# KdaiP/StableTTS

Measured on AMD Instinct MI355X. Metric: mel-frames/sec (whole node), 31M DiT, n_timesteps=10+CFG, higher is better.
Workload: dtype f16

## Files before the change

### stabletts_amd/csrc/common.h

```cpp
#pragma once
#include <hip/hip_runtime.h>
#include <stdint.h>

namespace st {

typedef __attribute__((ext_vector_type(8))) __bf16 bf16x8_t;
typedef __attribute__((ext_vector_type(8))) _Float16 f16x8_t;
typedef __attribute__((ext_vector_type(16))) float f32x16_t;
typedef __attribute__((ext_vector_type(4))) float f32x4_t;

struct OpBF16 {
    using elem = __bf16;
    using vec8 = bf16x8_t;
    static constexpr float kMaskedScore = -1e30f;
    static __device__ __forceinline__ f32x16_t mfma(vec8 a, vec8 b, f32x16_t c) {
        return __builtin_amdgcn_mfma_f32_32x32x16_bf16(a, b, c, 0, 0, 0);
    }
    static __device__ __forceinline__ f32x4_t mfma16(vec8 a, vec8 b, f32x4_t c) {
        return __builtin_amdgcn_mfma_f32_16x16x32_bf16(a, b, c, 0, 0, 0);
    }
};
struct OpF16 {
    using elem = _Float16;
    using vec8 = f16x8_t;
    static constexpr float kMaskedScore = -60000.0f;
    static __device__ __forceinline__ f32x16_t mfma(vec8 a, vec8 b, f32x16_t c) {
        return __builtin_amdgcn_mfma_f32_32x32x16_f16(a, b, c, 0, 0, 0);
    }
    static __device__ __forceinline__ f32x4_t mfma16(vec8 a, vec8 b, f32x4_t c) {
        return __builtin_amdgcn_mfma_f32_16x16x32_f16(a, b, c, 0, 0, 0);
    }
};

template <class P>
__device__ __forceinline__ typename P::elem to16(float f) { return (typename P::elem)f; }

template <class P>
__device__ __forceinline__ uint2 pack4(float a, float b, float c, float d) {
    typedef __attribute__((ext_vector_type(4))) typename P::elem v4;
    v4 v;
    v[0] = (typename P::elem)a; v[1] = (typename P::elem)b;
    v[2] = (typename P::elem)c; v[3] = (typename P::elem)d;
    return __builtin_bit_cast(uint2, v);
}

template <class P>
__device__ __forceinline__ uint2 scale_pack4(float a, float b, float c, float d, float s) {
    float pa = a * s, pb = b * s, pc = c * s, pd = d * s;
    asm volatile("" : "+v"(pa), "+v"(pb), "+v"(pc), "+v"(pd));
    return pack4<P>(pa, pb, pc, pd);
}

template <class P>
__device__ __forceinline__ uint2 scale_pack4_lo(float a, float b, float c, float d, float s) {
    float pa = a * s, pb = b * s, pc = c * s, pd = d * s;
    asm volatile("" : "+v"(pa), "+v"(pb), "+v"(pc), "+v"(pd));
    return pack4<P>(pa - (float)to16<P>(pa), pb - (float)to16<P>(pb), pc - (float)to16<P>(pc), pd - (float)to16<P>(pd));
}

template <class P>
__device__ __forceinline__ typename P::vec8 as_vec8(uint4 v) {
    return __builtin_bit_cast(typename P::vec8, v);
}

__device__ __forceinline__ float silu_f(float x) { return x / (1.0f + expf(-x)); }
__device__ __forceinline__ float silu_grad(float a) {
    const float s = 1.0f / (1.0f + expf(-a));
    return s * (1.0f + a * (1.0f - s));
}

__device__ __forceinline__ float silu_fast(float x) {
    return x * __builtin_amdgcn_rcpf(1.0f + __builtin_amdgcn_exp2f(-1.4426950408889634f * x));
}
__device__ __forceinline__ float silu_grad_fast(float a) {
    const float s = __builtin_amdgcn_rcpf(1.0f + __builtin_amdgcn_exp2f(-1.4426950408889634f * a));
    return s * (1.0f + a * (1.0f - s));
}

__device__ __forceinline__ float gelu_erf(float x) {
    const float z = x * 0.70710678118654752f, az = fabsf(z);
    const float t = __builtin_amdgcn_rcpf(fmaf(0.3275911f, az, 1.0f));
    const float poly = t * fmaf(t, fmaf(t, fmaf(t, fmaf(t, 1.061405429f, -1.453152027f), 1.421413741f), -0.284496736f), 0.254829592f);
    const float e = __builtin_amdgcn_exp2f(-1.4426950408889634f * z * z);
    const float er = copysignf(fmaf(-poly, e, 1.0f), z);
    return 0.5f * x * (1.0f + er);
}

__device__ __forceinline__ float add_f32_scalar(float a, float b) { return a + b; }
__device__ __forceinline__ float add_f32_asm_safe(float a, float b) {
    float r;
    asm("s_nop 0\n\tv_add_f32 %0, %1, %2" : "=v"(r) : "v"(a), "v"(b));
    return r;
}

__device__ __forceinline__ void rope_rot(float& x1, float& x2, float c, float s) {
#pragma clang fp contract(off)
    const float p = x2 * s, q = x1 * s;
    const float a = __builtin_fmaf(x1, c, -p), b = __builtin_fmaf(x2, c, q);
    x1 = a; x2 = b;
}

template <int CTRL>
__device__ __forceinline__ float dpp_add(float v) {
    return v + __uint_as_float(__builtin_amdgcn_update_dpp(0u, __float_as_uint(v), CTRL, 0xf, 0xf, false));
}
__device__ __forceinline__ float xor32_sum(float v) {
    const auto r = __builtin_amdgcn_permlane32_swap(__float_as_uint(v), __float_as_uint(v), false, false);
    return __uint_as_float(r[0]) + __uint_as_float(r[1]);
}
__device__ __forceinline__ float xor32_max(float v) {
    const auto r = __builtin_amdgcn_permlane32_swap(__float_as_uint(v), __float_as_uint(v), false, false);
    return fmaxf(__uint_as_float(r[0]), __uint_as_float(r[1]));
}
__device__ __forceinline__ float wave_sum(float v) {
    v = dpp_add<0x128>(v); v = dpp_add<0x124>(v); v = dpp_add<0x122>(v); v = dpp_add<0x121>(v);
    const auto a = __builtin_amdgcn_permlane16_swap(__float_as_uint(v), __float_as_uint(v), false, false);
    return xor32_sum(__uint_as_float(a[0]) + __uint_as_float(a[1]));
}

typedef unsigned u32x4_t __attribute__((ext_vector_type(4)));
typedef unsigned u32x2_t __attribute__((ext_vector_type(2)));
#if !defined(ST_ROW_STORE_POLICY) && defined(ST_ROW_STORE_POL)
#if ST_ROW_STORE_POL == 1
#define ST_ROW_STORE_POLICY "nt"
#elif ST_ROW_STORE_POL == 2
#define ST_ROW_STORE_POLICY "sc1 nt"
#elif ST_ROW_STORE_POL == 3
#define ST_ROW_STORE_POLICY "sc0 sc1"
#elif ST_ROW_STORE_POL == 4
#define ST_ROW_STORE_POLICY "sc0 sc1 nt"
#endif
#endif
#ifndef ST_ROW_STORE_POLICY
#define ST_ROW_STORE_POLICY "sc1"
#endif
__device__ __forceinline__ void store_row16(void* p, uint4 v) {
    asm volatile("global_store_dwordx4 %0, %1, off " ST_ROW_STORE_POLICY "\n\ts_nop 1" :: "v"(p), "v"(__builtin_bit_cast(u32x4_t, v)) : "memory");
}
__device__ __forceinline__ void store_row16(void* p, float4 v) { store_row16(p, __builtin_bit_cast(uint4, v)); }
__device__ __forceinline__ void store_row8(void* p, uint2 v) {
    asm volatile("global_store_dwordx2 %0, %1, off " ST_ROW_STORE_POLICY "\n\ts_nop 1" :: "v"(p), "v"(__builtin_bit_cast(u32x2_t, v)) : "memory");
}

typedef __attribute__((address_space(3))) void lds_void_t;
typedef __attribute__((address_space(1))) const void global_cvoid_t;

__device__ __forceinline__ void glds16b(const void* gsrc, unsigned char* lds_wave_base) {
    const unsigned off = __builtin_amdgcn_readfirstlane((unsigned)(uintptr_t)(lds_void_t*)lds_wave_base);
    unsigned keep;
    asm volatile("s_mov_b32 %0, m0\n\ts_mov_b32 m0, %2\n\ts_nop 0\n\tglobal_load_lds_dwordx4 %1, off\n\ts_mov_b32 m0, %0"
                 : "=&s"(keep) : "v"(gsrc), "s"(off) : "memory");
}
__device__ __forceinline__ void glds16s(const void* sbase, unsigned voff, unsigned char* lds_wave_base) {
    const unsigned off = __builtin_amdgcn_readfirstlane((unsigned)(uintptr_t)(lds_void_t*)lds_wave_base);
    unsigned keep;
    asm volatile("s_mov_b32 %0, m0\n\ts_mov_b32 m0, %3\n\ts_nop 0\n\tglobal_load_lds_dwordx4 %1, %2\n\ts_mov_b32 m0, %0"
                 : "=&s"(keep) : "v"(voff), "s"(sbase), "s"(off) : "memory");
}
__device__ __forceinline__ void glds16o(const void* sbase, unsigned voff, unsigned lds_off) {
    unsigned keep;
    asm volatile("s_mov_b32 %0, m0\n\ts_mov_b32 m0, %3\n\ts_nop 0\n\tglobal_load_lds_dwordx4 %1, %2\n\ts_mov_b32 m0, %0"
                 : "=&s"(keep) : "v"(voff), "s"(sbase), "s"(lds_off) : "memory");
}
__device__ __forceinline__ void glds16bo(const void* gsrc, unsigned lds_off) {
    unsigned keep;
    asm volatile("s_mov_b32 %0, m0\n\ts_mov_b32 m0, %2\n\ts_nop 0\n\tglobal_load_lds_dwordx4 %1, off\n\ts_mov_b32 m0, %0"
                 : "=&s"(keep) : "v"(gsrc), "s"(lds_off) : "memory");
}
__device__ __forceinline__ void glds4bo(const void* gsrc, unsigned lds_off) {
    unsigned keep;
    asm volatile("s_mov_b32 %0, m0\n\ts_mov_b32 m0, %2\n\ts_nop 0\n\tglobal_load_lds_dword %1, off\n\ts_mov_b32 m0, %0"
                 : "=&s"(keep) : "v"(gsrc), "s"(lds_off) : "memory");
}
__device__ __forceinline__ const unsigned char* sgpr_ptr64(const void* p) {
    const uintptr_t v = (uintptr_t)p;
    return (const unsigned char*)(((uintptr_t)(unsigned)__builtin_amdgcn_readfirstlane((int)(v >> 32)) << 32) |
                                  (unsigned)__builtin_amdgcn_readfirstlane((int)(unsigned)v));
}
__device__ __forceinline__ uint4 lds_read16(unsigned addr) {
    typedef unsigned __attribute__((ext_vector_type(4))) u32x4_raw;
    const u32x4_raw v = *(const __attribute__((address_space(3))) u32x4_raw*)(uintptr_t)addr;
    return make_uint4(v[0], v[1], v[2], v[3]);
}
#define ST_DMA_WAIT(n) asm volatile("s_waitcnt vmcnt(" #n ")" ::: "memory")

__host__ __device__ __forceinline__ unsigned drop_mix32(unsigned h) {
    h ^= h >> 16; h *= 0x85ebca6bu; h ^= h >> 13; h *= 0xc2b2ae35u; h ^= h >> 16;
    return h;
}
__host__ __device__ __forceinline__ unsigned drop_pair(unsigned rh, unsigned ch) {
    unsigned h = (rh ^ ch) * 0x9E3779B1u;
    return h ^ (h >> 15);
}
__host__ __device__ __forceinline__ unsigned drop_rowh(unsigned long long seed, unsigned row) { return drop_mix32((unsigned)seed ^ (row * 0x9E3779B1u)); }
__host__ __device__ __forceinline__ unsigned drop_colh(unsigned long long seed, unsigned j) { return drop_mix32((unsigned)(seed >> 32) ^ (j * 0x85ebca77u)); }
template <class D>
// ... 38 lines not shown
```

### stabletts_amd/csrc/conv_gemm2_impl.h

```cpp
#pragma once
#include "common.h"
#include "launch.h"
#include <algorithm>
#include <cstdlib>

#ifndef ST_STAGE_TIMING
#define ST_STAGE_TIMING 0
#endif

namespace st {

template <int BC, int BF, int WC, int WF, int TAPS, int WBUF = 2>
struct G2Cfg {
    static constexpr int NW = WC * WF, NT = 64 * NW;
    static constexpr int TC = BC / WC, TF = BF / WF, FC = TC / 32, FF = TF / 32;
    static constexpr int AROWS = BF + TAPS - 1;
    static constexpr int A_BYTES = AROWS * 128, W_BYTES = BC * 128;
    static constexpr int PITCH = BC + 4;
    static constexpr int STAGE_BYTES = (NW == 8 ? TF : BF) * PITCH * 4;
    static constexpr int STAGE16_BYTES = BF * (BC * 2 + 16);
    static constexpr int LOOP_BYTES = 2 * A_BYTES + WBUF * W_BYTES;
    static constexpr int LDS_MAX2 = LOOP_BYTES > STAGE_BYTES ? LOOP_BYTES : STAGE_BYTES;
    static constexpr int LDS_BYTES = LDS_MAX2 > STAGE16_BYTES ? LDS_MAX2 : STAGE16_BYTES;
    static_assert((BC / 8) % NW == 0 && (BF / 8) % NW == 0, "DMA pieces must split evenly over the waves");
// ... 27 lines not shown
                                        const float4 (&xin)[R]) {
    size_t grow[R];
#pragma unroll
    for (int u = 0; u < R; ++u) grow[u] = (size_t)n * g.T + t[u];
    static_assert(EPI != EPI_ACT16, "EPI_ACT16 has its own epilogue (g2_epilogue_act16)");
    {
        if constexpr (EPI == EPI_F32) {
            const bool msk = g.flags & GF_MASK;
#pragma unroll
            for (int u = 0; u < R; ++u) {
                const float mm = msk ? m[u] : 1.0f;
                v[u].x = (v[u].x + k.bias.x + xin[u].x) * mm; v[u].y = (v[u].y + k.bias.y + xin[u].y) * mm;
                v[u].z = (v[u].z + k.bias.z + xin[u].z) * mm; v[u].w = (v[u].w + k.bias.w + xin[u].w) * mm;
            }
        } else {
            if (g.branch32) {
#pragma unroll
                for (int u = 0; u < R; ++u)
                    if (ok[u]) store_row16(g.branch32 + grow[u] * g.cout + ch,
                                           make_float4((v[u].x + k.bias.x) * m[u], (v[u].y + k.bias.y) * m[u], (v[u].z + k.bias.z) * m[u], (v[u].w + k.bias.w) * m[u]));
            }
#pragma unroll
            for (int u = 0; u < R; ++u) {
                v[u].x = xin[u].x + k.gate.x * ((v[u].x + k.bias.x) * m[u]); v[u].y = xin[u].y + k.gate.y * ((v[u].y + k.bias.y) * m[u]);
                v[u].z = xin[u].z + k.gate.z * ((v[u].z + k.bias.z) * m[u]); v[u].w = xin[u].w + k.gate.w * ((v[u].w + k.bias.w) * m[u]);
            }
        }
        if (g.out16) {
#pragma unroll
            for (int u = 0; u < R; ++u)
                if (ok[u]) store_row8((unsigned char*)g.out16 + (grow[u] * g.cout + ch) * 2, pack4<P>(v[u].x, v[u].y, v[u].z, v[u].w));
            if (g.out16_lo) {
#pragma unroll
                for (int u = 0; u < R; ++u) {
                    const float4 l = make_float4(v[u].x - (float)to16<P>(v[u].x), v[u].y - (float)to16<P>(v[u].y),
                                                 v[u].z - (float)to16<P>(v[u].z), v[u].w - (float)to16<P>(v[u].w));
                    if (ok[u]) store_row8((unsigned char*)g.out16_lo + (grow[u] * g.cout + ch) * 2, pack4<P>(l.x, l.y, l.z, l.w));
                }
            }
        }
        if constexpr (LN) {
            if (g.ln_h16) {
                if (g.ln_film) {
#pragma unroll
                    for (int u = 0; u < R; ++u) {
                        v[u].x = (k.ga.x * v[u].x + k.be.x) * m[u]; v[u].y = (k.ga.y * v[u].y + k.be.y) * m[u];
                        v[u].z = (k.ga.z * v[u].z + k.be.z) * m[u]; v[u].w = (k.ga.w * v[u].w + k.be.w) * m[u];
                    }
                }
                if (g.out32) {
#pragma unroll
                    for (int u = 0; u < R; ++u)
                        if (ok[u]) store_row16(g.out32 + grow[u] * g.cout + ch, v[u]);
                }
                float mean[R], rstd[R];
#pragma unroll
                for (int u = 0; u < R; ++u) mean[u] = wave_sum(v[u].x + v[u].y + v[u].z + v[u].w) * (1.0f / 256.0f);
#pragma unroll
                for (int u = 0; u < R; ++u) {
                    v[u].x -= mean[u]; v[u].y -= mean[u]; v[u].z -= mean[u]; v[u].w -= mean[u];
                    rstd[u] = wave_sum(v[u].x * v[u].x + v[u].y * v[u].y + v[u].z * v[u].z + v[u].w * v[u].w) * (1.0f / 256.0f);
                }
                const bool mout = g.ln_mask_out;
#pragma unroll
                for (int u = 0; u < R; ++u) {
                    const float rs = 1.0f / sqrtf(rstd[u] + 1e-5f);
                    const float mm = mout ? m[u] : 1.0f;
                    const float h0 = (v[u].x * rs * (1.0f + k.sc.x) + k.sh.x) * mm, h1 = (v[u].y * rs * (1.0f + k.sc.y) + k.sh.y) * mm;
                    const float h2 = (v[u].z * rs * (1.0f + k.sc.z) + k.sh.z) * mm, h3 = (v[u].w * rs * (1.0f + k.sc.w) + k.sh.w) * mm;
                    if (ok[u]) store_row8((unsigned char*)g.ln_h16 + (grow[u] * 256 + ch) * 2, pack4<P>(h0, h1, h2, h3));
                }
                return;
            }
        }
        if (g.out32 && !(EPI == EPI_RESGATE && g.out32_readonly)) {
#pragma unroll
            for (int u = 0; u < R; ++u)
                if (ok[u]) store_row16(g.out32 + grow[u] * g.cout + ch, v[u]);
        }
    }
}

template <class P, int EPI, int BC, int BF, int WC, int WF, class Park>
__device__ __forceinline__ void g2_epilogue_core(Park park, float* stage, const ConvGemmArgs& g,
                                                 int n, int t0, int fvalid, int cbase, int wave, int lane) {
    constexpr int NW = WC * WF, TF = BF / WF, PITCH = BC + 4;
    const int l31 = lane & 31, hi = lane >> 5;
    const int wf = wave / WC;
    const int T = g.T;
    static_assert(EPI != EPI_QKV && EPI != EPI_ACT16 && EPI != EPI_SILU, "QKV: g2_epilogue_qkv; ACT16: g2_epilogue_act16; SILU: g2_epilogue_silu");
    static_assert(BC == 128 || BC == 256, "row walker handles 128 or 256 channels");
    constexpr bool LN = (BC == 256);
    constexpr int PASSF = (NW == 8) ? TF : BF, WFP = PASSF / TF, NPASS = BF / PASSF;
    static_assert(PASSF % TF == 0 && BF % PASSF == 0, "pass geometry");
    constexpr int RPW = LN ? PASSF / NW : PASSF / (2 * NW);
    const int chl = LN ? lane * 4 : l31 * 4;
    const G2Consts kc = g2_consts<EPI, LN>(g, n, cbase + chl);
    const float* mrow = g.mask ? g.mask + (size_t)(n % g.mask_mod) * T : nullptr;
    const int an = n < g.add_clamp ? n : g.add_clamp;
    const int tlim = g.t_lim ? min(T, g.t_lim[n % g.t_lim_mod]) : T;
#pragma unroll 1
    for (int p = 0; p < NPASS; ++p) {
        if (wf / WFP == p) park((wf % WFP) * TF);
        const int tbase = t0 + p * PASSF;
        float mk[RPW]; float4 xin[RPW]; int fr[RPW], tt[RPW]; bool ok[RPW];
#pragma unroll
        for (int u = 0; u < RPW; ++u) {
            const int f = LN ? (wave + u * NW) : ((wave + u * NW) * 2 + hi);
            const int t = tbase + f;
            fr[u] = f; tt[u] = t;
            ok[u] = (t < tlim) && (p * PASSF + f < fvalid);
            const int tl = t < tlim ? t : tlim - 1;
            mk[u] = mrow ? mrow[tl] : 1.0f;
            xin[u] = make_float4(0.f, 0.f, 0.f, 0.f);
            if constexpr (EPI == EPI_RESGATE) xin[u] = *(const float4*)((g.res32 ? g.res32 : g.out32) + ((size_t)n * T + tl) * g.cout + cbase + chl);
            if constexpr (EPI == EPI_F32) { if (g.add32) xin[u] = *(const float4*)(g.add32 + ((size_t)an * T + tl) * g.cout + cbase + chl); }
        }
        __syncthreads();
        constexpr int RB = (EPI != EPI_ACT16 && RPW > 4) ? 4 : RPW;
#pragma unroll
        for (int b0 = 0; b0 < RPW; b0 += RB) {
            float mk2[RB]; float4 xin2[RB], v[RB]; int tt2[RB]; bool ok2[RB];
#pragma unroll
            for (int u = 0; u < RB; ++u) {
                v[u] = *(const float4*)(stage + fr[b0 + u] * PITCH + chl);
                mk2[u] = mk[b0 + u]; xin2[u] = xin[b0 + u]; tt2[u] = tt[b0 + u]; ok2[u] = ok[b0 + u];
            }
            g2_rows<P, EPI, LN, RB>(g, kc, n, tt2, ok2, cbase + chl, v, mk2, xin2);
        }
        if (p + 1 < NPASS) __syncthreads();
    }
}

template <class P, int EPI, int BC, int BF, int WC, int WF>
__device__ __forceinline__ void g2_epilogue(f32x16_t (&acc)[BC / WC / 32][BF / WF / 32], float* stage, const ConvGemmArgs& g,
                                            int n, int t0, int fvalid, int cbase, int wave, int lane) {
    constexpr int TC = BC / WC, FC = TC / 32, FF = BF / WF / 32, PITCH = BC + 4;
    const int l31 = lane & 31, hi = lane >> 5, wc = wave % WC;
    g2_epilogue_core<P, EPI, BC, BF, WC, WF>([&](int fbase) {
#pragma unroll
        for (int a = 0; a < FC; ++a)
#pragma unroll
            for (int b = 0; b < FF; ++b)
#pragma unroll
                for (int q4 = 0; q4 < 4; ++q4) {
                    const int fl = fbase + b * 32 + l31;
                    const int ch = wc * TC + a * 32 + 8 * q4 + 4 * hi;
                    *(float4*)(stage + fl * PITCH + ch) = make_float4(acc[a][b][4 * q4 + 0], acc[a][b][4 * q4 + 1],
                                                                      acc[a][b][4 * q4 + 2], acc[a][b][4 * q4 + 3]);
                }
    }, stage, g, n, t0, fvalid, cbase, wave, lane);
}

template <int EPI, int FC, int FF>
__device__ __forceinline__ void g2_init_acc(f32x16_t (&acc)[FC][FF], const ConvGemmArgs& g, int chw, int hi) {
#pragma unroll
    for (int a = 0; a < FC; ++a)
#pragma unroll
        for (int q4 = 0; q4 < 4; ++q4) {
            float4 bv = make_float4(0.f, 0.f, 0.f, 0.f);
            if constexpr (EPI == EPI_ACT16 || EPI == EPI_GELU16 || EPI == EPI_QKV) { if (g.bias) bv = *(const float4*)(g.bias + chw + a * 32 + 8 * q4 + 4 * hi); }
#pragma unroll
            for (int b = 0; b < FF; ++b) {
                acc[a][b][4 * q4 + 0] = bv.x; acc[a][b][4 * q4 + 1] = bv.y;
                acc[a][b][4 * q4 + 2] = bv.z; acc[a][b][4 * q4 + 3] = bv.w;
            }
        }
}

template <class P, int BC, int BF, int WC, int WF, bool GELU = false>
__device__ __forceinline__ void g2_epilogue_act16(f32x16_t (&acc)[BC / WC / 32][BF / WF / 32], unsigned char* stage,
                                                  const ConvGemmArgs& g, int n, int t0, int fvalid, int cbase, int wave, int lane) {
    constexpr int NW = WC * WF, TC = BC / WC, TF = BF / WF, FC = TC / 32, FF = TF / 32, PB = BC * 2 + 16;
    const int l31 = lane & 31, hi = lane >> 5;
    const int wc = wave % WC, wf = wave / WC;
    const int T = g.T;
    const bool do_silu = g.flags & GF_SILU;
    const float* mrow = ((g.flags & GF_MASK) && g.mask) ? g.mask + (size_t)(n % g.mask_mod) * T : nullptr;
#pragma unroll
    for (int b = 0; b < FF; ++b) {
        const int fl = wf * TF + b * 32 + l31;
        const int t = t0 + fl;
        const float m = mrow ? mrow[t < T ? t : T - 1] : 1.0f;
        const bool allone = __all(m == 1.0f);
#pragma unroll
        for (int a = 0; a < FC; ++a) {
            f32x16_t v = acc[a][b];
            if constexpr (GELU) {
#pragma unroll
                for (int r = 0; r < 16; ++r) v[r] = gelu_erf(v[r]);
            } else if (do_silu) {
#pragma unroll
                for (int r = 0; r < 16; ++r) v[r] = silu_fast(v[r]);
            }
            if (!allone) {
#pragma unroll
                for (int r = 0; r < 16; ++r) v[r] *= m;
            }
#pragma unroll
            for (int q4 = 0; q4 < 4; ++q4) {
                const int ch = wc * TC + a * 32 + 8 * q4 + 4 * hi;
                *(uint2*)(stage + fl * PB + ch * 2) = pack4<P>(v[4 * q4 + 0], v[4 * q4 + 1], v[4 * q4 + 2], v[4 * q4 + 3]);
            }
        }
    }
    __syncthreads();
    constexpr int LPR = BC / 8, RPI = 64 / LPR;
    const int rsub = lane / LPR, cl = lane % LPR;
    unsigned char* obase = (unsigned char*)g.out16 + (((size_t)n * T + t0) * g.cout + cbase) * 2 + cl * 16;
#pragma unroll
    for (int i = 0; i < BF / (NW * RPI); ++i) {
        const int f = (i * NW + wave) * RPI + rsub;
        const uint4 v = *(const uint4*)(stage + f * PB + cl * 16);
        if (t0 + f < T && f < fvalid) store_row16(obase + (size_t)f * g.cout * 2, v);
    }
}

template <class P, int BC, int BF, int WC, int WF>
__device__ __forceinline__ void g2_epilogue_silu(f32x16_t (&acc)[BC / WC / 32][BF / WF / 32], unsigned char* stage,
                                                 const ConvGemmArgs& g, int n, int t0, int fvalid, int cbase, int wave, int lane) {
    constexpr int NW = WC * WF, TC = BC / WC, TF = BF / WF, FC = TC / 32, FF = TF / 32, PB = BC * 2 + 16;
    constexpr int LPR = BC / 8, RPI = 64 / LPR;
    typedef __attribute__((ext_vector_type(4))) typename P::elem v4;
    const int l31 = lane & 31, hi = lane >> 5;
    const int wc = wave % WC, wf = wave / WC;
    const int T = g.T;
    const float* mrow = g.mask ? g.mask + (size_t)(n % g.mask_mod) * T : nullptr;
    struct { unsigned long long seed; unsigned thresh16; float scale; } d = {g.drop_seed, g.drop_thresh16, g.drop_scale};
    const int rsub = lane / LPR, cl = lane % LPR;
    const size_t tile0 = (((size_t)n * T + t0) * g.cout + cbase) * 2 + cl * 16;
    auto rows_out = [&](void* dst) {
#pragma unroll
        for (int i = 0; i < BF / (NW * RPI); ++i) {
            const int f = (i * NW + wave) * RPI + rsub;
            const uint4 v = *(const uint4*)(stage + f * PB + cl * 16);
            if (t0 + f < T && f < fvalid) store_row16((unsigned char*)dst + tile0 + (size_t)f * g.cout * 2, v);
        }
    };
    const bool fwd = g.act16 != nullptr;
    if (!fwd) {
#pragma unroll
        for (int i = 0; i < BF / (NW * RPI); ++i) {
            const int f = (i * NW + wave) * RPI + rsub;
            uint4 v = make_uint4(0, 0, 0, 0);
            if (t0 + f < T && f < fvalid) v = *(const uint4*)((const unsigned char*)g.dact16 + tile0 + (size_t)f * g.cout * 2);
            *(uint4*)(stage + f * PB + cl * 16) = v;
        }
        __syncthreads();
    }
    auto factors = [&](int t, int ch, float2& f01, float2& f23) {
        f01 = make_float2(1.0f, 1.0f); f23 = f01;
        if (d.thresh16) {
            const unsigned long long i = ((unsigned long long)n * T + t) * g.cout + cbase + ch;
            f01 = drop_factors2(d, drop_ffn_hash(d, i)); f23 = drop_factors2(d, drop_ffn_hash(d, i + 2));
        }
    };
    if (fwd) {
#pragma unroll
        for (int b = 0; b < FF; ++b) {
            const int fl = wf * TF + b * 32 + l31;
#pragma unroll
            for (int a = 0; a < FC; ++a)
#pragma unroll
                for (int q4 = 0; q4 < 4; ++q4) {
                    const int ch = wc * TC + a * 32 + 8 * q4 + 4 * hi;
                    const float4 bv = g.bias ? *(const float4*)(g.bias + cbase + ch) : make_float4(0.f, 0.f, 0.f, 0.f);
                    *(uint2*)(stage + fl * PB + ch * 2) = pack4<P>(acc[a][b][4 * q4 + 0] + bv.x, acc[a][b][4 * q4 + 1] + bv.y,
                                                                   acc[a][b][4 * q4 + 2] + bv.z, acc[a][b][4 * q4 + 3] + bv.w);
                }
        }
        __syncthreads();
        rows_out(g.out16);
        __syncthreads();
    }
#pragma unroll
    for (int b = 0; b < FF; ++b) {
        const int fl = wf * TF + b * 32 + l31;
        const int t = t0 + fl;
        const float m = mrow ? mrow[t < T ? t : T - 1] : 1.0f;
#pragma unroll
        for (int a = 0; a < FC; ++a)
#pragma unroll
            for (int q4 = 0; q4 < 4; ++q4) {
                const int ch = wc * TC + a * 32 + 8 * q4 + 4 * hi;
                float2 f01, f23;
                factors(t, ch, f01, f23);
                const v4 pre = *(const v4*)(stage + fl * PB + ch * 2);
                uint2 o;
                if (fwd)
                    o = pack4<P>(silu_fast((float)pre[0]) * f01.x * m, silu_fast((float)pre[1]) * f01.y * m,
                                 silu_fast((float)pre[2]) * f23.x * m, silu_fast((float)pre[3]) * f23.y * m);
                else
                    o = pack4<P>(acc[a][b][4 * q4 + 0] * m * f01.x * silu_grad_fast((float)pre[0]), acc[a][b][4 * q4 + 1] * m * f01.y * silu_grad_fast((float)pre[1]),
                                 acc[a][b][4 * q4 + 2] * m * f23.x * silu_grad_fast((float)pre[2]), acc[a][b][4 * q4 + 3] * m * f23.y * silu_grad_fast((float)pre[3]));
                *(uint2*)(stage + fl * PB + ch * 2) = o;
            }
    }
    __syncthreads();
    rows_out(fwd ? g.act16 : g.out16);
}

constexpr int kQkvRowPitch = 144;
template <int BC, int BF> constexpr int g2_qkv_lds_bytes() {
    return (BC / 64) * BF * kQkvRowPitch > BC * (BF * 2 + 16) ? (BC / 64) * BF * kQkvRowPitch : BC * (BF * 2 + 16);
}
template <class P, int BC, int BF, int WC, int WF>
__device__ __forceinline__ void g2_epilogue_qkv(f32x16_t (&acc)[BC / WC / 32][BF / WF / 32], unsigned char* stage,
                                                const ConvGemmArgs& g, int n, int t0, int cbase, int wave, int lane) {
    static_assert(BC == 256 && (BC / WC) % 64 == 0, "one q/k/v plane per block, whole heads per wave");
    constexpr int NW = WC * WF, TC = BC / WC, TF = BF / WF, FF = TF / 32, HPW = TC / 64, PQ = kQkvRowPitch, PV = BF * 2 + 16;
    const int l31 = lane & 31, hi = lane >> 5;
    const int wc = wave % WC, wf = wave / WC;
    const int T = g.T, H = g.n_heads;
    const int which = cbase / BC;
    const int tlim = g.t_lim ? min(T, g.t_lim[n % g.t_lim_mod]) : T;
    if (which < 2) {
        const float sc = which == 0 ? g.qscale : 1.0f;
        unsigned char* dst_lo = (unsigned char*)(which == 0 ? g.q_lo : g.k_lo);
        for (int pass = 0; pass < (dst_lo ? 2 : 1); ++pass) {
        if (pass) __syncthreads();
#pragma unroll
        for (int b = 0; b < FF; ++b) {
            const int fl = wf * TF + b * 32 + l31;
            const int tl = t0 + fl < T ? t0 + fl : T - 1;
            float cc[2][4], ss[2][4];
#pragma unroll
            for (int q4 = 0; q4 < 2; ++q4) {
                const float4 cs = *(const float4*)(g.rope_cos + (size_t)tl * 16 + 8 * q4 + 4 * hi);
                const float4 sn = *(const float4*)(g.rope_sin + (size_t)tl * 16 + 8 * q4 + 4 * hi);
                cc[q4][0] = cs.x; cc[q4][1] = cs.y; cc[q4][2] = cs.z; cc[q4][3] = cs.w;
                ss[q4][0] = sn.x; ss[q4][1] = sn.y; ss[q4][2] = sn.z; ss[q4][3] = sn.w;
            }
#pragma unroll
            for (int hh = 0; hh < HPW; ++hh) {
                f32x16_t r = acc[2 * hh][b];
#pragma unroll
                for (int q4 = 0; q4 < 2; ++q4)
#pragma unroll
                    for (int e = 0; e < 4; ++e) {
                        float x1 = r[4 * q4 + e], x2 = r[4 * (q4 + 2) + e];
                        rope_rot(x1, x2, cc[q4][e], ss[q4][e]);
                        r[4 * q4 + e] = x1; r[4 * (q4 + 2) + e] = x2;
                    }
                unsigned char* row = stage + ((wc * HPW + hh) * BF + fl) * PQ + 4 * hi * 2;
#pragma unroll
                for (int q4 = 0; q4 < 4; ++q4) {
                    if (pass == 0) {
                        *(uint2*)(row + 16 * q4) = scale_pack4<P>(r[4 * q4 + 0], r[4 * q4 + 1], r[4 * q4 + 2], r[4 * q4 + 3], sc);
                        *(uint2*)(row + 64 + 16 * q4) = scale_pack4<P>(acc[2 * hh + 1][b][4 * q4 + 0], acc[2 * hh + 1][b][4 * q4 + 1],
                                                                       acc[2 * hh + 1][b][4 * q4 + 2], acc[2 * hh + 1][b][4 * q4 + 3], sc);
                    } else {
                        *(uint2*)(row + 16 * q4) = scale_pack4_lo<P>(r[4 * q4 + 0], r[4 * q4 + 1], r[4 * q4 + 2], r[4 * q4 + 3], sc);
                        *(uint2*)(row + 64 + 16 * q4) = scale_pack4_lo<P>(acc[2 * hh + 1][b][4 * q4 + 0], acc[2 * hh + 1][b][4 * q4 + 1],
                                                                          acc[2 * hh + 1][b][4 * q4 + 2], acc[2 * hh + 1][b][4 * q4 + 3], sc);
                    }
                }
            }
        }
        __syncthreads();
        unsigned char* dst = pass ? dst_lo : (unsigned char*)(which == 0 ? g.q : g.k);
        const int rsub = lane >> 3, seg = lane & 7;
#pragma unroll
        for (int i = 0; i < (BC / 64) * BF / (NW * 8); ++i) {
            const int rowid = (i * NW + wave) * 8 + rsub;
            const int head = rowid / BF, f = rowid % BF;
            const uint4 v = *(const uint4*)(stage + rowid * PQ + seg * 16);
            if (t0 + f < tlim) store_row16(dst + (((size_t)n * H + head) * T + t0 + f) * 128 + seg * 16, v);
        }
        }
    } else {
        auto plane = [&](auto pass_c, unsigned char* dst) {
            constexpr bool LO = decltype(pass_c)::value;
#pragma unroll
            for (int b = 0; b < FF; ++b) {
                const int fl = wf * TF + b * 32 + l31;
                const bool tv = t0 + fl < T;
                const int pos = (fl & ~12) | ((fl & 4) << 1) | ((fl & 8) >> 1);
#pragma unroll
                for (int a = 0; a < TC / 32; ++a)
#pragma unroll
                    for (int r = 0; r < 16; ++r) {
                        const int ch = wc * TC + a * 32 + (r & 3) + 8 * (r >> 2) + 4 * hi;
                        float x = tv ? acc[a][b][r] : 0.0f;
                        if constexpr (LO) {
                            asm volatile("" : "+v"(x));
                            x -= (float)to16<P>(x);
                        }
                        *(typename P::elem*)(stage + ch * PV + pos * 2) = to16<P>(x);
                    }
            }
            __syncthreads();
            constexpr int SPR = BF / 8, RPI = 64 / SPR;
            const int rsub = lane / SPR, seg = lane % SPR;
#pragma unroll
            for (int i = 0; i < BC / (NW * RPI); ++i) {
                const int ch = (i * NW + wave) * RPI + rsub;
                const uint4 v = *(const uint4*)(stage + ch * PV + seg * 16);
                const int tcol = t0 + seg * 8;
                if (tcol < g.Tp)
                    store_row16(dst + ((((size_t)n * H + (ch >> 6)) * 64 + (ch & 63)) * g.Tp + tcol) * 2, v);
            }
        };
        plane(std::false_type{}, (unsigned char*)g.vt);
        if (g.vt_lo) {
            __syncthreads();
            plane(std::true_type{}, (unsigned char*)g.vt_lo);
        }
    }
}

template <class P, int TAPS, int EPI, int BC, int BF, int WC, int WF, int WBUF = 2>
__global__ __launch_bounds__(64 * WC * WF, WBUF == 1 ? 4 : 2)
void conv_gemm2_kernel(const ConvGemmArgs g) {
    using vec8 = typename P::vec8;
    using K = G2Cfg<BC, BF, WC, WF, TAPS, WBUF>;
    constexpr int NW = K::NW, FC = K::FC, FF = K::FF, TC = K::TC, TF = K::TF;
    constexpr int A_BYTES = K::A_BYTES, W_BYTES = K::W_BYTES;

    extern __shared__ __attribute__((aligned(16))) unsigned char smem[];
    unsigned char* As = smem;
    unsigned char* Ws = smem + 2 * A_BYTES;

    const int ks = g.ksplit > 1 ? g.ksplit : 1;
    const int total = g.n_items * g.tiles_f * g.tiles_c * ks;
    const int per_xcd = gridDim.x >> 3;
    const int lin0 = (blockIdx.x & 7) * per_xcd + (blockIdx.x >> 3);
    if (lin0 >= total) return;
    const int kz = lin0 % ks;
    const int lin = lin0 / ks;
    const int tc = lin % g.tiles_c;
    const int rest = lin / g.tiles_c;
    const int tf = rest % g.tiles_f;
    const int n = rest / g.tiles_f;

    const int tid = threadIdx.x, lane = tid & 63;
    const int wave = __builtin_amdgcn_readfirstlane(tid >> 6);
    const int l31 = lane & 31, hi = lane >> 5;
    const int wc = wave % WC, wf = wave / WC;
    const int cbase = tc * BC, t0 = tf * BF;
    if (g.t_lim && t0 >= g.t_lim[n % g.t_lim_mod]) return;
    const int cin = g.c0 + g.c1 + g.c2;
    const int nch_all = (EPI == EPI_QKV && (g.flags & GF_K2_V_ONLY) && cbase < 2 * BC ? g.c0 : cin) >> 6;
    const int cb = kz * nch_all / ks, nch = (kz + 1) * nch_all / ks;
    const int T = g.T;

    const unsigned char* a0 = (const unsigned char*)g.a0 + (size_t)(n % g.a0_mod) * T * g.c0 * 2;
    const unsigned char* a1 = g.c1 ? (const unsigned char*)g.a1 + (size_t)(n % g.a1_mod) * T * g.c1 * 2 : nullptr;
    const unsigned char* wsrc = (const unsigned char*)g.w + (size_t)n * g.w_item_stride;

    constexpr int WPW = (BC / 8) / NW, APW = (BF / 8) / NW;
    const int prow = lane >> 3;
    unsigned voffW[WPW], voffA0[APW + 1], voffA1[APW + 1];
    bool validA[APW + 1];
#pragma unroll
    for (int k = 0; k < WPW; ++k) {
        const int row = (wave * WPW + k) * 8 + prow;
        voffW[k] = (unsigned)((cbase + row) * TAPS * cin * 2 + (((lane & 7) ^ ((row >> 1) & 7)) << 4));
    }
#pragma unroll
    for (int k = 0; k <= APW; ++k) {
        const int row = (k < APW) ? (wave * APW + k) * 8 + prow : BF + prow;
        const int t = t0 + row - (TAPS / 2);
        const unsigned segb = (unsigned)(((lane & 7) ^ ((row >> 1) & 7)) << 4);
        const bool mine = (k < APW) || (TAPS == 3 && wave == 0 && lane < 16);
        validA[k] = mine && (t >= 0 && t < T);
        voffA0[k] = (unsigned)(t * g.c0 * 2) + segb;
        voffA1[k] = (unsigned)(t * g.c1 * 2) + segb;
        if (mine && !(t >= 0 && t < T)) {
            const int pc = (k < APW) ? wave * APW + k : BF / 8;
            *(uint4*)(As + pc * 1024 + lane * 16) = make_uint4(0, 0, 0, 0);
            *(uint4*)(As + A_BYTES + pc * 1024 + lane * 16) = make_uint4(0, 0, 0, 0);
        }
    }
    auto issueW = [&](int c, int j, int buf) {
        const unsigned char* sb = wsrc + (size_t)(j * cin + (c << 6)) * 2;
#pragma unroll
        for (int k = 0; k < WPW; ++k) glds16s(sb, voffW[k], Ws + buf * W_BYTES + (wave * WPW + k) * 1024);
    };
    auto issueA = [&](int c, int buf) {
        int ch0 = c << 6;
        if (ch0 >= g.c0 + g.c1) ch0 -= g.c0 + g.c1;
        if (ch0 < g.c0) {
            const unsigned char* sb = a0 + (size_t)ch0 * 2;
#pragma unroll
            for (int k = 0; k <= APW; ++k) {
                if (k == APW && TAPS != 3) continue;
                const int pc = (k < APW) ? wave * APW + k : BF / 8;
                if (validA[k]) glds16s(sb, voffA0[k], As + buf * A_BYTES + pc * 1024);
            }
        } else {
            const unsigned char* sb = a1 + (size_t)(ch0 - g.c0) * 2;
#pragma unroll
            for (int k = 0; k <= APW; ++k) {
                if (k == APW && TAPS != 3) continue;
                const int pc = (k < APW) ? wave * APW + k : BF / 8;
                if (validA[k]) glds16s(sb, voffA1[k], As + buf * A_BYTES + pc * 1024);
            }
        }
    };

    f32x16_t acc[FC][FF];
    g2_init_acc<EPI, FC, FF>(acc, g, cbase + wc * TC, hi);

    int wrow_off[FC], wswz[FC];
#pragma unroll
    for (int a = 0; a < FC; ++a) {
        const int row = wc * TC + a * 32 + l31;
        wrow_off[a] = row * 128; wswz[a] = (row >> 1) & 7;
    }
    auto compute = [&](int abuf, int wbuf, int j) {
        const unsigned char* Ab = As + abuf * A_BYTES;
        const unsigned char* Wb = Ws + wbuf * W_BYTES;
        int arow_off[FF], aswz[FF];
#pragma unroll
        for (int b = 0; b < FF; ++b) {
            const int row = wf * TF + b * 32 + l31 + j;
            arow_off[b] = row * 128; aswz[b] = (row >> 1) & 7;
        }
#pragma unroll
        for (int ks = 0; ks < 4; ++ks) {
            vec8 wfr[FC], afr[FF];
            const int seg = ks * 2 + hi;
#pragma unroll
            for (int a = 0; a < FC; ++a) wfr[a] = as_vec8<P>(*(const uint4*)(Wb + wrow_off[a] + ((seg ^ wswz[a]) << 4)));
#pragma unroll
            for (int b = 0; b < FF; ++b) afr[b] = as_vec8<P>(*(const uint4*)(Ab + arow_off[b] + ((seg ^ aswz[b]) << 4)));
#pragma unroll
            for (int a = 0; a < FC; ++a)
#pragma unroll
                for (int b = 0; b < FF; ++b) acc[a][b] = P::mfma(wfr[a], afr[b], acc[a][b]);
        }
    };

    issueA(cb, cb & 1); issueW(cb, 0, 0);
    ST_DMA_WAIT(0);
    __syncthreads();
#if ST_STAGE_TIMING
    unsigned long long tm_issue = 0, tm_compute = 0, tm_dma = 0, tm_barrier = 0, tm_n = 0;
    unsigned long long tS = __builtin_amdgcn_s_memtime();
    const unsigned long long tStart = tS;
#endif
    int it = 0;
    for (int c = cb; c < nch; ++c) {
#pragma unroll
        for (int j = 0; j < TAPS; ++j) {
            const bool last = (c == nch - 1) && (j == TAPS - 1);
            if constexpr (WBUF == 1) {
                if ((j == 0) && (c + 1 < nch)) issueA(c + 1, (c + 1) & 1);
                compute(c & 1, 0, j);
                __syncthreads();
                if (!last) { if (j == TAPS - 1) issueW(c + 1, 0, 0); else issueW(c, j + 1, 0); }
                ST_DMA_WAIT(0);
                __syncthreads();
                ++it;
                continue;
            }
            if ((j == 0) && (c + 1 < nch)) issueA(c + 1, (c + 1) & 1);
            if (!last) { if (j == TAPS - 1) issueW(c + 1, 0, (it + 1) & 1); else issueW(c, j + 1, (it + 1) & 1); }
#if ST_STAGE_TIMING
            const unsigned long long tA = __builtin_amdgcn_s_memtime();
#endif
            compute(c & 1, it & 1, j);
#if ST_STAGE_TIMING
            asm volatile("s_waitcnt lgkmcnt(0)" ::: "memory");
            const unsigned long long tB = __builtin_amdgcn_s_memtime();
#endif
            ST_DMA_WAIT(0);
#if ST_STAGE_TIMING
            const unsigned long long tC = __builtin_amdgcn_s_memtime();
#endif
            __syncthreads();
#if ST_STAGE_TIMING
            {
                const unsigned long long tD = __builtin_amdgcn_s_memtime();
                tm_issue += tA - tS; tm_compute += tB - tA; tm_dma += tC - tB; tm_barrier += tD - tC; tS = tD; ++tm_n;
            }
#endif
            ++it;
        }
    }

#if ST_STAGE_TIMING
    const unsigned long long tLoop = __builtin_amdgcn_s_memtime();
#endif
    if constexpr (EPI == EPI_ACT16 || EPI == EPI_GELU16)
        g2_epilogue_act16<P, BC, BF, WC, WF, EPI == EPI_GELU16>(acc, smem, g, n, t0, BF, cbase, wave, lane);
    else if constexpr (EPI == EPI_QKV) g2_epilogue_qkv<P, BC, BF, WC, WF>(acc, smem, g, n, t0, cbase, wave, lane);
    else g2_epilogue<P, EPI, BC, BF, WC, WF>(acc, (float*)smem, g, kz * g.n_items + n, t0, BF, cbase, wave, lane);
#if ST_STAGE_TIMING
    if (g.dbg && lane == 0 && (wave == 0 || wave == NW - 1) && lin < 64) {
        unsigned long long* d = g.dbg + (size_t)(lin * 2 + (wave ? 1 : 0)) * 8;
        d[0] = tm_issue; d[1] = tm_compute; d[2] = tm_dma; d[3] = tm_barrier; d[4] = tm_n;
        d[5] = tLoop - tStart; d[6] = __builtin_amdgcn_s_memtime() - tLoop; d[7] = 1;
    }
#endif
}

template <class P, int EPI, int BC, int BF, int WC, int WF>
__global__ __launch_bounds__(64 * WC * WF, 2) void conv_gemm3_kernel(const ConvGemmArgs g) {
    using vec8 = typename P::vec8;
    constexpr int BFV = BF - 2, NW = WC * WF, TC = BC / WC, TF = BF / WF, FC = TC / 32, FF = TF / 32;
    constexpr int A_BYTES = BF * 128, W_BYTES = BC * 128;
    constexpr int WPW = (BC / 8) / NW, APW = (BF / 8) / NW;
    static_assert(WPW == 4 && APW == 4, "the counted waits below assume 4 + 4 pieces per wave");
    extern __shared__ __attribute__((aligned(16))) unsigned char smem[];
    unsigned char* As = smem;
    unsigned char* Ws = smem + 2 * A_BYTES;

    const int total = g.n_items * g.tiles_f * g.tiles_c;
    const int per_xcd = gridDim.x >> 3;
    const int lin = (blockIdx.x & 7) * per_xcd + (blockIdx.x >> 3);
    if (lin >= total) return;
    const int tc = lin % g.tiles_c;
    const int rest = lin / g.tiles_c;
    const int tf = rest % g.tiles_f;
    const int n = rest / g.tiles_f;

    const int tid = threadIdx.x, lane = tid & 63;
    const int wave = __builtin_amdgcn_readfirstlane(tid >> 6);
    const int l31 = lane & 31, hi = lane >> 5;
    const int wc = wave % WC, wf = wave / WC;
    const int cbase = tc * BC, t0 = tf * BFV;
    if (g.t_lim && t0 >= g.t_lim[n % g.t_lim_mod]) return;
    const int cin = g.c0 + g.c1;
    const int nch = cin >> 6;
    const int nst = nch * 3;
    const int T = g.T;

    const unsigned char* a0 = (const unsigned char*)g.a0 + (size_t)(n % g.a0_mod) * T * g.c0 * 2;
    const unsigned char* a1 = g.c1 ? (const unsigned char*)g.a1 + (size_t)(n % g.a1_mod) * T * g.c1 * 2 : nullptr;
    const unsigned char* wsrc = (const unsigned char*)g.w;
    const unsigned char* zeros = (const unsigned char*)g.zeros;

    const int prow = lane >> 3;
    auto issueW = [&](int c, int j, int buf) {
#pragma unroll
        for (int k = 0; k < WPW; ++k) {
            const int piece = wave * WPW + k;
            const int row = piece * 8 + prow;
            const int seg = (lane & 7) ^ ((row >> 1) & 7);
            const unsigned char* src = wsrc + ((size_t)((cbase + row) * 3 + j) * cin + (c << 6)) * 2 + seg * 16;
            glds16b(src, Ws + buf * W_BYTES + piece * 1024);
        }
    };
    auto issueA = [&](int c, int buf) {
        const int ch0 = c << 6;
        const unsigned char* srcb; int cs, coff;
        if (ch0 < g.c0) { srcb = a0; cs = g.c0; coff = ch0; }
        else            { srcb = a1; cs = g.c1; coff = ch0 - g.c0; }
#pragma unroll
        for (int k = 0; k < APW; ++k) {
            const int piece = wave * APW + k;
            const int row = piece * 8 + prow;
            const int seg = (lane & 7) ^ ((row >> 1) & 7);
            const int t = t0 + row - 1;
            const unsigned char* src = (t >= 0 && t < T) ? srcb + ((size_t)t * cs + coff) * 2 + seg * 16 : zeros;
            glds16b(src, As + buf * A_BYTES + piece * 1024);
        }
    };

    f32x16_t acc[FC][FF];
    g2_init_acc<EPI, FC, FF>(acc, g, cbase + wc * TC, hi);

    int wrow_off[FC], wswz[FC];
#pragma unroll
    for (int a = 0; a < FC; ++a) {
        const int row = wc * TC + a * 32 + l31;
        wrow_off[a] = row * 128; wswz[a] = (row >> 1) & 7;
    }
    auto compute = [&](int abuf, int wbuf, int j) {
        const unsigned char* Ab = As + abuf * A_BYTES;
        const unsigned char* Wb = Ws + wbuf * W_BYTES;
        int arow_off[FF], aswz[FF];
#pragma unroll
        for (int b = 0; b < FF; ++b) {
            const int row = wf * TF + b * 32 + l31 + j;
            arow_off[b] = row * 128; aswz[b] = (row >> 1) & 7;
        }
#pragma unroll
        for (int ks = 0; ks < 4; ++ks) {
            vec8 wfr[FC], afr[FF];
            const int seg = ks * 2 + hi;
#pragma unroll
            for (int a = 0; a < FC; ++a) wfr[a] = as_vec8<P>(*(const uint4*)(Wb + wrow_off[a] + ((seg ^ wswz[a]) << 4)));
#pragma unroll
            for (int b = 0; b < FF; ++b) afr[b] = as_vec8<P>(*(const uint4*)(Ab + arow_off[b] + ((seg ^ aswz[b]) << 4)));
#pragma unroll
            for (int a = 0; a < FC; ++a)
#pragma unroll
                for (int b = 0; b < FF; ++b) acc[a][b] = P::mfma(wfr[a], afr[b], acc[a][b]);
        }
    };
    auto wait_keep = [&](int keep) {
        if (keep >= 8)      asm volatile("s_waitcnt vmcnt(8)" ::: "memory");
        else if (keep >= 4) asm volatile("s_waitcnt vmcnt(4)" ::: "memory");
        else                asm volatile("s_waitcnt vmcnt(0)" ::: "memory");
    };

    issueA(0, 0); issueW(0, 0, 0);
    if (nst > 1) issueW(0, 1, 1);
    wait_keep(0);
    __builtin_amdgcn_s_barrier();
    for (int c = 0; c < nch; ++c) {
#pragma unroll
        for (int j = 0; j < 3; ++j) {
            const int gi = c * 3 + j;
            int younger = 0;
            if (j == 0 && c + 1 < nch) { issueA(c + 1, (c + 1) & 1); younger += 4; }
            if (gi + 2 < nst) {
                if (j == 0) issueW(c, 2, 2); else issueW(c + 1, j - 1, j - 1);
                younger += 4;
            }
            compute(c & 1, j, j);
            wait_keep(younger);
            asm volatile("s_waitcnt lgkmcnt(0)" ::: "memory");
            __builtin_amdgcn_s_barrier();
        }
    }
    if constexpr (EPI == EPI_ACT16) g2_epilogue_act16<P, BC, BF, WC, WF>(acc, smem, g, n, t0, BFV, cbase, wave, lane);
    else g2_epilogue<P, EPI, BC, BF, WC, WF>(acc, (float*)smem, g, n, t0, BFV, cbase, wave, lane);
}

template <class P, int EPI>
__global__ __launch_bounds__(256) void splitk_finish_kernel(const ConvGemmArgs g, const float* __restrict__ part, int S) {
    const int lane = threadIdx.x & 63;
    const int wave = __builtin_amdgcn_readfirstlane((int)(threadIdx.x >> 6));
    const int rows = g.n_items * g.T;
    const int row = blockIdx.x * 4 + wave;
    if (row >= rows) return;
    const int n = row / g.T, t = row - n * g.T;
    const int ch = lane * 4;
    const G2Consts kc = g2_consts<EPI, true>(g, n, ch);
    const float* src = part + (size_t)row * 256 + ch;
    const size_t plane = (size_t)rows * 256;
    float4 v[1]; v[0] = *(const float4*)src;
    int s = 1;
    for (; s + 4 <= S; s += 4) {
        float4 p[4];
#pragma unroll
        for (int i = 0; i < 4; ++i) p[i] = *(const float4*)(src + (s + i) * plane);
#pragma unroll
        for (int i = 0; i < 4; ++i) { v[0].x += p[i].x; v[0].y += p[i].y; v[0].z += p[i].z; v[0].w += p[i].w; }
    }
    for (; s < S; ++s) {
        const float4 p = *(const float4*)(src + s * plane);
        v[0].x += p.x; v[0].y += p.y; v[0].z += p.z; v[0].w += p.w;
    }
    const float m[1] = {g.mask ? g.mask[(size_t)(n % g.mask_mod) * g.T + t] : 1.0f};
    float4 xin[1]; xin[0] = make_float4(0.f, 0.f, 0.f, 0.f);
    if constexpr (EPI == EPI_RESGATE) xin[0] = *(const float4*)((g.res32 ? g.res32 : g.out32) + (size_t)row * 256 + ch);
    if constexpr (EPI == EPI_F32) {
        if (g.add32) xin[0] = *(const float4*)(g.add32 + ((size_t)(n < g.add_clamp ? n : g.add_clamp) * g.T + t) * 256 + ch);
    }
    const int tt[1] = {t}; const bool ok[1] = {true};
    g2_rows<P, EPI, true, 1>(g, kc, n, tt, ok, ch, v, m, xin);
}

template <class P>
static hipError_t launch_splitk_finish_t(int epi, const ConvGemmArgs& a, const float* part, int S, hipStream_t s) {
    if (a.cout != 256 || S < 1 || !part) return hipErrorInvalidValue;
    const int rows = a.n_items * a.T;
    const dim3 grid((rows + 3) / 4), blk(256);
    if (epi == EPI_F32) hipLaunchKernelGGL((splitk_finish_kernel<P, EPI_F32>), grid, blk, 0, s, a, part, S);
    else if (epi == EPI_RESGATE) hipLaunchKernelGGL((splitk_finish_kernel<P, EPI_RESGATE>), grid, blk, 0, s, a, part, S);
    else return hipErrorInvalidValue;
    return hipGetLastError();
}

template <class P, int EPI, int BC = 128, int BF = 128, int WC = 2, int WF = 2>
static hipError_t launch_g3(const ConvGemmArgs& a, hipStream_t s) {
    constexpr int lds_loop = 2 * BF * 128 + 3 * BC * 128, lds_stage = (WC * WF == 8 ? BF / WF : BF) * (BC + 4) * 4;
    constexpr int lds2 = lds_loop > lds_stage ? lds_loop : lds_stage, lds16 = BF * (BC * 2 + 16);
    constexpr int lds = lds2 > lds16 ? lds2 : lds16;
    static bool attr_done_dev[64] = {};
    int dev_ = 0;
    if (hipGetDevice(&dev_) != hipSuccess || dev_ < 0 || dev_ >= 64) return hipErrorInvalidDevice;
    bool& attr_done = attr_done_dev[dev_];
    if (!attr_done) {
        hipError_t e = hipFuncSetAttribute((const void*)conv_gemm3_kernel<P, EPI, BC, BF, WC, WF>, hipFuncAttributeMaxDynamicSharedMemorySize, lds);
        if (e != hipSuccess) return e;
        attr_done = true;
    }
    if (!a.zeros || (a.cout % BC) != 0 || ((a.c0 | a.c1) & 63) != 0 || a.c2 != 0 || a.ksplit > 1) return hipErrorInvalidValue;
    ConvGemmArgs b = a;
    b.tiles_f = (a.T + BF - 3) / (BF - 2);
    b.tiles_c = a.cout / BC;
    const int total = b.n_items * b.tiles_f * b.tiles_c;
    const int grid = ((total + 7) / 8) * 8;
    hipLaunchKernelGGL((conv_gemm3_kernel<P, EPI, BC, BF, WC, WF>), dim3(grid), dim3(64 * WC * WF), lds, s, b);
    return hipGetLastError();
}

template <class P, int TAPS, int EPI, int BC, int BF, int WC, int WF, int WBUF = 2>
static hipError_t launch_g2(const ConvGemmArgs& a, hipStream_t s) {
    using K = G2Cfg<BC, BF, WC, WF, TAPS, WBUF>;
    constexpr int qkv_lds = (EPI == EPI_QKV) ? g2_qkv_lds_bytes<BC, BF>() : 0;
    constexpr int LDS = K::LDS_BYTES > qkv_lds ? K::LDS_BYTES : qkv_lds;
    static bool attr_done_dev[64] = {};
    int dev_ = 0;
    if (hipGetDevice(&dev_) != hipSuccess || dev_ < 0 || dev_ >= 64) return hipErrorInvalidDevice;
    bool& attr_done = attr_done_dev[dev_];
    if (!attr_done) {
        hipError_t e = hipFuncSetAttribute((const void*)conv_gemm2_kernel<P, TAPS, EPI, BC, BF, WC, WF, WBUF>,
                                           hipFuncAttributeMaxDynamicSharedMemorySize, LDS);
        if (e != hipSuccess) return e;
        attr_done = true;
    }
    if (!a.zeros || (a.cout % BC) != 0 || ((a.c0 | a.c1 | a.c2) & 63) != 0 || (a.c2 && a.c2 > a.c0)) return hipErrorInvalidValue;
    ConvGemmArgs b = a;
    b.tiles_f = (a.T + BF - 1) / BF;
    b.tiles_c = a.cout / BC;
    if (a.ksplit > 1) {
        if (EPI != EPI_F32 || a.bias || a.add32 || a.out16 || a.ln_h16 || (a.flags & GF_MASK) || !a.out32 ||
            a.ksplit > (a.c0 + a.c1 + a.c2) / 64 || a.w_item_stride)
            return hipErrorInvalidValue;
    }
    const int total = b.n_items * b.tiles_f * b.tiles_c * (a.ksplit > 1 ? a.ksplit : 1);
    const int grid = ((total + 7) / 8) * 8;
    if (EPI == EPI_QKV && (a.cout != 3 * BC || a.n_heads * 64 != BC || !a.q || !a.k || !a.vt)) return hipErrorInvalidValue;
    hipLaunchKernelGGL((conv_gemm2_kernel<P, TAPS, EPI, BC, BF, WC, WF, WBUF>), dim3(grid), dim3(K::NT), LDS, s, b);
    return hipGetLastError();
}

}
```

### stabletts_amd/csrc/conv_gemm2_inst.h

```cpp
#pragma once
#include "conv_gemm2_impl.h"
#include "conv_gemm_phased.h"

namespace st {

template <class P>
static hipError_t launch_conv_gemm2_t(int cfg, int taps, int epi, const ConvGemmArgs& a, hipStream_t s) {
    if (cfg == 0) {
        if (taps == 3 && epi == EPI_ACT16) return launch_g2<P, 3, EPI_ACT16, 128, 128, 2, 2>(a, s);
        if (taps == 1 && epi == EPI_F32) return launch_g2<P, 1, EPI_F32, 128, 128, 2, 2>(a, s);
        if (taps == 3 && epi == EPI_F32) return launch_g2<P, 3, EPI_F32, 128, 128, 2, 2>(a, s);
        if (taps == 1 && epi == EPI_RESGATE) return launch_g2<P, 1, EPI_RESGATE, 128, 128, 2, 2>(a, s);
        if (taps == 3 && epi == EPI_RESGATE) return launch_g2<P, 3, EPI_RESGATE, 128, 128, 2, 2>(a, s);
        if (taps == 1 && epi == EPI_GELU16) return launch_g2<P, 1, EPI_GELU16, 128, 128, 2, 2>(a, s);
    } else if (cfg == 1) {
        if (taps == 3 && epi == EPI_F32) return launch_g2<P, 3, EPI_F32, 256, 128, 4, 2>(a, s);
        if (taps == 1 && epi == EPI_F32) return launch_g2<P, 1, EPI_F32, 256, 128, 4, 2>(a, s);
        if (taps == 3 && epi == EPI_RESGATE) return launch_g2<P, 3, EPI_RESGATE, 256, 128, 4, 2>(a, s);
        if (taps == 1 && epi == EPI_RESGATE) return launch_g2<P, 1, EPI_RESGATE, 256, 128, 4, 2>(a, s);
        if (taps == 1 && epi == EPI_QKV) return launch_g2<P, 1, EPI_QKV, 256, 128, 4, 2>(a, s);
    } else if (cfg == 3) {
        if (taps == 3 && epi == EPI_ACT16) return launch_g2<P, 3, EPI_ACT16, 256, 256, 2, 4>(a, s);
        if (taps == 3 && epi == EPI_F32) return launch_g2<P, 3, EPI_F32, 256, 256, 2, 4>(a, s);
        if (taps == 1 && epi == EPI_F32) return launch_g2<P, 1, EPI_F32, 256, 256, 2, 4>(a, s);
        if (taps == 3 && epi == EPI_RESGATE) return launch_g2<P, 3, EPI_RESGATE, 256, 256, 2, 4>(a, s);
        if (taps == 1 && epi == EPI_RESGATE) return launch_g2<P, 1, EPI_RESGATE, 256, 256, 2, 4>(a, s);
        if (taps == 1 && epi == EPI_QKV) return launch_g2<P, 1, EPI_QKV, 256, 256, 2, 4>(a, s);
        if (taps == 1 && epi == EPI_GELU16) return launch_g2<P, 1, EPI_GELU16, 256, 256, 2, 4>(a, s);
    } else if (cfg == 4) {
        if (taps == 3 && epi == EPI_ACT16) return launch_g2<P, 3, EPI_ACT16, 128, 64, 2, 2>(a, s);
        if (taps == 1 && epi == EPI_F32) return launch_g2<P, 1, EPI_F32, 128, 64, 2, 2>(a, s);
        if (taps == 3 && epi == EPI_F32) return launch_g2<P, 3, EPI_F32, 128, 64, 2, 2>(a, s);
    } else if (cfg == 5) {
        if (taps == 1 && epi == EPI_QKV) return launch_g2<P, 1, EPI_QKV, 256, 64, 4, 2>(a, s);
    } else if (cfg == 6) {
        if (taps == 3 && epi == EPI_ACT16) return launch_phased3<P, EPI_ACT16>(a, s);
        if (taps == 3 && epi == EPI_F32) return launch_phased3<P, EPI_F32>(a, s);
        if (taps == 3 && epi == EPI_RESGATE) return launch_phased3<P, EPI_RESGATE>(a, s);
        if (taps == 3 && epi == EPI_SILU) return launch_phased3<P, EPI_SILU>(a, s);
    } else if (cfg == 7) {
        if (taps == 1 && epi == EPI_QKV) return launch_g2<P, 1, EPI_QKV, 256, 128, 4, 2, 1>(a, s);
    } else if (cfg == 2) {
        if (taps == 3 && epi == EPI_ACT16) return launch_g3<P, EPI_ACT16>(a, s);
        if (taps == 3 && epi == EPI_F32) return launch_g3<P, EPI_F32>(a, s);
        if (taps == 3 && epi == EPI_RESGATE) return launch_g3<P, EPI_RESGATE>(a, s);
    }
    return hipErrorInvalidValue;
}

}
```

### stabletts_amd/csrc/engine.cpp

```cpp
#include "engine_internal.h"
#include "train_launch.h"
#include "mas_launch.h"
#include "align_train_launch.h"

#include <algorithm>
#include <cmath>
#include <cstdio>
#include <cstring>
#include <map>
#include <string>
#include <vector>

using namespace st;
using namespace sthost;

namespace sthost {
std::string g_create_error;

const char* kProfNames[PC_COUNT] = {
    "prep", "prenet_conv", "in_proj", "film_ln1", "qkv_rope", "attention", "out_proj", "ln2",
    "ffn_conv1", "ffn_conv2", "lsc_conv", "final_proj", "ode_update", "train_forward", "train_backward"};

int dev_alloc(st_engine* e, void** p, size_t bytes) {
    HIPCHK(e, hipMalloc(p, bytes ? bytes : 16));
// ... 37 lines not shown
            expect(e, p + "block.attn.conv_" + nm + ".bias", {C});
        }
        expect(e, p + "block.mlp.conv_1.weight", {F, C, K}); expect(e, p + "block.mlp.conv_1.bias", {F});
        expect(e, p + "block.mlp.conv_2.weight", {C, F, K}); expect(e, p + "block.mlp.conv_2.bias", {C});
        if (G != C) {
            expect(e, p + "block.adaLN_modulation.0.weight", {C, G});
            expect(e, p + "block.adaLN_modulation.0.bias", {C});
        }
        expect(e, p + "block.adaLN_modulation.2.weight", {6 * C, C});
        expect(e, p + "block.adaLN_modulation.2.bias", {6 * C});
    }
    expect(e, "final_proj.weight", {M, C, 1}); expect(e, "final_proj.bias", {M});
    expect(e, "cond_proj.0.weight", {F, M, K}); expect(e, "cond_proj.0.bias", {F});
    expect(e, "cond_proj.2.weight", {F, F, K}); expect(e, "cond_proj.2.bias", {F});
    expect(e, "cond_proj.4.weight", {C, F, K}); expect(e, "cond_proj.4.bias", {C});
    for (int i = 0; i < e->L / 2; ++i) {
        expect(e, "lsc_layers." + std::to_string(i) + ".weight", {C, 2 * C, K});
        expect(e, "lsc_layers." + std::to_string(i) + ".bias", {C});
    }
}

const float* P(st_engine* e, const std::string& name) { return e->params.at(name).dev; }

static bool big_tiles(const st_engine* e, const ConvGemmArgs& a) {
    const int T = a.T;
    const bool fills = ((T + 255) / 256) * 256 * 10 <= ((T + 127) / 128) * 128 * 11;
    const bool big_fills_chip = (int64_t)e->conc * a.n_items * ((T + 255) / 256) * (a.cout / 256) >= e->big_min_blocks;
    return a.cout % 256 == 0 && fills && big_fills_chip;
}
bool gemm_is_phased(const st_engine* e, int taps, const ConvGemmArgs& a) { return taps == 3 && e->phased && big_tiles(e, a); }

hipError_t gemm(st_engine* e, int taps, int epi, const ConvGemmArgs& a, hipStream_t s) {
    const bool bf = e->dt == DT_BF16;
    const int T = a.T;
    if (epi == EPI_SILU && !gemm_is_phased(e, taps, a)) return hipErrorInvalidValue;
    if (e->kpart && e->conc == 1 && a.cout == 256 && (epi == EPI_F32 || epi == EPI_RESGATE) && !a.w_item_stride) {
        const int nch = (a.c0 + a.c1 + a.c2) / 64;
        const int64_t blocks = (int64_t)a.n_items * ((T + 127) / 128) * 2;
        const int64_t plane = (int64_t)a.n_items * T * 256 * 4;
        int ks = (int)std::min<int64_t>(std::min(nch, e->splitk_max), e->splitk_target / blocks);
        ks = (int)std::min<int64_t>(ks, (int64_t)e->kpart_bytes / plane);
        if (ks >= 2 && nch * taps >= e->splitk_min_stages) {
            ConvGemmArgs pa = a;
            pa.t_lim = nullptr;
            pa.bias = nullptr; pa.flags = 0; pa.mask = nullptr; pa.add32 = nullptr; pa.out16 = nullptr; pa.out16_lo = nullptr;
            pa.ln_h16 = nullptr; pa.gate = nullptr; pa.res32 = nullptr; pa.branch32 = nullptr; pa.out32 = e->kpart; pa.ksplit = ks;
            const int pcfg = e->small_tiles ? G2_T64 : G2_T128;
            hipError_t he = bf ? launch_conv_gemm2_bf16(pcfg, taps, EPI_F32, pa, s) : launch_conv_gemm2_f16(pcfg, taps, EPI_F32, pa, s);
            if (he != hipSuccess) return he;
            return bf ? launch_splitk_finish_bf16(epi, a, e->kpart, ks, s) : launch_splitk_finish_f16(epi, a, e->kpart, ks, s);
        }
    }
    if (epi == EPI_QKV && e->qkv_ws && !a.q_lo && !a.vt_lo && e->sink && a.w_frag && a.cout == 768 && a.c0 == 256 && !a.c1 && !a.c2 && a.n_heads == 4 &&
        (int64_t)a.n_items * ((T + 63) / 64) >= e->qkv_ws_min_tiles) {
        ConvGemmArgs b = a; b.sink = e->sink;
        return launch_qkv_ws(e->dt, b, s);
    }
    if (epi == EPI_RESGATE && taps == 1 && e->oproj_ws && e->sink && a.w_frag && a.ln_h16 && !a.ln_film && a.cout == 256 && a.c0 == 256 &&
        !a.c1 && !a.c2 && !a.out16 && !a.res32 && !a.branch32 && !a.out32_readonly && a.out32 &&
        (int64_t)a.n_items * ((T + 31) / 32) >= e->oproj_ws_min_tiles) {
        ConvGemmArgs b = a; b.sink = e->sink;
        return launch_oproj_ws(e->dt, b, s);
    }
    int cfg;
    if (big_tiles(e, a)) cfg = (e->phased && taps == 3) ? G2_PHASED : (epi == EPI_QKV && e->qkv_rc1) ? G2_RC1 : G2_BIG;
    else if (a.ln_h16 || epi == EPI_QKV) cfg = G2_RC;
    else if (taps == 3 && a.c0 + a.c1 >= 512 && a.c2 == 0) cfg = G2_K3PIPE;
    else cfg = G2_T128;
    const bool tiny = e->small_tiles && e->conc == 1 && (int64_t)a.n_items * ((T + 127) / 128) * (a.cout / 128) <= e->small_tiles;
    if (tiny && cfg == G2_T128 && (epi == EPI_ACT16 ? taps == 3 : epi == EPI_F32)) cfg = G2_T64;
    if (tiny && cfg == G2_RC && epi == EPI_QKV) cfg = G2_RC64;
    return bf ? launch_conv_gemm2_bf16(cfg, taps, epi, a, s) : launch_conv_gemm2_f16(cfg, taps, epi, a, s);
}

ProfScope::ProfScope(st_engine* e_, hipStream_t s_, int cls, double flops) : e(e_), s(s_) {
    if (!e->prof || !((e->prof_mask >> cls) & 1ull)) return;
    if ((e->prof_seen[cls]++ % e->prof_stride) != 0) return;
    ProfEvent ev; ev.cls = cls; ev.flops = flops;
    for (hipEvent_t* h : {&ev.a, &ev.b}) {
        if (!e->ev_pool.empty()) { *h = e->ev_pool.back(); e->ev_pool.pop_back(); }
        else if (hipEventCreate(h) != hipSuccess) return;
    }
    hipEventRecord(ev.a, s);
    e->evs.push_back(ev);
    idx = (int)e->evs.size() - 1;
}
ProfScope::~ProfScope() { if (idx >= 0) hipEventRecord(e->evs[idx].b, s); }

void prof_collect(st_engine* e) {
    for (auto& ev : e->evs) {
        float ms = 0.f;
        if (hipEventSynchronize(ev.b) == hipSuccess && hipEventElapsedTime(&ms, ev.a, ev.b) == hipSuccess) {
            e->prof_launches[ev.cls] += 1;
            e->prof_ms[ev.cls] += ms;
            e->prof_flops[ev.cls] = ev.flops;
        }
        e->ev_pool.push_back(ev.a); e->ev_pool.push_back(ev.b);
    }
    e->evs.clear();
}

void capture(st_engine* e, const std::string& name, const void* dev, int64_t n, bool is16, hipStream_t s) {
    if (!e->capture) return;
    Captured& c = e->caps[name];
    const size_t bytes = (size_t)n * (is16 ? 2 : 4);
    if (c.dev) { hipFree(c.dev); c.dev = nullptr; }
    if (hipMalloc(&c.dev, bytes) != hipSuccess) { c.dev = nullptr; return; }
    c.n = n; c.is16 = is16;
    hipMemcpyAsync(c.dev, dev, bytes, hipMemcpyDeviceToDevice, s);
}

size_t layout_plan(st_engine* e, int B, int T, bool cfg, int n_t, size_t off, Plan* p) {
    const int C = e->C, F = e->F, Mp = e->Mp, L = e->L;
    p->B = B; p->T = T; p->cfg = cfg; p->n_t = n_t;
    p->Tp = (T + 63) / 64 * 64;
    p->N = cfg ? 2 * B : B;
    p->Pn = cfg ? B + 1 : B;
    const size_t N = p->N, Pn = p->Pn, TT = T;
    p->slots.clear();
    auto want = [&](void** dst, size_t bytes) { p->slots.push_back({dst, off}); off = align_up(off + bytes, 256); };
    want(&p->mu16, Pn * TT * Mp * 2);
    want(&p->pre1, Pn * TT * F * 2);
    want(&p->pre2, Pn * TT * F * 2);
    want(&p->cond16, Pn * TT * C * 2);
    want(&p->cond16lo, Pn * TT * C * 2);
    want((void**)&p->cpart, Pn * TT * C * 4);
    want(&p->x16, (size_t)B * TT * Mp * 2);
    want(&p->x16lo, (size_t)B * TT * Mp * 2);
    want((void**)&p->xstate, (size_t)B * TT * Mp * 4);
    for (int i = 0; i < 7; ++i) want((void**)&p->kbuf[i], (size_t)B * TT * Mp * 4);
    want((void**)&p->ynew, (size_t)B * TT * Mp * 4);
    want((void**)&p->ode_partial, (size_t)2 * kOdeNormBlocks * 4);
    want((void**)&p->ode_out, 16);
    want((void**)&p->X, N * TT * C * 4);
    want(&p->h16, N * TT * C * 2);
    want(&p->h2_16, N * TT * C * 2);
    want(&p->q16, N * TT * C * 2);
    want(&p->k16, N * TT * C * 2);
    want(&p->q16lo, N * TT * C * 2);
    want(&p->k16lo, N * TT * C * 2);
    want(&p->vt16, N * (size_t)C * p->Tp * 2);
    want(&p->ao16, N * TT * C * 2);
    want(&p->u16, N * TT * F * 2);
    want(&p->cur16, N * TT * C * 2);
    want(&p->cur16lo, N * TT * C * 2);
    for (int i = 0; i < L / 2; ++i) want(&p->skip16[i], N * TT * C * 2);
    want((void**)&p->v32, N * TT * Mp * 4);
    want((void**)&p->tvals, (size_t)n_t * 4);
    want((void**)&p->emb, (size_t)n_t * C * 4);
    want((void**)&p->th, (size_t)n_t * F * 4);
    want((void**)&p->tau, (size_t)n_t * C * 4);
    want((void**)&p->film, (size_t)L * n_t * 2 * C * 4);
    want((void**)&p->cvec, N * (size_t)e->G * 4);
    want((void**)&p->ada_tmp, N * (size_t)C * 4);
    want((void**)&p->ada, (size_t)L * N * 6 * C * 4);
    want((void**)&p->n_full, (size_t)B * 4);
    want((void**)&p->kv_end, (size_t)B * 4);
    want((void**)&p->t_lim, (size_t)(B + 1) * 4);
    want((void**)&p->kbias, (size_t)B * p->Tp * 4);
    want((void**)&p->maskbuf, (size_t)B * TT * 4);
    return off;
}

int ensure_ws(st_engine* e, size_t bytes) {
    if (bytes <= e->ws_cap) return ST_OK;
    e->drop_graphs();
    if (e->ws) { HIPCHK(e, hipDeviceSynchronize()); HIPCHK(e, hipFree(e->ws)); e->ws = nullptr; e->ws_cap = 0; }
    HIPCHK(e, hipMalloc((void**)&e->ws, bytes));
    e->ws_cap = bytes;
    e->ws_sig = 0;
    return ST_OK;
}

int arena_fresh(st_engine* e, uint64_t sig, size_t used_bytes, hipStream_t s) {
    if (sig == e->ws_sig) return ST_OK;
    HIPCHK(e, hipMemsetAsync(e->ws, 0, used_bytes, s));
    e->ws_sig = sig;
    return ST_OK;
}

uint64_t layout_sig(int entry, int B, int T, int cfg, int n_t, int parts) {
    uint64_t h = 1469598103934665603ull;
    for (uint64_t v : {(uint64_t)entry, (uint64_t)B, (uint64_t)T, (uint64_t)cfg, (uint64_t)n_t, (uint64_t)parts}) { h ^= v + 0x9E3779B97F4A7C15ull; h *= 1099511628211ull; }
    return h | 1ull;
}

void bind_plan(st_engine* e, Plan* p) {
    for (auto& sl : p->slots) *sl.dst = e->ws + sl.off;
}

int make_plan(st_engine* e, int B, int T, bool cfg, int n_t, Plan* p) {
    const size_t end = layout_plan(e, B, T, cfg, n_t, 0, p);
    int rc = ensure_ws(e, end); if (rc) return rc;
    bind_plan(e, p);
    return ST_OK;
}

int ensure_rope(st_engine* e, int T, hipStream_t s) {
    if (T <= e->rope_T) return ST_OK;
    const int newT = (T + 255) / 256 * 256;
    std::vector<float> hc((size_t)newT * 16), hs((size_t)newT * 16);
    for (int j = 0; j < 16; ++j) {
        const float theta = 1.0f / powf(10000.0f, (float)(2 * j) / 32.0f);
        for (int t = 0; t < newT; ++t) {
            const float ang = (float)t * theta;
            hc[(size_t)t * 16 + j] = cosf(ang);
            hs[(size_t)t * 16 + j] = sinf(ang);
        }
    }
    if (e->rope_cos) {
        e->drop_graphs();
        HIPCHK(e, hipDeviceSynchronize()); hipFree(e->rope_cos); hipFree(e->rope_sin);
        e->rope_cos = e->rope_sin = nullptr; e->rope_T = 0;
    }
    HIPCHK(e, hipMalloc((void**)&e->rope_cos, hc.size() * 4));
    HIPCHK(e, hipMalloc((void**)&e->rope_sin, hs.size() * 4));
    HIPCHK(e, hipMemcpy(e->rope_cos, hc.data(), hc.size() * 4, hipMemcpyHostToDevice));
    HIPCHK(e, hipMemcpy(e->rope_sin, hs.data(), hs.size() * 4, hipMemcpyHostToDevice));
    e->rope_T = newT;
    (void)s;
    return ST_OK;
}

ConvGemmArgs base_args(const st_engine* e, const Plan& p, const Conv& cv, int n_items) {
    ConvGemmArgs a;
    memset(&a, 0, sizeof(a));
    a.w = cv.w; a.bias = cv.bias; a.cout = cv.cout; a.T = p.T; a.n_items = n_items;
    a.tiles_f = (p.T + kGemmFramesPerTile - 1) / kGemmFramesPerTile;
    a.tiles_c = cv.cout / kGemmChannelsPerTile;
    a.a0_mod = n_items; a.a1_mod = n_items; a.mask_mod = p.B;
    a.zeros = e->zeros;
    if (e->ragged_skip && !e->capture && e->kind == KIND_DECODER) { a.t_lim = p.t_lim; a.t_lim_mod = (n_items == p.B + 1) ? p.B + 1 : p.B; }
    return a;
}

inline double conv_flops(const Plan& p, const Conv& cv, int n_items) {
    return 2.0 * (double)n_items * p.T * cv.cout * (cv.split ? cv.cin / 3 : cv.cin) * cv.taps;
}

int run_prenet(st_engine* e, const Plan& p, hipStream_t s) {
    {
        ConvGemmArgs a = base_args(e, p, e->pre[0], p.Pn);
        a.a0 = p.mu16; a.c0 = e->Mp; a.flags = GF_SILU; a.out16 = p.pre1;
        ProfScope ps(e, s, PC_PRENET, conv_flops(p, e->pre[0], p.Pn));
        HIPCHK(e, gemm(e, 3, EPI_ACT16, a, s));
    }
    {
        ConvGemmArgs a = base_args(e, p, e->pre[1], p.Pn);
        a.a0 = p.pre1; a.c0 = e->F; a.flags = GF_SILU; a.out16 = p.pre2;
        ProfScope ps(e, s, PC_PRENET, conv_flops(p, e->pre[1], p.Pn));
        HIPCHK(e, gemm(e, 3, EPI_ACT16, a, s));
    }
    {
        ConvGemmArgs a = base_args(e, p, e->pre[2], p.Pn);
        a.a0 = p.pre2; a.c0 = e->F; a.out16 = p.cond16; a.out16_lo = p.cond16lo;
        ProfScope ps(e, s, PC_PRENET, conv_flops(p, e->pre[2], p.Pn));
        HIPCHK(e, gemm(e, 3, EPI_F32, a, s));
    }
    capture(e, "cond", p.cond16, (int64_t)p.Pn * p.T * e->C, true, s);
    {
        ConvGemmArgs a = base_args(e, p, e->inc, p.Pn);
        a.a0 = p.cond16; a.c0 = e->C; a.a1 = p.cond16lo; a.c1 = e->C; a.c2 = e->C; a.out32 = p.cpart;
        ProfScope ps(e, s, PC_INPROJ, conv_flops(p, e->inc, p.Pn));
        HIPCHK(e, gemm(e, 1, EPI_F32, a, s));
    }
    return ST_OK;
}

int run_adaln(st_engine* e, const Plan& p, hipStream_t s) {
    const int C = e->C;
    ProfScope ps(e, s, PC_PREP, 0);
    if (e->G == C) HIPCHK(e, launch_silu_rows(p.cvec, (int64_t)p.N * C, p.ada_tmp, s));
    for (int i = 0; i < e->L; ++i) {
        const std::string pre = e->blk(i) + "adaLN_modulation.";
        if (e->G != C) {
            HIPCHK(e, launch_linear(p.cvec, p.N, e->G, P(e, pre + "0.weight"), P(e, pre + "0.bias"), C, p.ada_tmp, 0, 0, s));
            HIPCHK(e, launch_linear(p.ada_tmp, p.N, C, P(e, pre + "2.weight"), P(e, pre + "2.bias"), 6 * C,
                                    p.ada + (size_t)i * p.N * 6 * C, 1, 0, s));
        } else {
            HIPCHK(e, launch_linear(p.ada_tmp, p.N, C, P(e, pre + "2.weight"), P(e, pre + "2.bias"), 6 * C,
                                    p.ada + (size_t)i * p.N * 6 * C, 0, 0, s));
        }
    }
    return ST_OK;
}

int run_time_tables(st_engine* e, const Plan& p, hipStream_t s) {
    const int C = e->C, F = e->F;
    ProfScope ps(e, s, PC_PREP, 0);
    HIPCHK(e, launch_time_embed(p.tvals, p.n_t, C, p.emb, s));
    HIPCHK(e, launch_linear(p.emb, p.n_t, C, P(e, "time_mlp.layer.0.weight"), P(e, "time_mlp.layer.0.bias"), F, p.th, 0, 1, s));
    HIPCHK(e, launch_linear(p.th, p.n_t, F, P(e, "time_mlp.layer.2.weight"), P(e, "time_mlp.layer.2.bias"), C, p.tau, 0, 0, s));
    for (int i = 0; i < e->L; ++i) {
        const std::string pre = "blocks." + std::to_string(i) + ".time_fusion.film.";
        HIPCHK(e, launch_linear(p.tau, p.n_t, C, P(e, pre + "weight"), P(e, pre + "bias"), 2 * C,
                                p.film + (size_t)i * p.n_t * 2 * C, 0, 0, s));
    }
    return ST_OK;
}

int run_estimator(st_engine* e, const Plan& p, const float* mask, int ev, hipStream_t s) {
    const int C = e->C, F = e->F, L = e->L, N = p.N, T = p.T;
    const int64_t rowsC = (int64_t)N * T * C;
    const bool cap = e->capture;
    const bool dec = e->kind == KIND_DECODER;
    const bool film = dec;
    const bool skips = dec;
    const bool dec_fast_paths = dec;
    const bool split_qk = dec_fast_paths && e->attn_split;
    const bool ragged = dec_fast_paths && e->ragged_skip && !cap;
    const int ln1_by_ffn = skips ? L / 2 : L;
    auto ada_of = [&](int i) { return p.ada + (size_t)i * N * 6 * C; };
    auto fuse_ln1 = [&](ConvGemmArgs& a, int i) {
        a.ln_film = nullptr; a.ln_film_stride = 0; a.ln_film_mod = 1;
        if (film) {
            const float* fb = p.film + (size_t)i * p.n_t * 2 * C;
            if (ev >= 0) a.ln_film = fb + (size_t)ev * 2 * C;
            else         { a.ln_film = fb; a.ln_film_stride = 2 * C; a.ln_film_mod = p.B; }
        }
        a.ln_ada = ada_of(i); a.ln_ada_stride = 6 * C; a.ln_shift_off = 0; a.ln_scale_off = C;
        a.ln_mask_out = 0; a.ln_h16 = p.h16; a.mask = mask;
    };
    if (film) {
        ConvGemmArgs a = base_args(e, p, e->inx, N);
        a.a0 = p.x16; a.c0 = e->Mp; a.a0_mod = p.B; a.a1 = p.x16lo; a.c1 = e->Mp; a.a1_mod = p.B; a.c2 = e->Mp;
        a.bias = nullptr;
        a.add32 = p.cpart; a.add_clamp = p.B;
        a.out32 = p.X; a.out16 = p.skip16[0];
        fuse_ln1(a, 0);
        ProfScope ps(e, s, PC_INPROJ, conv_flops(p, e->inx, N));
        HIPCHK(e, gemm(e, 1, EPI_F32, a, s));
    } else {
        FilmLnArgs a; memset(&a, 0, sizeof(a));
        a.X = p.X; a.h16 = p.h16; a.film = nullptr; a.film_mod = 1;
        a.ada = ada_of(0); a.ada_stride = 6 * C; a.shift_off = 0; a.scale_off = C;
        a.mask = mask; a.mask_mod = p.B; a.mask_out = 0; a.T = T; a.rows = N * T;
        ProfScope ps(e, s, PC_FILM_LN1, 0);
        HIPCHK(e, launch_film_ln(e->dt, a, s));
    }
    if (film && cap) capture(e, "h0", p.skip16[0], rowsC, true, s);
    for (int i = 0; i < L; ++i) {
        const std::string bn = "b" + std::to_string(i) + ".";
        const float* ada_i = ada_of(i);
        if (skips && i >= L / 2) {
            const int j = i - L / 2;
            ConvGemmArgs a = base_args(e, p, e->lsc[j], N);
            a.a0 = p.cur16; a.c0 = C; a.a1 = p.skip16[L - 1 - i]; a.c1 = C;
            a.out32 = p.X;
            fuse_ln1(a, i);
            ProfScope ps(e, s, PC_LSC, conv_flops(p, e->lsc[j], N));
            if (!(e->skip_mask >> PC_LSC & 1)) HIPCHK(e, gemm(e, 3, EPI_F32, a, s));
        }
        if (cap) { capture(e, bn + "x1", p.X, rowsC, false, s); capture(e, bn + "h1", p.h16, rowsC, true, s); }
        {
            ConvGemmArgs a = base_args(e, p, e->qkv[i], N);
            a.a0 = p.h16; a.c0 = C;
            a.q = p.q16; a.k = p.k16; a.vt = p.vt16; a.rope_cos = e->rope_cos; a.rope_sin = e->rope_sin;
            if (split_qk) { a.q_lo = p.q16lo; a.k_lo = p.k16lo; }
            a.Tp = p.Tp; a.n_heads = e->H;
            if ((int)e->qkv_frag.size() == L) a.w_frag = e->qkv_frag[i];
            a.qscale = 1.4426950408889634f / sqrtf((float)(C / e->H));
            ProfScope ps(e, s, PC_QKV, conv_flops(p, e->qkv[i], N));
            if (!(e->skip_mask >> PC_QKV & 1)) HIPCHK(e, gemm(e, 1, EPI_QKV, a, s));
        }
        if (cap) {
            capture(e, bn + "q", p.q16, rowsC, true, s); capture(e, bn + "k", p.k16, rowsC, true, s);
            capture(e, bn + "vt", p.vt16, (int64_t)N * C * p.Tp, true, s);
        }
        {
            AttnArgs a; memset(&a, 0, sizeof(a));
            a.q = p.q16; a.k = p.k16; a.vt = p.vt16; a.out = p.ao16; a.kbias = p.kbias; a.mask_mod = p.B; a.zeros = e->zeros;
            a.kv_end = p.kv_end; a.n_full = p.n_full; a.T = T; a.Tp = p.Tp; a.H = e->H; a.n_items = N;
            a.small_max_blocks = e->conc == 1 ? e->attn_small_blocks : 0;
            if (split_qk) { a.q_lo = p.q16lo; a.k_lo = p.k16lo; }
            if (dec_fast_paths) a.lse_max = e->lse_cells;
            if (ragged) a.t_lim = p.t_lim;
            ProfScope ps(e, s, PC_ATTN, 4.0 * (double)N * e->H * (double)T * T * (C / e->H));
            if (!(e->skip_mask >> PC_ATTN & 1)) HIPCHK(e, launch_attention(e->dt, a, s));
        }
        if (cap) capture(e, bn + "attn", p.ao16, rowsC, true, s);
        const bool fused = dec_fast_paths && e->fused_ffn && !cap && (int)e->ffn_stream.size() == L && e->ffn_stream[i] &&
                           (int64_t)e->conc * N * ((T + kFfnFusedFrames - 1) / kFfnFusedFrames) >= e->big_min_blocks;
        void* h2buf = fused ? p.h2_16 : p.h16;
        {
            ConvGemmArgs a = base_args(e, p, e->oproj[i], N);
            a.a0 = p.ao16; a.c0 = C; a.mask = mask; a.gate = ada_i + 2 * C; a.gate_stride = 6 * C; a.out32 = p.X;
            a.ln_h16 = h2buf; a.ln_film = nullptr; a.ln_film_mod = 1;
            a.ln_ada = ada_i; a.ln_ada_stride = 6 * C; a.ln_shift_off = 3 * C; a.ln_scale_off = 4 * C; a.ln_mask_out = 1;
            if (dec_fast_paths && (int)e->oproj_frag.size() == L && !cap) a.w_frag = e->oproj_frag[i];
            ProfScope ps(e, s, PC_OPROJ, conv_flops(p, e->oproj[i], N));
            if (!(e->skip_mask >> PC_OPROJ & 1)) HIPCHK(e, gemm(e, 1, EPI_RESGATE, a, s));
        }
        if (cap) { capture(e, bn + "x2", p.X, rowsC, false, s); capture(e, bn + "h2", p.h16, rowsC, true, s); }
        if (!fused) {
            ConvGemmArgs a = base_args(e, p, e->ffn1[i], N);
            a.a0 = p.h16; a.c0 = C; a.mask = mask; a.flags = GF_SILU | GF_MASK; a.out16 = p.u16;
            ProfScope ps(e, s, PC_FFN1, conv_flops(p, e->ffn1[i], N));
            HIPCHK(e, gemm(e, 3, EPI_ACT16, a, s));
        }
        if (cap) capture(e, bn + "u", p.u16, (int64_t)N * T * F, true, s);
        void* copy16 = (skips && i + 1 < L / 2) ? p.skip16[i + 1] : p.cur16;
        {
            ConvGemmArgs a = base_args(e, p, e->ffn2[i], N);
            a.a0 = p.u16; a.c0 = F; a.mask = mask; a.gate = ada_i + 5 * C; a.gate_stride = 6 * C; a.out32 = p.X;
            if (fused) { a.a0 = h2buf; a.c0 = C; a.w = e->ffn_stream[i]; a.bias1 = e->ffn1[i].bias; a.cmid = F; a.flags = GF_SILU | GF_MASK; }
            a.out16 = copy16;
            if (i + 1 == L) a.out16_lo = p.cur16lo;
            if (i + 1 < ln1_by_ffn) fuse_ln1(a, i + 1);
            else if (dec_fast_paths && !cap) a.out32_readonly = 1;
            ProfScope ps(e, s, PC_FFN2, conv_flops(p, e->ffn2[i], N) + (fused ? conv_flops(p, e->ffn1[i], N) : 0.0));
            if (e->skip_mask >> PC_FFN2 & 1) {}
            else if (fused && e->fused_ffn == 3) HIPCHK(e, launch_ffn_wino_f16(a, s));
            else if (fused) HIPCHK(e, e->dt == DT_BF16 ? launch_ffn_fused_bf16(a, s) : launch_ffn_fused_f16(a, s));
            else HIPCHK(e, gemm(e, 3, EPI_RESGATE, a, s));
        }
        if (cap) {
            if (film && i + 1 < ln1_by_ffn) capture(e, bn + "x3", copy16, rowsC, true, s);
            else capture(e, bn + "x3", p.X, rowsC, false, s);
        }
    }
    {
        ConvGemmArgs a = base_args(e, p, e->fin, N);
        a.a0 = p.cur16; a.c0 = C; a.a1 = p.cur16lo; a.c1 = C; a.c2 = C; a.mask = mask; a.flags = GF_MASK; a.out32 = p.v32;
        ProfScope ps(e, s, PC_FINAL, conv_flops(p, e->fin, N));
        HIPCHK(e, gemm(e, 1, EPI_F32, a, s));
    }
    if (cap) capture(e, "v", p.v32, (int64_t)N * T * e->Mp, false, s);
    return ST_OK;
}

int check_handle(st_engine* e, Kind kind) {
    if (!e) return ST_ERR_INVALID;
    if (e->kind != kind)
        return e->fail(ST_ERR_STATE, std::string("this handle is not a ") + kKinds[kind].what + " (" + kKinds[kind].creator + ")");
    return ST_OK;
}

int check_finalized(st_engine* e) {
    return e->finalized ? ST_OK : e->fail(ST_ERR_STATE, "st_finalize() has not been called after loading parameters");
}

int check_sizes(st_engine* e, int B, int T, const char* t_name) {
    return B >= 1 && T >= 1 ? ST_OK : e->fail(ST_ERR_INVALID, std::string("B and ") + t_name + " must be >= 1");
}

int check_dropout(st_engine* e, float p_dropout) {
    return p_dropout >= 0.0f && p_dropout < 1.0f ? ST_OK : e->fail(ST_ERR_INVALID, "p_dropout must be in [0, 1)");
}

int check_ready(st_engine* e, int B, int T) {
    if (!e) return ST_ERR_INVALID;
    int rc = check_finalized(e); if (rc) return rc;
    if ((rc = check_sizes(e, B, T))) return rc;
    if ((int64_t)2 * B * T * e->F >= (int64_t)1 << 31) return e->fail(ST_ERR_INVALID, "B*T too large for 32-bit row indexing");
    return ST_OK;
}

int new_handle(Kind kind, int device, st_engine** out) {
    int ndev = 0;
    if (hipGetDeviceCount(&ndev) != hipSuccess || device < 0 || device >= ndev) { g_create_error = "no such HIP device"; return ST_ERR_HIP; }
    if (hipSetDevice(device) != hipSuccess) { g_create_error = "hipSetDevice failed"; return ST_ERR_HIP; }
    st_engine* e = new st_engine();
    e->device = device; e->kind = kind;
    *out = e;
    return ST_OK;
}

static int find_param(st_engine* e, const char* name, const float* data, const int64_t* shape, int ndim, Param** out) {
    if (!e) return ST_ERR_INVALID;
    if (!name || !data || !shape) return e->fail(ST_ERR_INVALID, "null argument");
    auto it = e->params.find(name);
    if (it == e->params.end()) return e->fail(ST_ERR_INVALID, std::string("unexpected parameter name: ") + name);
    Param& p = it->second;
    bool ok = (int)p.shape.size() == ndim;
    for (int i = 0; ok && i < ndim; ++i) ok = p.shape[i] == shape[i];
    if (!ok) return e->fail(ST_ERR_INVALID, std::string("shape mismatch for ") + name);
    *out = &p;
    return ST_OK;
}

}

extern "C" {

int st_abi_version(void) { return ST_ABI_VERSION; }

static int create_engine(const st_config* cfg, Kind kind, int n_vocab, int device, st_engine** out) {
    if (!cfg || !out) { g_create_error = "null argument"; return ST_ERR_INVALID; }
    auto bad = [&](const char* m) { g_create_error = m; return ST_ERR_INVALID; };
    if (kind == KIND_DECODER && (cfg->n_layers % 2 != 0 || cfg->n_layers < 2 || cfg->n_layers > 16))
        return bad("n_layers must be even (estimator.py:92) and in [2, 16]");
    if (kind == KIND_TEXT_ENCODER && (cfg->n_layers < 1 || cfg->n_layers > 16)) return bad("n_layers must be in [1, 16]");
    if (kind == KIND_TEXT_ENCODER && n_vocab < 1) return bad("n_vocab must be >= 1");
    if (cfg->hidden_channels % 2 != 0) return bad("SinusoidalPosEmb requires dim to be even (estimator.py:39)");
    if (cfg->n_heads < 1 || cfg->hidden_channels % cfg->n_heads != 0)
        return bad("channels % n_heads != 0 (diffusion_transformer.py:35)");
    if (cfg->hidden_channels != 256) { g_create_error = "native kernels are built for hidden_channels == 256"; return ST_ERR_UNSUPPORTED; }
    if (cfg->hidden_channels / cfg->n_heads != 64) { g_create_error = "native kernels are built for head_dim == 64"; return ST_ERR_UNSUPPORTED; }
    if (cfg->kernel_size != 3) { g_create_error = "native kernels are built for kernel_size == 3"; return ST_ERR_UNSUPPORTED; }
    if (cfg->filter_channels % 128 != 0 || cfg->filter_channels < 128) { g_create_error = "filter_channels must be a multiple of 128"; return ST_ERR_UNSUPPORTED; }
    if (cfg->noise_channels < 1 || cfg->noise_channels > 1024) return bad("noise_channels out of range");
    if (cfg->gin_channels < 4 || cfg->gin_channels % 4 != 0) return bad("gin_channels must be a positive multiple of 4");
    if (cfg->operand_dtype != ST_OPERAND_BF16 && cfg->operand_dtype != ST_OPERAND_F16) return bad("operand_dtype");
    st_engine* e = nullptr;
    if (int rc = new_handle(kind, device, &e)) return rc;
    e->cfg = *cfg;
    e->dt = cfg->operand_dtype == ST_OPERAND_BF16 ? DT_BF16 : DT_F16;
    e->M = cfg->noise_channels; e->Mp = (e->M + 127) / 128 * 128;
    e->C = cfg->hidden_channels; e->F = cfg->filter_channels; e->H = cfg->n_heads; e->L = cfg->n_layers;
    e->K = cfg->kernel_size; e->G = cfg->gin_channels;
    e->n_vocab = n_vocab;
    if (const char* mb = getenv("ST_BIG_MIN_BLOCKS")) e->big_min_blocks = atoi(mb);
    if (const char* v = getenv("ST_PHASED")) e->phased = atoi(v);
    if (const char* v = getenv("ST_FUSED_FFN")) e->fused_ffn = atoi(v);
    if (e->fused_ffn < 0 || e->fused_ffn > 3 || e->fused_ffn == 2) e->fused_ffn = 1;
    if (e->fused_ffn == 3 && e->dt != DT_F16) e->fused_ffn = 1;
    if (const char* v = getenv("ST_RAGGED_SKIP")) e->ragged_skip = atoi(v);
#ifdef ST_DEVTOOLS
    if (const char* v = getenv("ST_SKIP_CLASSES")) e->skip_mask = (unsigned)strtoul(v, nullptr, 0);
#endif
    if (const char* v = getenv("ST_QKV_WS")) e->qkv_ws = atoi(v);
    if (const char* v = getenv("ST_QKV_WS_MIN_TILES")) e->qkv_ws_min_tiles = atoi(v);
    if (const char* v = getenv("ST_OPROJ_WS")) e->oproj_ws = atoi(v);
    if (const char* v = getenv("ST_OPROJ_WS_MIN_TILES")) e->oproj_ws_min_tiles = atoi(v);
    if (const char* v = getenv("ST_QKV_RC1")) e->qkv_rc1 = atoi(v);
    if (const char* v = getenv("ST_SMALL_GRID")) {
        if (atoi(v) == 0) {
            e->splitk_target = 0; e->small_tiles = 0; e->attn_small_blocks = 0;
        }
    }
    build_param_table(e);
    if (hipMalloc((void**)&e->kpart, kSplitKBytes) == hipSuccess) e->kpart_bytes = kSplitKBytes; else e->kpart = nullptr;
    if (hipMalloc(&e->sink, 65536) != hipSuccess) e->sink = nullptr;
    if (hipMalloc((void**)&e->lse_cells, kLseCells * 64) != hipSuccess ||
        hipMemsetD32((hipDeviceptr_t)e->lse_cells, (int)0x80000000, kLseCells * 16) != hipSuccess) { (void)hipGetLastError(); e->lse_cells = nullptr; }
    if (hipMalloc(&e->zeros, 256) != hipSuccess || hipMemset(e->zeros, 0, 256) != hipSuccess) {
        g_create_error = "hipMalloc failed";
        if (e->kpart) hipFree(e->kpart);
        delete e;
        return ST_ERR_HIP;
    }
    if (hipHostMalloc((void**)&e->status_host, sizeof(int), hipHostMallocMapped) == hipSuccess &&
        hipHostGetDevicePointer((void**)&e->status_dev, e->status_host, 0) == hipSuccess) *e->status_host = 0;
    else { (void)hipGetLastError(); e->status_host = nullptr; e->status_dev = nullptr; }
    *out = e;
    return ST_OK;
}

int st_create(const st_config* cfg, int device, st_engine** out) { return create_engine(cfg, KIND_DECODER, 0, device, out); }

int st_create_text_encoder(const st_config* cfg, int n_vocab, int device, st_engine** out) {
    return create_engine(cfg, KIND_TEXT_ENCODER, n_vocab, device, out);
}

void st_destroy(st_engine* e) {
    if (!e) return;
    hipSetDevice(e->device);
    hipDeviceSynchronize();
    e->drop_graphs();
    train_destroy(e);
    vocos_destroy(e);
    style_destroy(e);
    duration_destroy(e);
    mel_destroy(e);
    period_disc_destroy(e);
    resolution_disc_destroy(e);
    ffgan_destroy(e);
    sd_train_destroy(e);
    if (e->gstream) hipStreamDestroy(e->gstream);
    e->part_streams.destroy();
    for (auto& kv : e->params) if (kv.second.dev && !kv.second.borrowed) hipFree(kv.second.dev);
    for (void* p : e->owned) hipFree(p);
    for (auto& kv : e->caps) if (kv.second.dev) hipFree(kv.second.dev);
    prof_collect(e);
    for (hipEvent_t ev : e->ev_pool) hipEventDestroy(ev);
    if (e->ws) hipFree(e->ws);
    if (e->adams_buf) hipFree(e->adams_buf);
    if (e->pk_fwd.dev) hipFree(e->pk_fwd.dev);
    if (e->pk_T.dev) hipFree(e->pk_T.dev);
    if (e->rope_cos) hipFree(e->rope_cos);
    if (e->rope_sin) hipFree(e->rope_sin);
// ... 327 lines not shown
    if (!duration || !mask || !cum_scratch || !path) return align_fail(ST_ERR_INVALID, "null tensor pointer");
    if (B < 1 || Tx < 1 || Ty < 1 || B > 65535 || Tx > 65535) return align_fail(ST_ERR_INVALID, "shape out of range");
    if (launch_cumsum_rows(duration, B, Tx, cum_scratch, (hipStream_t)stream) != hipSuccess ||
        launch_path(cum_scratch, mask, B, Tx, Ty, path, (hipStream_t)stream) != hipSuccess)
        return align_fail(ST_ERR_HIP, "generate_path kernel launch failed");
    return ST_OK;
}

int st_align(const float* cum, const float* x_mask, const int64_t* y_lengths, const float* mu_x, int B, int M, int Tx, int Ty,
             float* attn, float* mu_y, float* y_mask, void* stream) {
    if (!cum || !x_mask || !y_lengths || !mu_x || !mu_y) return align_fail(ST_ERR_INVALID, "null tensor pointer");
    if (B < 1 || M < 1 || Tx < 1 || Ty < 1 || B > 65535) return align_fail(ST_ERR_INVALID, "shape out of range");
    if (launch_align(cum, x_mask, (const long long*)y_lengths, mu_x, B, M, Tx, Ty, attn, mu_y, y_mask, (hipStream_t)stream) != hipSuccess)
        return align_fail(ST_ERR_HIP, "align kernel launch failed");
    return ST_OK;
}

int64_t st_maximum_path_workspace_bytes(int B, int Ty, int Tx) { return (int64_t)mas_workspace_bytes(B, Ty, Tx); }

int st_maximum_path(const float* neg_cent, const int32_t* t_y, const int32_t* t_x, int B, int Ty, int Tx, float* path,
                    int32_t* durations, void* workspace, void* stream) {
    if (!neg_cent || !t_y || !t_x || !path) return align_fail(ST_ERR_INVALID, "null tensor pointer");
    if (B < 1 || Ty < 1 || Tx < 1 || B > 65535) return align_fail(ST_ERR_INVALID, "shape out of range");
    if (Tx > kMasMaxTx) return align_fail(ST_ERR_UNSUPPORTED, "maximum_path supports Tx <= 4096 (one row per wave in registers)");
    if (mas_workspace_bytes(B, Ty, Tx) && !workspace)
        return align_fail(ST_ERR_INVALID, "this shape needs st_maximum_path_workspace_bytes() of workspace");
    if (launch_mas_path(neg_cent, t_y, t_x, B, Ty, Tx, path, durations, workspace, (hipStream_t)stream) != hipSuccess)
        return align_fail(ST_ERR_HIP, "maximum_path kernel launch failed");
    return ST_OK;
}

int st_mas_neg_cent(const float* mu_x, const float* y, int B, int D, int Tx, int Ty, float* neg_cent, void* stream) {
    if (!mu_x || !y || !neg_cent) return align_fail(ST_ERR_INVALID, "null tensor pointer");
    if (B < 1 || D < 1 || Tx < 1 || Ty < 1 || B > 65535 || (Ty + 63) / 64 > 65535) return align_fail(ST_ERR_INVALID, "shape out of range");
    if (launch_mas_neg_cent(mu_x, y, B, D, Tx, Ty, neg_cent, (hipStream_t)stream) != hipSuccess)
        return align_fail(ST_ERR_HIP, "neg_cent kernel launch failed");
    return ST_OK;
}

int st_align_train_scratch_floats(int B, int M, int Ty) {
    if (B < 1 || M < 1 || Ty < 1) return ST_ERR_INVALID;
    return align_train_scratch_floats(B, M, Ty);
}

static int align_train_shape(int B, int M, int Tx, int Ty) {
    if (B < 1 || M < 1 || Tx < 1 || Ty < 1 || B > 65535 || (M + kAlignTrainChannels - 1) / kAlignTrainChannels > 65535 ||
        align_train_scratch_floats(B, M, Ty) < 0)
        return align_fail(ST_ERR_INVALID, "shape out of range");
    if (Tx > kAlignTrainMaxTx) return align_fail(ST_ERR_UNSUPPORTED, "the alignment training kernels support Tx <= 4096 (one item's running sum in LDS)");
    return ST_OK;
}

int st_align_train_forward(const int32_t* durations, const float* x_mask, const float* y_mask, const float* mu_x, const float* y,
                           const float* fake_content, const float* keep, int B, int M, int Tx, int Ty, int32_t* frame_token,
                           float* mu_y, float* mu_y_masked, float* scratch, float* prior_loss, void* stream) {
    if (!durations || !x_mask || !y_mask || !mu_x || !y || !frame_token || !mu_y_masked || !scratch || !prior_loss)
        return align_fail(ST_ERR_INVALID, "null tensor pointer");
    if (int rc = align_train_shape(B, M, Tx, Ty)) return rc;
    if (launch_align_train_forward(durations, x_mask, y_mask, mu_x, y, fake_content, keep, B, M, Tx, Ty, frame_token, mu_y, mu_y_masked,
                                   scratch, prior_loss, (hipStream_t)stream) != hipSuccess)
        return align_fail(ST_ERR_HIP, "align_train_forward kernel launch failed");
    return ST_OK;
}

int st_align_train_backward(const int32_t* durations, const float* x_mask, const float* y_mask, const float* mu_x, const float* y,
                            const float* keep, const float* scratch, const float* grad_mu_y_masked, const float* grad_mu_y,
                            const float* grad_prior, int B, int M, int Tx, int Ty, float* grad_mu_x, float* grad_fake_content,
                            void* stream) {
    if (!durations || !x_mask || !mu_x || !grad_mu_x) return align_fail(ST_ERR_INVALID, "null tensor pointer");
    if (grad_prior && (!y || !y_mask || !scratch)) return align_fail(ST_ERR_INVALID, "grad_prior needs y, y_mask and the forward's scratch");
    if (int rc = align_train_shape(B, M, Tx, Ty)) return rc;
    if (launch_align_train_backward(durations, x_mask, y_mask, mu_x, y, keep, scratch, grad_mu_y_masked, grad_mu_y, grad_prior, B, M, Tx,
                                    Ty, grad_mu_x, grad_fake_content, (hipStream_t)stream) != hipSuccess)
        return align_fail(ST_ERR_HIP, "align_train_backward kernel launch failed");
    return ST_OK;
}

int st_duration_loss_scratch_floats(void) { return kDurLossScratchFloats; }

int st_duration_loss(const float* logw, const int32_t* durations, const float* x_mask, const int64_t* x_lengths, int B, int Tx,
                     float* logw_target, float* scratch, float* loss, void* stream) {
    if (!logw || !durations || !x_mask || !x_lengths || !scratch || !loss) return align_fail(ST_ERR_INVALID, "null tensor pointer");
    if (B < 1 || Tx < 1) return align_fail(ST_ERR_INVALID, "shape out of range");
    if (launch_duration_loss(logw, durations, x_mask, (const long long*)x_lengths, B, Tx, logw_target, scratch, loss, (hipStream_t)stream) != hipSuccess)
        return align_fail(ST_ERR_HIP, "duration_loss kernel launch failed");
    return ST_OK;
}

int st_duration_loss_backward(const float* logw, const int32_t* durations, const float* x_mask, const float* scratch,
                              const float* grad_loss, int B, int Tx, float* grad_logw, void* stream) {
    if (!logw || !durations || !x_mask || !scratch || !grad_loss || !grad_logw) return align_fail(ST_ERR_INVALID, "null tensor pointer");
    if (B < 1 || Tx < 1) return align_fail(ST_ERR_INVALID, "shape out of range");
    if (launch_duration_loss_bwd(logw, durations, x_mask, scratch, grad_loss, B, Tx, grad_logw, (hipStream_t)stream) != hipSuccess)
        return align_fail(ST_ERR_HIP, "duration_loss_bwd kernel launch failed");
    return ST_OK;
}

int st_output_status(st_engine* e, void* stream, int* nonfinite) {
    if (!e) return ST_ERR_INVALID;
    if (!nonfinite) return e->fail(ST_ERR_INVALID, "null argument");
    if (!e->status_host) return e->fail(ST_ERR_UNSUPPORTED, "host-mapped status word unavailable on this device");
    HIPCHK(e, hipSetDevice(e->device));
    HIPCHK(e, hipStreamSynchronize((hipStream_t)stream));
    *nonfinite = *e->status_host != 0;
    e->arena_poisoned();
    return ST_OK;
}

int st_cfm_loss_prep(const float* x1, const float* z, const float* t_rand, float sigma_min, int B, int M, int T, float* t, float* y,
                     float* u, void* stream) {
    if (!x1 || !z || !t_rand || !t || !y || !u) return align_fail(ST_ERR_INVALID, "null tensor pointer");
    if (B < 1 || M < 1 || T < 1 || B > 65535) return align_fail(ST_ERR_INVALID, "shape out of range");
    if (launch_cfm_loss_prep(x1, z, t_rand, sigma_min, B, M, T, t, y, u, (hipStream_t)stream) != hipSuccess)
        return align_fail(ST_ERR_HIP, "cfm_loss_prep kernel launch failed");
    return ST_OK;
}

int st_cfm_loss(const float* pred, const float* u, const float* mask, int B, int M, int T, float* scratch, float* loss, void* stream) {
    if (!pred || !u || !mask || !scratch || !loss) return align_fail(ST_ERR_INVALID, "null tensor pointer");
    if (B < 1 || M < 1 || T < 1) return align_fail(ST_ERR_INVALID, "shape out of range");
    if (launch_cfm_loss(pred, u, mask, B, M, T, scratch, loss, (hipStream_t)stream) != hipSuccess)
        return align_fail(ST_ERR_HIP, "cfm_loss kernel launch failed");
    return ST_OK;
}

int st_cfm_loss_backward(const float* pred, const float* u, const float* scratch, const float* grad_loss, int B, int M, int T,
                         float* grad_pred, void* stream) {
    if (!pred || !u || !scratch || !grad_loss || !grad_pred) return align_fail(ST_ERR_INVALID, "null tensor pointer");
    if (B < 1 || M < 1 || T < 1) return align_fail(ST_ERR_INVALID, "shape out of range");
    if (launch_cfm_loss_bwd(pred, u, scratch, grad_loss, B, M, T, grad_pred, (hipStream_t)stream) != hipSuccess)
        return align_fail(ST_ERR_HIP, "cfm_loss_bwd kernel launch failed");
    return ST_OK;
}

int st_cfm_loss_scratch_floats(void) { return 2 * kCfmLossBlocks + 2; }

int st_last_solve_stats(const st_engine* e, int64_t* nfe, int64_t* steps, int64_t* rejects) {
    if (!e) return ST_ERR_INVALID;
    if (nfe) *nfe = e->last_nfe;
    if (steps) *steps = e->last_steps;
    if (rejects) *rejects = e->last_rejects;
    return ST_OK;
}

int st_set_option(st_engine* e, const char* name, int value) {
    if (!e || !name) return ST_ERR_INVALID;
    const std::string n(name);
    if (n == "attention_precision") {
        if (value != 0 && value != 1) return e->fail(ST_ERR_INVALID, "attention_precision: 0 (16-bit q / k operands) or 1 (split hi + lo operands)");
        if (e->kind != KIND_DECODER) return e->fail(ST_ERR_UNSUPPORTED, "attention_precision: CFM decoder handles only");
        if (value != e->attn_split) { e->drop_graphs(); e->attn_split = value; }
        return ST_OK;
    }
    if (n == "fused_ffn") return e->fail(ST_ERR_INVALID, "fused_ffn is read-only (ST_FUSED_FFN at st_create)");
    return e->fail(ST_ERR_INVALID, std::string("unknown option: ") + name);
}

int st_get_option(const st_engine* e, const char* name, int* value) {
    if (!e || !name || !value) return ST_ERR_INVALID;
    const std::string n(name);
    if (n == "attention_precision") { *value = e->attn_split; return ST_OK; }
    if (n == "fused_ffn") { *value = e->fused_ffn; return ST_OK; }
    return ST_ERR_INVALID;
}

int st_attention_stats(st_engine* e, void* stream, float* max_lse) {
    if (!e || !max_lse) return ST_ERR_INVALID;
    if (!e->lse_cells) return e->fail(ST_ERR_STATE, "attention statistics unavailable (allocation failed at st_create)");
    HIPCHK(e, hipSetDevice(e->device));
    HIPCHK(e, hipStreamSynchronize((hipStream_t)stream));
    int cells[kLseCells * 16];
    HIPCHK(e, hipMemcpy(cells, e->lse_cells, sizeof(cells), hipMemcpyDeviceToHost));
    int best = (int)0x80000000;
    for (int c = 0; c < kLseCells; ++c) best = std::max(best, cells[c * 16]);
    HIPCHK(e, hipMemsetD32((hipDeviceptr_t)e->lse_cells, (int)0x80000000, kLseCells * 16));
    if (best == (int)0x80000000) { *max_lse = -INFINITY; return ST_OK; }
    const int bits = best >= 0 ? best : best ^ 0x7fffffff;
    float v; memcpy(&v, &bits, 4);
    *max_lse = v * 0.6931471805599453f;
    return ST_OK;
}

int st_debug_capture(st_engine* e, int enable) {
    if (!e) return ST_ERR_INVALID;
    e->capture = enable != 0;
    if (!enable) {
        hipSetDevice(e->device);
        hipDeviceSynchronize();
        for (auto& kv : e->caps) if (kv.second.dev) hipFree(kv.second.dev);
        e->caps.clear();
    }
    return ST_OK;
}

int64_t st_debug_fetch(st_engine* e, const char* name, float* host_out, int64_t capacity) {
    if (!e || !name) return ST_ERR_INVALID;
    auto it = e->caps.find(name);
    if (it == e->caps.end() || !it->second.dev) { e->err = std::string("no captured tensor named ") + name; return ST_ERR_INVALID; }
    Captured& c = it->second;
    if (!host_out) return c.n;
    if (capacity < c.n) { e->err = "capacity too small"; return ST_ERR_INVALID; }
    if (hipSetDevice(e->device) != hipSuccess || hipDeviceSynchronize() != hipSuccess) return ST_ERR_HIP;
    if (!c.is16) {
        if (hipMemcpy(host_out, c.dev, (size_t)c.n * 4, hipMemcpyDeviceToHost) != hipSuccess) return ST_ERR_HIP;
        return c.n;
    }
    float* tmp = nullptr;
    if (hipMalloc((void**)&tmp, (size_t)c.n * 4) != hipSuccess) return ST_ERR_HIP;
    hipError_t r = launch_cvt16_to_f32(e->dt, c.dev, tmp, c.n, nullptr);
    if (r == hipSuccess) r = hipMemcpy(host_out, tmp, (size_t)c.n * 4, hipMemcpyDeviceToHost);
    hipFree(tmp);
    return r == hipSuccess ? c.n : (int64_t)ST_ERR_HIP;
}

int st_profile_enable(st_engine* e, int enable) {
    if (!e) return ST_ERR_INVALID;
    hipSetDevice(e->device);
    prof_collect(e);
    e->prof = enable != 0;
    for (int i = 0; i < PC_COUNT; ++i) { e->prof_launches[i] = 0; e->prof_ms[i] = 0; e->prof_flops[i] = 0; }
    return ST_OK;
}

int st_profile_select(st_engine* e, uint64_t class_mask) {
    if (!e) return ST_ERR_INVALID;
    e->prof_mask = class_mask;
    return ST_OK;
}

int st_profile_stride(st_engine* e, int stride) {
    if (!e || stride < 1) return ST_ERR_INVALID;
    e->prof_stride = stride;
    for (int i = 0; i < PC_COUNT; ++i) e->prof_seen[i] = 0;
    return ST_OK;
}

int st_profile_num_classes(void) { return PC_COUNT; }

const char* st_profile_class_name(int cls) { return (cls >= 0 && cls < PC_COUNT) ? kProfNames[cls] : ""; }

int st_profile_read(st_engine* e, int cls, int64_t* launches, double* total_ms, double* flops_per_launch) {
    if (!e || cls < 0 || cls >= PC_COUNT) return ST_ERR_INVALID;
    hipSetDevice(e->device);
    prof_collect(e);
    if (launches) *launches = e->prof_launches[cls];
    if (total_ms) *total_ms = e->prof_ms[cls];
    if (flops_per_launch) *flops_per_launch = e->prof_flops[cls];
    e->prof_launches[cls] = 0; e->prof_ms[cls] = 0;
    return ST_OK;
}

int64_t st_device_bytes(const st_engine* e) {
    if (!e) return ST_ERR_INVALID;
    int64_t n = e->weight_bytes + (int64_t)e->ws_cap + train_bytes(e);
    if (e->sdt) n += (int64_t)(e->sdt->act_cap + e->sdt->scr_cap);
    for (auto& kv : e->params) if (kv.second.dev && !kv.second.borrowed) n += kv.second.numel() * 4;
    return n;
}

}
```

### stabletts_amd/csrc/engine_internal.h

```cpp
#pragma once
#include "../../include/stabletts_hip.h"
#include "launch.h"
#include "stream_fork.h"

#include <map>
#include <string>
#include <vector>

namespace sthost {

enum ProfClass {
    PC_PREP = 0, PC_PRENET, PC_INPROJ, PC_FILM_LN1, PC_QKV, PC_ATTN, PC_OPROJ, PC_LN2, PC_FFN1, PC_FFN2,
    PC_LSC, PC_FINAL, PC_ODE, PC_TRAIN_FWD, PC_TRAIN_BWD, PC_COUNT
};

struct Param {
    std::vector<int64_t> shape;
    float* dev = nullptr;
    bool loaded = false;
    bool borrowed = false;
    int64_t numel() const { int64_t n = 1; for (auto s : shape) n *= s; return n; }
};

struct Conv {
    void* w = nullptr;
    float* bias = nullptr;
    int cout = 0, cin = 0, taps = 0;
    bool split = false;
};

struct Captured { void* dev = nullptr; int64_t n = 0; bool is16 = false; };

struct ProfEvent { int cls; hipEvent_t a, b; double flops; };

inline size_t align_up(size_t v, size_t a) { return (v + a - 1) / a * a; }

struct FloatArena {
    size_t off = 0;
    size_t want(size_t n) { const size_t o = off; off += (n + 63) / 64 * 64; return o; }
};

enum Kind { KIND_DECODER = 0, KIND_TEXT_ENCODER, KIND_VOCODER, KIND_STYLE_ENCODER, KIND_DURATION_PREDICTOR, KIND_MEL_EXTRACTOR, KIND_PERIOD_DISC, KIND_RESOLUTION_DISC,
            KIND_FFGAN, KIND_COUNT };
struct KindName { const char* what; const char* creator; };
constexpr KindName kKinds[KIND_COUNT] = {
    {"CFM decoder", "st_create"},
    {"text encoder", "st_create_text_encoder"},
    {"vocoder", "st_create_vocoder"},
    {"style encoder", "st_create_style_encoder"},
    {"duration predictor", "st_create_duration_predictor"},
    {"mel extractor", "st_create_mel_extractor"},
    {"period discriminator", "st_create_period_discriminator"},
    {"resolution discriminator", "st_create_resolution_discriminator"},
    {"FireflyGAN vocoder", "st_create_ffgan"},
};
constexpr bool reads_params_in_place(Kind k) { return k == KIND_STYLE_ENCODER || k == KIND_DURATION_PREDICTOR; }

struct TrainState;
struct VocosState;
struct StyleState;
struct DurState;
struct MelState;
struct PdState;
struct RdState;
struct FfganState;

struct SdTrain {
    char* act = nullptr; size_t act_cap = 0;
    char* scr = nullptr; size_t scr_cap = 0;
    int64_t serial = 0;
    bool have = false;
    int B = 0, T = 0;
    float p = 0.0f; unsigned long long seed = 0;
    bool masked = false;
};
int sd_train_grow(st_engine* e, char** buf, size_t* cap, size_t bytes);
void sd_train_destroy(st_engine* e);
SdTrain* sd_train_begin(st_engine* e);
void sd_train_commit(SdTrain* st, int B, int T, float p_dropout, unsigned long long seed, bool masked);
int sd_train_check(st_engine* e, const char* entry, const char* t_name, int64_t serial, int B, int T);

}

constexpr int kMaxParts = 1 + sthost::StreamFork::kMaxChildren;
constexpr int kSplitKMax = 16;
constexpr size_t kSplitKBytes = 32u << 20;

struct st_engine {
    st_config cfg{};
    int device = 0;
    int dt = st::DT_BF16;
    int M = 0, Mp = 0, C = 0, F = 0, H = 0, L = 0, K = 0, G = 0;
    sthost::Kind kind = sthost::KIND_DECODER;
    int n_vocab = 0;
    std::string blk(int i) const {
        return kind == sthost::KIND_DECODER ? "blocks." + std::to_string(i) + ".block." : "encoder." + std::to_string(i) + ".";
    }
    std::map<std::string, sthost::Param> params;
    bool finalized = false;
    struct PackList { std::vector<st::PackJob> jobs; st::PackJob* dev = nullptr; unsigned nblocks = 0; bool ready = false; bool recording = false; };
    PackList pk_fwd, pk_T;
    bool packed_once = false;
    std::string err;
    int64_t weight_bytes = 0;

    std::vector<sthost::Conv> pre;
    sthost::Conv inx, inc, fin;
    std::vector<sthost::Conv> lsc, qkv, oproj, ffn1, ffn2;
    std::vector<void*> oproj_frag;
    std::vector<void*> qkv_frag;
    std::vector<void*> ffn_stream;
    std::vector<void*> owned;

    float* rope_cos = nullptr; float* rope_sin = nullptr; int rope_T = 0;
    void* sink = nullptr;
    void* zeros = nullptr;

    char* ws = nullptr; size_t ws_cap = 0;
    uint64_t ws_sig = 0;

    bool capture = false;
    std::map<std::string, sthost::Captured> caps;
    bool prof = false;
    uint64_t prof_mask = ~0ull;
    int prof_stride = 1;
    int64_t prof_seen[sthost::PC_COUNT] = {0};
    std::vector<sthost::ProfEvent> evs;
    std::vector<hipEvent_t> ev_pool;
    int64_t prof_launches[sthost::PC_COUNT] = {0};
    double prof_ms[sthost::PC_COUNT] = {0};
    double prof_flops[sthost::PC_COUNT] = {0};

    int64_t last_nfe = 0, last_steps = 0, last_rejects = 0;
    int* status_host = nullptr; int* status_dev = nullptr;
    bool arena_poisoned() { if (status_host && *status_host) { *status_host = 0; ws_sig = 0; return true; } return false; }

    void* adams_buf = nullptr; size_t adams_bytes = 0;
    int big_min_blocks = 192;
    unsigned skip_mask = 0;
    int qkv_ws_min_tiles = 400;
    int qkv_ws = 1;
    int oproj_ws = 1;
    int oproj_ws_min_tiles = 1000;
    int qkv_rc1 = 1;
    int ragged_skip = 1;
    int fused_ffn = -1;
    int phased = 1;
    int splitk_max = kSplitKMax, splitk_min_stages = 4;
    int small_tiles = 256;
    int splitk_target = 256;
    int attn_split = 0;
    unsigned* lse_cells = nullptr;
    int attn_small_blocks = 32;
    float* kpart = nullptr;
    size_t kpart_bytes = 0;
    int conc = 1;
    sthost::StreamFork part_streams;

    struct SolveGraph {
        int B, T, n_steps, solver, use_cfg; float cfg_strength; const char* ws; int parts; int seen; hipGraphExec_t exec;
    };
    std::vector<SolveGraph> graphs;
    hipStream_t gstream = nullptr;
    void drop_graphs() {
        for (auto& g : graphs) if (g.exec) hipGraphExecDestroy(g.exec);
        graphs.clear();
    }

    sthost::TrainState* train = nullptr;
    sthost::VocosState* voc = nullptr;
    sthost::StyleState* sty = nullptr;
    sthost::SdTrain* sdt = nullptr;
    sthost::DurState* dur = nullptr;
    sthost::MelState* mel = nullptr;
    sthost::PdState* pd = nullptr;
    sthost::RdState* rd = nullptr;
    sthost::FfganState* ffg = nullptr;

    int fail(int code, const std::string& msg) { err = msg; return code; }
};


namespace sthost {

#define HIPCHK(e, call)                                                                         \
    do {                                                                                        \
        hipError_t _err = (call);                                                               \
        if (_err != hipSuccess)                                                                 \
            return (e)->fail(ST_ERR_HIP, std::string(#call) + ": " + hipGetErrorString(_err));  \
    } while (0)

int dev_alloc(st_engine* e, void** p, size_t bytes);
const float* P(st_engine* e, const std::string& name);
hipError_t gemm(st_engine* e, int taps, int epi, const st::ConvGemmArgs& a, hipStream_t s);
bool gemm_is_phased(const st_engine* e, int taps, const st::ConvGemmArgs& a);
void prof_collect(st_engine* e);
void capture(st_engine* e, const std::string& name, const void* dev, int64_t n, bool is16, hipStream_t s);
int ensure_ws(st_engine* e, size_t bytes);
int arena_fresh(st_engine* e, uint64_t sig, size_t used_bytes, hipStream_t s);
int ensure_rope(st_engine* e, int T, hipStream_t s);
int check_handle(st_engine* e, Kind kind);
int check_finalized(st_engine* e);
int check_sizes(st_engine* e, int B, int T, const char* t_name = "T");
int check_dropout(st_engine* e, float p_dropout);
int check_ready(st_engine* e, int B, int T);
extern std::string g_create_error;
int new_handle(Kind kind, int device, st_engine** out);
void expect(st_engine* e, const std::string& name, std::vector<int64_t> shape);
int vocos_finalize(st_engine* e);
int pack_all(st_engine* e, hipStream_t s);
bool pk_replay(st_engine* e, st_engine::PackList& L, hipStream_t s, int* rc);
void pk_begin(st_engine::PackList& L);
int pk_end(st_engine* e, st_engine::PackList& L, hipStream_t s);
void pk_drop(st_engine* e);
int pk_weight(st_engine* e, st_engine::PackList& L, const float* src, int cout, int cin_total, int K, int ci_off, int ci_cnt, void* dst,
              int row_off, int cin_p, int col_off, int slice_w, int lo, hipStream_t s);
int pk_weight_t(st_engine* e, st_engine::PackList& L, const float* src, int cout, int cin_total, int taps, int ci_off, int ci_cnt, void* dst,
                int cin_p, int ld, int col_off, hipStream_t s);
int pk_copy(st_engine* e, st_engine::PackList& L, float* dst, const float* src, int n, hipStream_t s);
void vocos_destroy(st_engine* e);
void style_destroy(st_engine* e);
void duration_destroy(st_engine* e);
int mel_finalize(st_engine* e);
void mel_destroy(st_engine* e);
int period_disc_weights(st_engine* e, hipStream_t s);
void period_disc_destroy(st_engine* e);
int resolution_disc_weights(st_engine* e, hipStream_t s);
void resolution_disc_destroy(st_engine* e);
int ffgan_finalize(st_engine* e);
void ffgan_destroy(st_engine* e);

struct ProfScope {
    st_engine* e; hipStream_t s; int idx = -1;
    ProfScope(st_engine* e_, hipStream_t s_, int cls, double flops);
    ~ProfScope();
};

struct Plan {
    int B, T, Tp, N, Pn, n_t;
    bool cfg;
    void *mu16, *pre1, *pre2, *cond16, *cond16lo, *x16, *x16lo, *h16, *h2_16, *q16, *k16, *q16lo, *k16lo, *vt16, *ao16, *u16, *cur16, *cur16lo;
    void* skip16[8];
    float *cpart, *X, *v32, *xstate, *kbuf[7], *ynew, *ode_partial, *ode_out, *tvals, *emb, *th, *tau, *film, *cvec, *ada, *ada_tmp;
    int *n_full, *kv_end;
    int* t_lim;
    float* kbias;
    float* maskbuf;
    struct Slot { void** dst; size_t off; };
    std::vector<Slot> slots;
};
size_t layout_plan(st_engine* e, int B, int T, bool cfg, int n_t, size_t off, Plan* p);
void bind_plan(st_engine* e, Plan* p);
uint64_t layout_sig(int entry, int B, int T, int cfg, int n_t, int parts);
int run_prenet(st_engine* e, const Plan& p, hipStream_t s);
int run_adaln(st_engine* e, const Plan& p, hipStream_t s);
int run_time_tables(st_engine* e, const Plan& p, hipStream_t s);
int run_estimator(st_engine* e, const Plan& p, const float* mask, int ev, hipStream_t s);

int train_prepare(st_engine* e, hipStream_t s);
void train_invalidate(st_engine* e);
void train_destroy(st_engine* e);
int64_t train_bytes(const st_engine* e);
int64_t train_grad_layout(const st_engine* e, std::map<std::string, int64_t>* offs);

}
```

### stabletts_amd/csrc/engine_solve.cpp

```cpp
#include "engine_internal.h"

#include <algorithm>
#include <cmath>
#include <cstring>
#include <deque>
#include <string>
#include <vector>

using namespace st;

namespace sthost {
namespace {

constexpr int kPartPhaseUs = 100;
constexpr int kDefaultSplit = -1;

std::vector<float> linspace01(int n) {
    const int steps = n + 1;
    std::vector<float> t(steps);
    const float step = (1.0f - 0.0f) / (float)(steps - 1);
    const int half = steps / 2;
    for (int i = 0; i < steps; ++i) t[i] = i < half ? 0.0f + step * (float)i : 1.0f - step * (float)(steps - i - 1);
    return t;
}
// ... 122 lines not shown
                for (int j = 0; j < 7; ++j) { ks[j] = k[0]; cm[j] = 0.f; }
                for (int j = 0; j < S; ++j) { ks[j] = k[j]; cm[j] = (float)(tb.cmid[j] * dt); }
                ks[6] = k[S]; cm[6] = (float)(tb.cmid[S] * dt);
                ProfScope ps(e, s, PC_ODE, 0);
                HIPCHK(e, launch_dopri5_interp(y, y1, ks, cm, (float)dt, (float)((t_end - t) / (t1 - t)), nstate, p.ynew, s));
                return ST_OK;
            }
            std::swap(y, y1);
            std::swap(k[0], k[S]);
            t = t1;
        } else {
            e->last_rejects += 1;
        }
        dt = dt_next;
        if (!(dt > 0.0) || dt < 1e-12) return e->fail(ST_ERR_INVALID, std::string(tb.name) + ": step size underflow");
    }
    return e->fail(ST_ERR_INVALID, std::string(tb.name) + ": too many steps");
}

static void adams_weights(int order, bool implicit, double* w) {
    std::vector<long double> nodes((size_t)order);
    for (int i = 0; i < order; ++i) nodes[(size_t)i] = implicit ? (i == 0 ? 1.0L : -(long double)(i - 1)) : -(long double)i;
    for (int j = 0; j < order; ++j) {
        std::vector<long double> poly(1, 1.0L);
        long double den = 1.0L;
        for (int i = 0; i < order; ++i) {
            if (i == j) continue;
            poly.insert(poly.begin(), 0.0L);
            for (size_t k = 0; k + 1 < poly.size(); ++k) poly[k] -= nodes[(size_t)i] * poly[k + 1];
            den *= nodes[(size_t)j] - nodes[(size_t)i];
        }
        long double integ = 0.0L;
        for (size_t k = 0; k < poly.size(); ++k) integ += poly[k] / (long double)(k + 1);
        w[j] = (double)(integ / den);
    }
}

int solve_implicit_adams(st_engine* e, const Plan& p, const float* mask, int use_cfg, float cfg_strength, int n_steps,
                         hipStream_t s) {
    constexpr int kMaxHist = 11, kMaxIters = 4, kExtra = 11;
    const double rtol = 1e-5, atol = 1e-5;
    const int64_t nstate = (int64_t)p.B * p.T * e->Mp;
    const size_t sbytes = (size_t)nstate * 4;
    int rc;
    if (e->adams_bytes < sbytes * kExtra) {
        if (e->adams_buf) { HIPCHK(e, hipStreamSynchronize(s)); hipFree(e->adams_buf); e->adams_buf = nullptr; e->adams_bytes = 0; }
        HIPCHK(e, hipMalloc(&e->adams_buf, sbytes * kExtra));
        e->adams_bytes = sbytes * kExtra;
    }
    std::vector<float*> pool;
    for (int j = 0; j < 7; ++j) pool.push_back(p.kbuf[j]);
    pool.push_back(p.ynew);
    for (int j = 0; j < kExtra; ++j) pool.push_back((float*)((char*)e->adams_buf + (size_t)j * sbytes));
    float* zero = pool.back(); pool.pop_back();
    float* dyA = pool.back(); pool.pop_back();
    float* dyB = pool.back(); pool.pop_back();
    float* delta = pool.back(); pool.pop_back();
    float* tmp[3]; for (int j = 0; j < 3; ++j) { tmp[j] = pool.back(); pool.pop_back(); }
    HIPCHK(e, hipMemsetAsync(zero, 0, sbytes, s));
    std::deque<float*> hist;
    auto eval = [&](float t, float* kout) { return eval_rhs(e, p, mask, use_cfg, cfg_strength, t, kout, s); };
    auto combine = [&](const float* base, const std::vector<const float*>& ks, const std::vector<float>& cf, float* out32, bool operands) -> int {
        size_t done = 0;
        const float* cur = base;
        do {
            const int nk = (int)std::min<size_t>(7, ks.size() - done);
            const bool last = done + (size_t)nk == ks.size();
            ProfScope ps(e, s, PC_ODE, 0);
            HIPCHK(e, launch_lincomb(e->dt, cur, ks.data() + done, cf.data() + done, nk, nstate, out32,
                                     last && operands ? p.x16 : nullptr, last && operands ? p.x16lo : nullptr, s));
            cur = out32; done += (size_t)nk;
        } while (done < ks.size());
        return ST_OK;
    };
    float* y = p.xstate;
    const std::vector<float> grid = linspace01(n_steps);
    float host2[2];
    for (int i = 0; i < n_steps; ++i) {
        const float t0 = grid[(size_t)i], t1 = grid[(size_t)i + 1], dt = t1 - t0;
        if ((int)hist.size() == kMaxHist) { pool.push_back(hist.back()); hist.pop_back(); }
        float* f0 = pool.back(); pool.pop_back();
        if ((rc = eval(t0, f0))) return rc;
        hist.push_front(f0);
        const int order = (int)hist.size();
        if (order < 3) {
            if ((rc = combine(y, {f0}, {dt / 3.0f}, nullptr, true))) return rc;
            if ((rc = eval(t0 + dt / 3.0f, tmp[0]))) return rc;
            if ((rc = combine(y, {tmp[0], f0}, {dt, -dt / 3.0f}, nullptr, true))) return rc;
            if ((rc = eval(t0 + dt * 2.0f / 3.0f, tmp[1]))) return rc;
            if ((rc = combine(y, {f0, tmp[0], tmp[1]}, {dt, -dt, dt}, nullptr, true))) return rc;
            if ((rc = eval(t1, tmp[2]))) return rc;
            if ((rc = combine(y, {f0, tmp[0], tmp[1], tmp[2]}, {dt * 0.125f, dt * 0.375f, dt * 0.375f, dt * 0.125f}, y, true))) return rc;
            continue;
        }
        double wb[12], wm[13];
        adams_weights(order, false, wb);
        adams_weights(order + 1, true, wm);
        std::vector<const float*> hs(hist.begin(), hist.end());
        std::vector<float> cb((size_t)order), cm((size_t)order);
        for (int j = 0; j < order; ++j) { cb[(size_t)j] = (float)((double)dt * wb[j]); cm[(size_t)j] = (float)((double)dt * wm[j + 1]); }
        float* dy = dyA; float* dyn = dyB;
        if ((rc = combine(zero, hs, cb, dy, false))) return rc;
        if ((rc = combine(zero, hs, cm, delta, false))) return rc;
        bool converged = false;
        for (int it = 0; it < kMaxIters && !converged; ++it) {
            if ((rc = combine(y, {dy}, {1.0f}, nullptr, true))) return rc;
            if ((rc = eval(t1, tmp[0]))) return rc;
            if ((rc = combine(delta, {tmp[0]}, {(float)((double)dt * wm[0])}, dyn, false))) return rc;
            OdeNormArgs na; memset(&na, 0, sizeof(na));
            na.mode = 3; na.y = dy; na.a = dy; na.b = dyn; na.rtol = (float)rtol; na.atol = (float)atol; na.n = nstate;
            na.partial = p.ode_partial; na.out = p.ode_out;
            HIPCHK(e, launch_ode_norm(na, s));
            HIPCHK(e, hipMemcpyAsync(host2, p.ode_out, 8, hipMemcpyDeviceToHost, s));
            HIPCHK(e, hipStreamSynchronize(s));
            converged = host2[0] == 0.0f;
            std::swap(dy, dyn);
        }
        if (!converged) { pool.push_back(hist.back()); hist.pop_back(); e->last_rejects += 1; }
        if ((rc = combine(y, {dy}, {1.0f}, y, true))) return rc;
    }
    return ST_OK;
}

struct Part { Plan p; int b0, nb; hipStream_t s; const float* mask; };

struct Solve {
    int B, T, n_steps, solver, use_cfg; float cfg_strength;
    bool adams, adaptive;
    int64_t per_item, bct;
    std::vector<Part> parts;
    std::vector<float> dts;
};

int solve_part_count(const st_engine* e, int B, int T, int use_cfg, bool adaptive) {
    int nparts = 1;
    const char* sv = getenv("ST_SPLIT");
    const int want = sv ? atoi(sv) : kDefaultSplit;
    const int64_t frames = (int64_t)(use_cfg ? 2 : 1) * B * T;
    if (!adaptive && !e->capture && B >= 2 && (want >= 2 || (want != 0 && want != 1 && frames >= 24000 && B >= 8))) nparts = 2;
    if (!adaptive && !e->capture && want != 0 && want != 1 && want != 2 && frames >= 48000 && B >= 32 && !(e->qkv_ws && e->sink)) nparts = 4;
    if (want > 2 && B >= want) nparts = std::min(want, kMaxParts);
    if (want == 1 || want == 0) nparts = 1;
    return nparts;
}

int boundary_in(st_engine* e, Solve& sv, const float* mu, const float* mask, const float* z, const float* c, const float* fake_speaker,
                const float* fake_content, const std::vector<float>& tv, hipStream_t s) {
    const int T = sv.T;
    for (auto& pt : sv.parts) {
        const Plan& p = pt.p;
        ProfScope ps(e, s, PC_PREP, 0);
        HIPCHK(e, launch_set_values(p.tvals, tv.data(), (int)tv.size(), s));
        HIPCHK(e, launch_mask_prep(mask + (int64_t)pt.b0 * T, pt.nb, T, p.Tp, p.n_full, p.kv_end, p.kbias, p.t_lim, s));
        HIPCHK(e, hipMemsetAsync(p.v32, 0, (size_t)p.N * T * e->Mp * 4, s));
        HIPCHK(e, launch_cvec_prep(mask + (int64_t)pt.b0 * T, nullptr, pt.nb, T, p.maskbuf, s));
        pt.mask = p.maskbuf;
        HIPCHK(e, launch_to_time_major(e->dt, mu + pt.b0 * sv.bct, pt.nb, e->M, T, e->Mp, nullptr, p.mu16, nullptr, s));
        HIPCHK(e, launch_to_time_major(e->dt, z + pt.b0 * sv.bct, pt.nb, e->M, T, e->Mp, p.xstate, p.x16, p.x16lo, s));
        HIPCHK(e, launch_cvec_prep(c + (int64_t)pt.b0 * e->G, sv.use_cfg ? fake_speaker : nullptr, pt.nb, e->G, p.cvec, s));
        if (sv.use_cfg) {
            HIPCHK(e, launch_fill_rows16(e->dt, fake_content, e->M, e->Mp, T,
                                         (char*)p.mu16 + (size_t)pt.nb * sv.per_item * 2, s));
        }
    }
    return ST_OK;
}

int step_fixed(st_engine* e, const Solve& sv, const Part& pt, int i) {
    const Plan& p = pt.p;
    const hipStream_t s = pt.s;
    const int Bp = pt.nb, use_cfg = sv.use_cfg;
    const int64_t per_item = sv.per_item, nstate = (int64_t)Bp * per_item;
    const float cfg_strength = sv.cfg_strength, dt = sv.dts[i];
    int rc;
    if (sv.solver == ST_SOLVER_EULER) {
        if ((rc = run_estimator(e, p, pt.mask, i, s))) return rc;
        ProfScope ps(e, s, PC_ODE, 0);
        HIPCHK(e, launch_cfg_combine(e->dt, p.v32, Bp, per_item, use_cfg, cfg_strength, nullptr, p.xstate, p.x16, p.x16lo, dt, s));
    } else if (sv.solver == ST_SOLVER_MIDPOINT) {
        if ((rc = run_estimator(e, p, pt.mask, 2 * i, s))) return rc;
        {
            ProfScope ps(e, s, PC_ODE, 0);
            HIPCHK(e, launch_cfg_combine(e->dt, p.v32, Bp, per_item, use_cfg, cfg_strength, p.kbuf[0], nullptr, nullptr, nullptr, 0.f, s));
            const float* ks[1] = {p.kbuf[0]}; const float cf[1] = {0.5f * dt};
            HIPCHK(e, launch_lincomb(e->dt, p.xstate, ks, cf, 1, nstate, nullptr, p.x16, p.x16lo, s));
        }
        if ((rc = run_estimator(e, p, pt.mask, 2 * i + 1, s))) return rc;
        ProfScope ps(e, s, PC_ODE, 0);
        HIPCHK(e, launch_cfg_combine(e->dt, p.v32, Bp, per_item, use_cfg, cfg_strength, nullptr, p.xstate, p.x16, p.x16lo, dt, s));
    } else {
        for (int st = 0; st < 4; ++st) {
            if ((rc = run_estimator(e, p, pt.mask, 4 * i + st, s))) return rc;
            ProfScope ps(e, s, PC_ODE, 0);
            HIPCHK(e, launch_cfg_combine(e->dt, p.v32, Bp, per_item, use_cfg, cfg_strength, p.kbuf[st], nullptr, nullptr, nullptr, 0.f, s));
            if (st == 0) {
                const float* ks[1] = {p.kbuf[0]}; const float cf[1] = {dt / 3.0f};
                HIPCHK(e, launch_lincomb(e->dt, p.xstate, ks, cf, 1, nstate, nullptr, p.x16, p.x16lo, s));
            } else if (st == 1) {
                const float* ks[2] = {p.kbuf[1], p.kbuf[0]}; const float cf[2] = {dt, -dt / 3.0f};
                HIPCHK(e, launch_lincomb(e->dt, p.xstate, ks, cf, 2, nstate, nullptr, p.x16, p.x16lo, s));
            } else if (st == 2) {
                const float* ks[3] = {p.kbuf[0], p.kbuf[1], p.kbuf[2]}; const float cf[3] = {dt, -dt, dt};
                HIPCHK(e, launch_lincomb(e->dt, p.xstate, ks, cf, 3, nstate, nullptr, p.x16, p.x16lo, s));
            } else {
                const float* ks[4] = {p.kbuf[0], p.kbuf[1], p.kbuf[2], p.kbuf[3]};
                const float cf[4] = {dt * 0.125f, dt * 0.375f, dt * 0.375f, dt * 0.125f};
                HIPCHK(e, launch_lincomb(e->dt, p.xstate, ks, cf, 4, nstate, p.xstate, p.x16, p.x16lo, s));
            }
        }
    }
    return ST_OK;
}

int solve_body(st_engine* e, Solve& sv, hipStream_t cs) {
    StreamFork& f = e->part_streams;
    ForkGuard guard{f, cs};
    const int nparts = (int)sv.parts.size();
    int rc;
    e->conc = nparts;
    HIPCHK(e, f.fork(cs, nparts - 1));
    for (int k = 0; k < nparts; ++k) sv.parts[k].s = k == 0 ? cs : f.child[k - 1];
    for (auto& pt : sv.parts) {
        if ((rc = run_prenet(e, pt.p, pt.s))) return rc;
        if ((rc = run_adaln(e, pt.p, pt.s))) return rc;
        if (!sv.adaptive && (rc = run_time_tables(e, pt.p, pt.s))) return rc;
    }
    if (sv.adams) {
        if ((rc = solve_implicit_adams(e, sv.parts[0].p, sv.parts[0].mask, sv.use_cfg, sv.cfg_strength, sv.n_steps, cs))) return rc;
    } else if (sv.adaptive) {
        const RkTableau& tb = sv.solver == ST_SOLVER_BOSH3 ? kBosh3 : sv.solver == ST_SOLVER_FEHLBERG2 ? kFehlberg2
                            : sv.solver == ST_SOLVER_ADAPTIVE_HEUN ? kAdaptiveHeun : kDopri5;
        if ((rc = solve_adaptive(e, sv.parts[0].p, sv.parts[0].mask, sv.use_cfg, sv.cfg_strength, tb, cs))) return rc;
    } else {
        if (nparts == 2) HIPCHK(e, launch_delay(kPartPhaseUs, sv.parts[1].s));
        for (int i = 0; i < sv.n_steps; ++i)
            for (auto& pt : sv.parts)
                if ((rc = step_fixed(e, sv, pt, i))) return rc;
    }
    HIPCHK(e, f.join(cs));
    return ST_OK;
}

int solve_graph(st_engine* e, Solve& sv, hipStream_t s, bool* replayed) {
    const char* genv = getenv("ST_HIP_GRAPH");
    if (!(genv && atoi(genv) == 1 && !sv.adaptive && !e->prof && !e->capture)) return ST_OK;
    const int nparts = (int)sv.parts.size();
    st_engine::SolveGraph* g = nullptr;
    for (auto& q : e->graphs)
        if (q.B == sv.B && q.T == sv.T && q.n_steps == sv.n_steps && q.solver == sv.solver && q.use_cfg == (sv.use_cfg != 0) &&
            q.cfg_strength == sv.cfg_strength && q.ws == e->ws && q.parts == nparts) g = &q;
    if (!g) {
        if (e->graphs.size() >= 16) e->drop_graphs();
        e->graphs.push_back({sv.B, sv.T, sv.n_steps, sv.solver, sv.use_cfg != 0, sv.cfg_strength, e->ws, nparts, 0, nullptr});
        g = &e->graphs.back();
    }
    if (g->seen >= 1 && !g->exec) {
        if (!e->gstream) HIPCHK(e, hipStreamCreateWithFlags(&e->gstream, hipStreamNonBlocking));
        hipGraph_t graph = nullptr;
        HIPCHK(e, hipStreamBeginCapture(e->gstream, hipStreamCaptureModeRelaxed));
        const int brc = solve_body(e, sv, e->gstream);
        const hipError_t ec = hipStreamEndCapture(e->gstream, &graph);
        e->conc = 1;
        if (brc) { if (graph) hipGraphDestroy(graph); return brc; }
        if (ec != hipSuccess || !graph) return e->fail(ST_ERR_HIP, std::string("hipStreamEndCapture: ") + hipGetErrorString(ec));
        const hipError_t ei = hipGraphInstantiate(&g->exec, graph, nullptr, nullptr, 0);
        hipGraphDestroy(graph);
        if (ei != hipSuccess) { g->exec = nullptr; return e->fail(ST_ERR_HIP, std::string("hipGraphInstantiate: ") + hipGetErrorString(ei)); }
    }
    g->seen += 1;
    if (g->exec) { HIPCHK(e, hipGraphLaunch(g->exec, s)); *replayed = true; }
    return ST_OK;
}

}
}

using namespace sthost;

extern "C" int st_cfm_solve(st_engine* e, const float* mu, const float* mask, const float* z, const float* c,
                            int n_steps, int solver, int use_cfg, float cfg_strength,
                            const float* fake_speaker, const float* fake_content,
                            float* out, int B, int T, void* stream) {
    int rc = check_ready(e, B, T); if (rc) return rc;
    if ((rc = check_handle(e, KIND_DECODER))) return rc;
    if (!mu || !mask || !z || !c || !out) return e->fail(ST_ERR_INVALID, "null tensor pointer");
    if (n_steps < 1 || n_steps > 4096) return e->fail(ST_ERR_INVALID, "n_steps out of range");
    if (solver < ST_SOLVER_EULER || solver > ST_SOLVER_IMPLICIT_ADAMS)
        return e->fail(ST_ERR_UNSUPPORTED, "solver not implemented natively (euler, midpoint, rk4, dopri5, bosh3, "
                                           "fehlberg2, adaptive_heun, implicit_adams are)");
    if (use_cfg && (!fake_speaker || !fake_content)) return e->fail(ST_ERR_INVALID, "CFG needs fake_speaker and fake_content");
    HIPCHK(e, hipSetDevice(e->device));
    hipStream_t s = (hipStream_t)stream;
    const bool adams = solver == ST_SOLVER_IMPLICIT_ADAMS;
    const bool adaptive = solver >= ST_SOLVER_DOPRI5;
    const int stages = solver == ST_SOLVER_EULER ? 1 : (solver == ST_SOLVER_MIDPOINT ? 2 : 4);
    const int n_t = adaptive ? 1 : n_steps * stages;
    const int nparts = solve_part_count(e, B, T, use_cfg, adaptive);
    Solve sv{B, T, n_steps, solver, use_cfg, cfg_strength, adams, adaptive, (int64_t)T * e->Mp, (int64_t)e->M * T,
             std::vector<Part>((size_t)nparts), std::vector<float>((size_t)n_steps)};
    {
        size_t off = 0;
        for (int k = 0; k < nparts; ++k) {
            sv.parts[k].b0 = (int)((int64_t)B * k / nparts);
            sv.parts[k].nb = (int)((int64_t)B * (k + 1) / nparts) - sv.parts[k].b0;
            off = layout_plan(e, sv.parts[k].nb, T, use_cfg != 0, n_t, off, &sv.parts[k].p);
        }
        if ((rc = ensure_ws(e, off))) return rc;
        e->arena_poisoned();
        if ((rc = arena_fresh(e, layout_sig(2, B, T, use_cfg != 0, n_t, nparts), off, s))) return rc;
        for (auto& pt : sv.parts) bind_plan(e, &pt.p);
    }
    if ((rc = ensure_rope(e, T, s))) return rc;
    if (nparts > 1) HIPCHK(e, e->part_streams.ensure(nparts - 1, 1, 0));

    const std::vector<float> grid = linspace01(n_steps);
    std::vector<float> tv((size_t)n_t);
    for (int i = 0; i < n_steps && !adaptive; ++i) {
        const float t0 = grid[i], t1 = grid[i + 1], dt = t1 - t0;
        sv.dts[i] = dt;
        if (stages == 1) tv[i] = t0;
        else if (stages == 2) { tv[2 * i] = t0; tv[2 * i + 1] = t0 + 0.5f * dt; }
        else { tv[4 * i] = t0; tv[4 * i + 1] = t0 + dt / 3.0f; tv[4 * i + 2] = t0 + dt * 2.0f / 3.0f; tv[4 * i + 3] = t1; }
    }
    if ((rc = boundary_in(e, sv, mu, mask, z, c, fake_speaker, fake_content, tv, s))) return rc;
    e->last_nfe = adaptive ? 0 : (int64_t)n_t; e->last_steps = adaptive && !adams ? 0 : n_steps; e->last_rejects = 0;

    bool replayed = false;
    if ((rc = solve_graph(e, sv, s, &replayed))) return rc;
// ... 12 lines not shown
```

### stabletts_amd/csrc/launch.h

```cpp
#pragma once
#include <hip/hip_runtime.h>
#include <stdint.h>

namespace st {

enum { DT_BF16 = 0, DT_F16 = 1 };

enum { EPI_ACT16 = 0, EPI_F32 = 1, EPI_RESGATE = 2, EPI_QKV = 3,
       EPI_GELU16 = 4,
       EPI_SILU = 5 };
enum { GF_SILU = 1, GF_MASK = 2,
       GF_K2_V_ONLY = 4 };

struct ConvGemmArgs {
    const void* a0; const void* a1;
    int c0, c1;
    int c2;
    int a0_mod, a1_mod;
    const void* w;
    long long w_item_stride;
    const float* bias;
    int cout, T, n_items;
    int tiles_f, tiles_c;
    const float* mask; int mask_mod;
    int flags;
    void* out16; float* out32;
    int out32_readonly;
    void* out16_lo;
    const float* add32; int add_clamp;
    const float* gate; int gate_stride;
    const float* res32;
    float* branch32;
    void* q; void* k; void* vt;
    void* q_lo; void* k_lo;
    void* vt_lo;
    const float* rope_cos; const float* rope_sin;
    int Tp; float qscale; int n_heads;
    const void* zeros;
    const void* w_frag;
    void* sink;
    void* ln_h16;
    const float* ln_film; int ln_film_stride; int ln_film_mod;
    const float* ln_ada; int ln_ada_stride; int ln_shift_off; int ln_scale_off;
    int ln_mask_out;
    const int* t_lim; int t_lim_mod;
    void* act16; const void* dact16;
    unsigned long long drop_seed; unsigned drop_thresh16; float drop_scale;
    int ksplit;
    const float* bias1; int cmid;
    unsigned long long* dbg;
};

enum { G2_T128 = 0, G2_RC = 1, G2_K3PIPE = 2,
       G2_BIG = 3,
       G2_T64 = 4, G2_RC64 = 5,
       G2_PHASED = 6,
       G2_RC1 = 7 };
hipError_t launch_conv_gemm2_bf16(int cfg, int taps, int epi, const ConvGemmArgs& a, hipStream_t s);
hipError_t launch_conv_gemm2_f16(int cfg, int taps, int epi, const ConvGemmArgs& a, hipStream_t s);
hipError_t launch_splitk_finish_bf16(int epi, const ConvGemmArgs& a, const float* part, int S, hipStream_t s);
hipError_t launch_splitk_finish_f16(int epi, const ConvGemmArgs& a, const float* part, int S, hipStream_t s);
constexpr int kFfnFusedFrames = 126;
hipError_t launch_ffn_fused_bf16(const ConvGemmArgs& a, hipStream_t s);
hipError_t launch_ffn_fused_f16(const ConvGemmArgs& a, hipStream_t s);
hipError_t launch_pack_ffn_stream(int dtype, const float* src, int stage, int F, void* dst, hipStream_t s);
hipError_t launch_pack_ffn_wino(const float* src, int stage, int F, void* dst, hipStream_t s);
hipError_t launch_ffn_wino_f16(const ConvGemmArgs& a, hipStream_t s);
hipError_t launch_qkv_ws(int dtype, const ConvGemmArgs& a, hipStream_t s);
hipError_t launch_oproj_ws(int dtype, const ConvGemmArgs& a, hipStream_t s);
hipError_t launch_pack_qkv_frag(int dtype, const float* src, int plane, void* dst, hipStream_t s);
constexpr int kGemmFramesPerTile = 128;
constexpr int kGemmChannelsPerTile = 128;

struct DropCfg { unsigned long long seed; unsigned thresh16; float scale; const unsigned* rowh; const unsigned* colh; };
hipError_t launch_drop_tables(const DropCfg& d, int n_rows, int n_colpairs, unsigned* rowh, unsigned* colh, hipStream_t s);

struct AttnArgs {
    const void* q; const void* k; const void* vt; void* out;
    const void* q_lo; const void* k_lo;
    const void* vt_lo;
    unsigned* lse_max;
    const float* kbias; int mask_mod;
    const int* kv_end; const int* n_full;
    int T, Tp, H, n_items;
    const void* zeros;
    float* lse;
    DropCfg drop;
    const int* t_lim;
    int small_max_blocks;
};
constexpr int kLseCells = 16;
hipError_t launch_attention(int dtype, const AttnArgs& a, hipStream_t s);

struct FilmLnArgs {
    float* X;
    void* h16;
    const float* film; int film_stride; int film_mod;
    const float* ada; int ada_stride;
    int shift_off, scale_off;
    const float* mask; int mask_mod;
    int mask_out;
    int T, rows;
};
hipError_t launch_film_ln(int dtype, const FilmLnArgs& a, hipStream_t s);

hipError_t launch_time_embed(const float* t, int n_t, int dim, float* emb, hipStream_t s);
hipError_t launch_silu_rows(const float* in, int64_t n, float* out, hipStream_t s);
struct LinearJobs { const float* in[8]; const float* W[8]; const float* bias[8]; float* out[8]; int n; };
hipError_t launch_linear_multi(const LinearJobs& J, int n, int k, int o, int silu_in, int silu_out, hipStream_t s);
hipError_t launch_linear(const float* in, int n, int k, const float* W, const float* bias, int o,
                         float* out, int silu_in, int silu_out, hipStream_t s);
constexpr int kFrameHalo = 4;
hipError_t launch_mask_prep(const float* mask, int B, int T, int Tp, int* n_full, int* kv_end, float* kbias, int* t_lim, hipStream_t s);

hipError_t launch_to_time_major(int dtype, const float* in, int B, int C, int T, int Cp,
                                float* out32, void* out16, void* out16lo, hipStream_t s);
hipError_t launch_from_time_major(const float* in, int B, int C, int T, int Cp, float* out, hipStream_t s, int* nonfinite = nullptr);
hipError_t launch_embed_tokens(const long long* tokens, const long long* lengths, const float* emb, int n_vocab,
                               int C, float scale, int B, int T, float* X, float* mask_out, hipStream_t s);
hipError_t launch_set_values(float* dst, const float* host_vals, int n, hipStream_t s);
hipError_t launch_delay(int us, hipStream_t s);
hipError_t launch_cvec_prep(const float* c, const float* fake_or_null, int B, int G, float* dst, hipStream_t s);
hipError_t launch_fill_rows16(int dtype, const float* vec, int C, int Cp, int T, void* out16, hipStream_t s);

hipError_t launch_cfg_combine(int dtype, const float* v, int B, int64_t per_item, int use_cfg, float s,
                              float* kout, float* xio, void* x16, void* x16lo, float dt, hipStream_t stream);
hipError_t launch_lincomb(int dtype, const float* x, const float* const* k, const float* coef, int nk,
                          int64_t n, float* y32, void* y16, void* y16lo, hipStream_t s);

hipError_t launch_pack_weight(int dtype, const float* src, int cout, int cin_total, int K, int ci_off,
                              int ci_cnt, void* dst, int row_off, int cin_p, int col_off, int slice_w, int lo,
                              hipStream_t s);
hipError_t launch_cvt16_to_f32(int dtype, const void* src, float* dst, int64_t n, hipStream_t s);
struct PackJob { const float* src; void* dst; int kind, cout, cin_total, K, ci_off, ci_cnt, row_off, cin_p, col_off, slice_w, lo; unsigned blk0; };
hipError_t launch_pack_jobs(int dtype, const PackJob* jobs_dev, int njobs, unsigned nblocks, hipStream_t s);

constexpr int kCfmLossBlocks = 1024;
hipError_t launch_cfm_loss_prep(const float* x1, const float* z, const float* t_rand, float sigma_min, int B, int M, int T,
                                float* t_out, float* y, float* u, hipStream_t s);
hipError_t launch_cfm_loss(const float* pred, const float* u, const float* mask, int B, int M, int T, float* scratch, float* loss, hipStream_t s);
hipError_t launch_cfm_loss_bwd(const float* pred, const float* u, const float* scratch, const float* grad_loss, int B, int M, int T, float* gpred, hipStream_t s);

hipError_t launch_durations(const float* logw, const float* x_mask, float length_scale, int B, int Tx, float* w_ceil,
                            float* cum, long long* y_len, hipStream_t s);
hipError_t launch_cumsum_rows(const float* dur, int B, int Tx, float* cum, hipStream_t s);
hipError_t launch_path(const float* cum, const float* mask, int B, int Tx, int Ty, float* path, hipStream_t s);
hipError_t launch_align(const float* cum, const float* x_mask, const long long* y_len, const float* mu_x, int B, int M, int Tx,
                        int Ty, float* attn, float* mu_y, float* y_mask, hipStream_t s);

hipError_t launch_set_scalar(float* dst, float v, hipStream_t s);
struct OdeNormArgs { const float* y; const float* a; const float* b; const float* k[7]; float coef[7]; int nk;
                     float rtol, atol; int64_t n; int mode; float* partial; float* out; };
hipError_t launch_ode_norm(const OdeNormArgs& a, hipStream_t s);
constexpr int kOdeNormBlocks = 1024;
hipError_t launch_dopri5_interp(const float* y0, const float* y1, const float* const* k, const float* cmid_dt, float dt,
                                float x, int64_t n, float* out, hipStream_t s);

}
```

### stabletts_amd/csrc/misc_kernels.hip

```cpp
#include "common.h"
#include "launch.h"

namespace st {

template <class P>
__global__ __launch_bounds__(256) void film_ln_kernel(const FilmLnArgs a) {
    const int lane = threadIdx.x & 63, wave = threadIdx.x >> 6;
    for (int row = blockIdx.x * 4 + wave; row < a.rows; row += gridDim.x * 4) {
        const int n = row / a.T, t = row - n * a.T;
        const float m = a.mask ? a.mask[(size_t)(n % a.mask_mod) * a.T + t] : 1.0f;
        float4 x = *(const float4*)(a.X + (size_t)row * 256 + lane * 4);
        if (a.film) {
            const float* f = a.film + (size_t)(n % a.film_mod) * a.film_stride + lane * 4;
            const float4 ga = *(const float4*)f;
            const float4 be = *(const float4*)(f + 256);
            x.x = (ga.x * x.x + be.x) * m; x.y = (ga.y * x.y + be.y) * m;
            x.z = (ga.z * x.z + be.z) * m; x.w = (ga.w * x.w + be.w) * m;
            *(float4*)(a.X + (size_t)row * 256 + lane * 4) = x;
        }
        const float mean = wave_sum(x.x + x.y + x.z + x.w) * (1.0f / 256.0f);
        const float d0 = x.x - mean, d1 = x.y - mean, d2 = x.z - mean, d3 = x.w - mean;
        const float var = wave_sum(d0 * d0 + d1 * d1 + d2 * d2 + d3 * d3) * (1.0f / 256.0f);
        const float rstd = 1.0f / sqrtf(var + 1e-5f);
        const float* ad = a.ada + (size_t)n * a.ada_stride + lane * 4;
        const float4 sh = *(const float4*)(ad + a.shift_off);
        const float4 sc = *(const float4*)(ad + a.scale_off);
        float h0 = d0 * rstd * (1.0f + sc.x) + sh.x;
        float h1 = d1 * rstd * (1.0f + sc.y) + sh.y;
        float h2 = d2 * rstd * (1.0f + sc.z) + sh.z;
        float h3 = d3 * rstd * (1.0f + sc.w) + sh.w;
        if (a.mask_out) { h0 *= m; h1 *= m; h2 *= m; h3 *= m; }
        *(uint2*)((unsigned char*)a.h16 + ((size_t)row * 256 + lane * 4) * 2) = pack4<P>(h0, h1, h2, h3);
    }
}

hipError_t launch_film_ln(int dtype, const FilmLnArgs& a, hipStream_t s) {
    int grid = (a.rows + 3) / 4;
    if (grid > 256 * 16) grid = 256 * 16;
    if (grid < 1) grid = 1;
    if (dtype == DT_BF16) hipLaunchKernelGGL((film_ln_kernel<OpBF16>), dim3(grid), dim3(256), 0, s, a);
    else                  hipLaunchKernelGGL((film_ln_kernel<OpF16>), dim3(grid), dim3(256), 0, s, a);
    return hipGetLastError();
}

__global__ void time_embed_kernel(const float* t, int n_t, int dim, float* emb) {
    const int half = dim / 2;
    const int idx = blockIdx.x * blockDim.x + threadIdx.x;
    if (idx >= n_t * half) return;
    const int n = idx / half, i = idx - n * half;
    const float e = logf(10000.0f) / (float)(half - 1);
    const float f = expf((float)i * -e);
    const float arg = 1000.0f * t[n] * f;
    emb[(size_t)n * dim + i] = sinf(arg);
    emb[(size_t)n * dim + half + i] = cosf(arg);
}

hipError_t launch_time_embed(const float* t, int n_t, int dim, float* emb, hipStream_t s) {
    const int total = n_t * (dim / 2);
    hipLaunchKernelGGL(time_embed_kernel, dim3((total + 255) / 256), dim3(256), 0, s, t, n_t, dim, emb);
    return hipGetLastError();
}

__global__ __launch_bounds__(256) void linear_kernel(const float* in, int n, int k, const float* W, const float* bias,
                                                     int o, float* out, int silu_in, int silu_out) {
    const int lane = threadIdx.x & 63;
    const long long wid = (long long)blockIdx.x * 4 + (threadIdx.x >> 6);
    if (wid >= (long long)n * o) return;
    const int ni = (int)(wid / o), oi = (int)(wid - (long long)ni * o);
    const float* x = in + (size_t)ni * k;
    const float* w = W + (size_t)oi * k;
    float acc = 0.f;
    for (int i = lane * 4; i < k; i += 256) {
        float4 xv = *(const float4*)(x + i);
        const float4 wv = *(const float4*)(w + i);
        if (silu_in) { xv.x = silu_f(xv.x); xv.y = silu_f(xv.y); xv.z = silu_f(xv.z); xv.w = silu_f(xv.w); }
        acc += xv.x * wv.x + xv.y * wv.y + xv.z * wv.z + xv.w * wv.w;
    }
    acc = wave_sum(acc);
    if (lane == 0) {
        float v = acc + (bias ? bias[oi] : 0.f);
        if (silu_out) v = silu_f(v);
        out[(size_t)ni * o + oi] = v;
    }
}

__global__ __launch_bounds__(256) void silu_rows_kernel(const float* in, int64_t n, float* out) {
    const int64_t i = (int64_t)blockIdx.x * 256 + threadIdx.x;
    if (i < n) out[i] = silu_f(in[i]);
}
hipError_t launch_silu_rows(const float* in, int64_t n, float* out, hipStream_t s) {
    hipLaunchKernelGGL(silu_rows_kernel, dim3((unsigned)((n + 255) / 256)), dim3(256), 0, s, in, n, out);
    return hipGetLastError();
}

__global__ __launch_bounds__(256) void linear_multi_kernel(LinearJobs J, int n, int k, int o, int silu_in, int silu_out) {
    constexpr int NI = 32, OT = 16, KC = 256, XP = KC + 4;
    __shared__ __attribute__((aligned(16))) float xs[NI][XP];
    __shared__ __attribute__((aligned(16))) float ws[OT][KC];
    const int tid = threadIdx.x;
    const int set = blockIdx.y, o0 = blockIdx.x * OT, n0 = blockIdx.z * NI;
    const float* X = J.in[set];
    const float* W = J.W[set];
    const int ni = tid & 31, op = tid >> 5;
    float acc0 = 0.f, acc1 = 0.f;
    for (int k0 = 0; k0 < k; k0 += KC) {
        const int kc = min(KC, k - k0);
#pragma unroll
        for (int i = 0; i < NI * KC / 4 / 256; ++i) {
            const int idx = tid + 256 * i, r = idx / (KC / 4), c = (idx % (KC / 4)) * 4;
            float4 v = make_float4(0.f, 0.f, 0.f, 0.f);
            if (n0 + r < n && c < kc) {
                v = *(const float4*)(X + (size_t)(n0 + r) * k + k0 + c);
                if (silu_in) { v.x = silu_f(v.x); v.y = silu_f(v.y); v.z = silu_f(v.z); v.w = silu_f(v.w); }
            }
            *(float4*)&xs[r][c] = v;
        }
#pragma unroll
        for (int i = 0; i < OT * KC / 4 / 256; ++i) {
            const int idx = tid + 256 * i, r = idx / (KC / 4), c = (idx % (KC / 4)) * 4;
            float4 v = make_float4(0.f, 0.f, 0.f, 0.f);
            if (o0 + r < o && c < kc) v = *(const float4*)(W + (size_t)(o0 + r) * k + k0 + c);
            *(float4*)&ws[r][c] = v;
        }
        __syncthreads();
#pragma unroll 8
        for (int c = 0; c < KC; c += 4) {
            const float4 xv = *(const float4*)&xs[ni][c];
            const float4 w0 = *(const float4*)&ws[2 * op][c];
            const float4 w1 = *(const float4*)&ws[2 * op + 1][c];
            acc0 += xv.x * w0.x + xv.y * w0.y + xv.z * w0.z + xv.w * w0.w;
            acc1 += xv.x * w1.x + xv.y * w1.y + xv.z * w1.z + xv.w * w1.w;
        }
        __syncthreads();
    }
    if (n0 + ni < n) {
        const float* bias = J.bias[set];
#pragma unroll
        for (int j = 0; j < 2; ++j) {
            const int oi = o0 + 2 * op + j;
            if (oi < o) {
                float v = (j ? acc1 : acc0) + (bias ? bias[oi] : 0.f);
                if (silu_out) v = silu_f(v);
                J.out[set][(size_t)(n0 + ni) * o + oi] = v;
            }
        }
    }
}
hipError_t launch_linear_multi(const LinearJobs& J, int n, int k, int o, int silu_in, int silu_out, hipStream_t s) {
    if (J.n < 1 || J.n > 8 || (k & 3) || n < 1 || o < 1) return hipErrorInvalidValue;
    hipLaunchKernelGGL(linear_multi_kernel, dim3((unsigned)((o + 15) / 16), J.n, (unsigned)((n + 31) / 32)), dim3(256), 0, s, J, n, k, o, silu_in, silu_out);
    return hipGetLastError();
}

hipError_t launch_linear(const float* in, int n, int k, const float* W, const float* bias, int o,
                         float* out, int silu_in, int silu_out, hipStream_t s) {
    const long long waves = (long long)n * o;
    const int grid = (int)((waves + 3) / 4);
    hipLaunchKernelGGL(linear_kernel, dim3(grid), dim3(256), 0, s, in, n, k, W, bias, o, out, silu_in, silu_out);
    return hipGetLastError();
}

__global__ __launch_bounds__(256) void mask_prep_kernel(const float* mask, int T, int Tp, int* n_full, int* kv_end,
                                                        float* kbias, int* t_lim) {
    __shared__ int s_first_zero, s_last_nz;
    const int b = blockIdx.x;
    if (threadIdx.x == 0) { s_first_zero = T; s_last_nz = -1; }
    __syncthreads();
    int fz = T, ln = -1;
    for (int t = threadIdx.x; t < Tp; t += blockDim.x) {
        const bool nz = (t < T) && (mask[(size_t)b * T + t] != 0.0f);
        kbias[(size_t)b * Tp + t] = nz ? 0.0f : -1e30f;
        if (t < T) {
            if (!nz && t < fz) fz = t;
            if (nz && t > ln) ln = t;
        }
    }
    atomicMin(&s_first_zero, fz);
    atomicMax(&s_last_nz, ln);
    __syncthreads();
    if (threadIdx.x == 0) {
        n_full[b] = s_first_zero; kv_end[b] = s_last_nz + 1;
        if (t_lim) {
            const int lim = min(T, s_last_nz + 1 + kFrameHalo);
            t_lim[b] = lim;
            atomicMax(&t_lim[gridDim.x], lim);
        }
    }
}

hipError_t launch_mask_prep(const float* mask, int B, int T, int Tp, int* n_full, int* kv_end, float* kbias, int* t_lim, hipStream_t s) {
    if (t_lim) { hipError_t e = hipMemsetAsync(t_lim + B, 0, sizeof(int), s); if (e != hipSuccess) return e; }
    hipLaunchKernelGGL(mask_prep_kernel, dim3(B), dim3(256), 0, s, mask, T, Tp, n_full, kv_end, kbias, t_lim);
    return hipGetLastError();
}

template <class P>
__global__ __launch_bounds__(256) void to_time_major_kernel(const float* in, int C, int T, int Cp,
                                                            float* out32, typename P::elem* out16, typename P::elem* out16lo) {
    __shared__ float tile[32][33];
    const int b = blockIdx.z, c0 = blockIdx.y * 32, t0 = blockIdx.x * 32;
    const int tx = threadIdx.x & 31, ty = threadIdx.x >> 5;
#pragma unroll
    for (int i = 0; i < 4; ++i) {
        const int c = c0 + ty + i * 8, t = t0 + tx;
        float v = 0.f;
        if (c < C && t < T) v = in[((size_t)b * C + c) * T + t];
        tile[ty + i * 8][tx] = v;
    }
    __syncthreads();
#pragma unroll
    for (int i = 0; i < 4; ++i) {
        const int t = t0 + ty + i * 8, c = c0 + tx;
        if (t < T && c < Cp) {
            const float v = tile[tx][ty + i * 8];
            const size_t o = ((size_t)b * T + t) * Cp + c;
            if (out32) out32[o] = v;
            if (out16) out16[o] = to16<P>(v);
            if (out16lo) out16lo[o] = to16<P>(v - (float)to16<P>(v));
        }
    }
}

hipError_t launch_to_time_major(int dtype, const float* in, int B, int C, int T, int Cp,
                                float* out32, void* out16, void* out16lo, hipStream_t s) {
    dim3 grid((T + 31) / 32, (Cp + 31) / 32, B);
    if (dtype == DT_BF16)
        hipLaunchKernelGGL((to_time_major_kernel<OpBF16>), grid, dim3(256), 0, s, in, C, T, Cp, out32, (__bf16*)out16, (__bf16*)out16lo);
    else
        hipLaunchKernelGGL((to_time_major_kernel<OpF16>), grid, dim3(256), 0, s, in, C, T, Cp, out32, (_Float16*)out16, (_Float16*)out16lo);
    return hipGetLastError();
}

__global__ __launch_bounds__(256) void from_time_major_kernel(const float* in, int C, int T, int Cp, float* out, int* nonfinite) {
    __shared__ float tile[32][33];
    const int b = blockIdx.z, c0 = blockIdx.y * 32, t0 = blockIdx.x * 32;
    const int tx = threadIdx.x & 31, ty = threadIdx.x >> 5;
#pragma unroll
    for (int i = 0; i < 4; ++i) {
        const int t = t0 + ty + i * 8, c = c0 + tx;
        float v = 0.f;
        if (t < T && c < Cp) v = in[((size_t)b * T + t) * Cp + c];
        tile[ty + i * 8][tx] = v;
    }
    __syncthreads();
#pragma unroll
    for (int i = 0; i < 4; ++i) {
        const int c = c0 + ty + i * 8, t = t0 + tx;
        if (c < C && t < T) {
            const float v = tile[tx][ty + i * 8];
            out[((size_t)b * C + c) * T + t] = v;
            if (nonfinite && !(fabsf(v) <= 3.4028234664e38f)) *nonfinite = 1;
        }
    }
}

hipError_t launch_from_time_major(const float* in, int B, int C, int T, int Cp, float* out, hipStream_t s, int* nonfinite) {
    dim3 grid((T + 31) / 32, (C + 31) / 32, B);
    hipLaunchKernelGGL(from_time_major_kernel, grid, dim3(256), 0, s, in, C, T, Cp, out, nonfinite);
    return hipGetLastError();
}

template <class P>
__global__ void fill_rows16_kernel(const float* vec, int C, int Cp, int T, typename P::elem* out) {
    const size_t idx = (size_t)blockIdx.x * blockDim.x + threadIdx.x;
    if (idx >= (size_t)T * Cp) return;
    const int c = (int)(idx % Cp);
    out[idx] = to16<P>(c < C ? vec[c] : 0.f);
}

hipError_t launch_fill_rows16(int dtype, const float* vec, int C, int Cp, int T, void* out16, hipStream_t s) {
    const size_t total = (size_t)T * Cp;
    const int grid = (int)((total + 255) / 256);
    if (dtype == DT_BF16) hipLaunchKernelGGL((fill_rows16_kernel<OpBF16>), dim3(grid), dim3(256), 0, s, vec, C, Cp, T, (__bf16*)out16);
    else                  hipLaunchKernelGGL((fill_rows16_kernel<OpF16>), dim3(grid), dim3(256), 0, s, vec, C, Cp, T, (_Float16*)out16);
    return hipGetLastError();
}

struct SetValuesArgs { float v[64]; };
__global__ void set_values_kernel(float* dst, int n, SetValuesArgs a) {
    const int i = threadIdx.x;
    if (i < n) dst[i] = a.v[i];
}
__global__ void delay_kernel(unsigned long long ticks, int max_iters) {
    const unsigned long long t0 = __builtin_amdgcn_s_memrealtime();
    for (int i = 0; i < max_iters && __builtin_amdgcn_s_memrealtime() - t0 < ticks; ++i) __builtin_amdgcn_s_sleep(16);
}
hipError_t launch_delay(int us, hipStream_t s) {
    static int khz[64] = {};
    int dev = 0;
    if (hipGetDevice(&dev) != hipSuccess || dev < 0 || dev >= 64) return hipErrorInvalidDevice;
    if (!khz[dev]) {
        int r = 0;
        if (hipDeviceGetAttribute(&r, hipDeviceAttributeWallClockRate, dev) != hipSuccess || r <= 0) { (void)hipGetLastError(); r = 100000; }
        khz[dev] = r;
    }
    hipLaunchKernelGGL(delay_kernel, dim3(1), dim3(64), 0, s, (unsigned long long)us * (unsigned long long)khz[dev] / 1000ull, 4 * us + 64);
    return hipGetLastError();
}

hipError_t launch_set_values(float* dst, const float* host_vals, int n, hipStream_t s) {
    for (int o = 0; o < n; o += 64) {
        SetValuesArgs a;
        const int m = n - o < 64 ? n - o : 64;
        for (int i = 0; i < 64; ++i) a.v[i] = i < m ? host_vals[o + i] : 0.f;
        hipLaunchKernelGGL(set_values_kernel, dim3(1), dim3(64), 0, s, dst + o, m, a);
    }
    return hipGetLastError();
}

__global__ void cvec_prep_kernel(const float* c, const float* fake, int B, int G, float* dst) {
    const int i = blockIdx.x * blockDim.x + threadIdx.x;
    const int n = B * G;
    if (i < n) dst[i] = c[i];
    else if (fake && i < 2 * n) dst[i] = fake[(i - n) % G];
}
hipError_t launch_cvec_prep(const float* c, const float* fake_or_null, int B, int G, float* dst, hipStream_t s) {
    const int total = (fake_or_null ? 2 : 1) * B * G;
    hipLaunchKernelGGL(cvec_prep_kernel, dim3((total + 255) / 256), dim3(256), 0, s, c, fake_or_null, B, G, dst);
    return hipGetLastError();
}

__global__ __launch_bounds__(256) void embed_tokens_kernel(const long long* tokens, const long long* lengths,
                                                           const float* emb, int n_vocab, int C, float scale, int B,
                                                           int T, float* X, float* mask_out) {
    const int row = blockIdx.x * 4 + (threadIdx.x >> 6);
    const int lane = threadIdx.x & 63;
    if (row >= B * T) return;
    const int b = row / T, t = row % T;
    const float m = (long long)t < lengths[b] ? 1.0f : 0.0f;
    long long tok = tokens[row];
    tok = tok < 0 ? 0 : (tok >= n_vocab ? n_vocab - 1 : tok);
    const float s = scale * m;
    for (int ch = lane * 4; ch < C; ch += 256) {
        const float4 v = *(const float4*)(emb + (size_t)tok * C + ch);
        *(float4*)(X + (size_t)row * C + ch) = make_float4(v.x * s, v.y * s, v.z * s, v.w * s);
    }
    if (lane == 0) mask_out[row] = m;
}
hipError_t launch_embed_tokens(const long long* tokens, const long long* lengths, const float* emb, int n_vocab,
                               int C, float scale, int B, int T, float* X, float* mask_out, hipStream_t s) {
    const int rows = B * T;
    hipLaunchKernelGGL(embed_tokens_kernel, dim3((rows + 3) / 4), dim3(256), 0, s, tokens, lengths, emb, n_vocab, C,
                       scale, B, T, X, mask_out);
    return hipGetLastError();
}

template <class P>
__device__ __forceinline__ uint2 pack4_lo(float a, float b, float c, float d) {
    return pack4<P>(a - (float)to16<P>(a), b - (float)to16<P>(b), c - (float)to16<P>(c), d - (float)to16<P>(d));
}

template <class P>
__global__ __launch_bounds__(256) void cfg_combine_kernel(const float* v, int64_t half, int use_cfg, float s,
                                                          float* kout, float* xio, typename P::elem* x16,
                                                          typename P::elem* x16lo, float dt) {
    const int64_t i = ((int64_t)blockIdx.x * blockDim.x + threadIdx.x) * 4;
    if (i >= half) return;
    float4 vc = *(const float4*)(v + i);
    if (use_cfg) {
        const float4 vu = *(const float4*)(v + half + i);
        vc.x = vu.x + s * (vc.x - vu.x); vc.y = vu.y + s * (vc.y - vu.y);
        vc.z = vu.z + s * (vc.z - vu.z); vc.w = vu.w + s * (vc.w - vu.w);
    }
    if (kout) *(float4*)(kout + i) = vc;
    if (xio) {
        float4 x = *(const float4*)(xio + i);
        x.x += dt * vc.x; x.y += dt * vc.y; x.z += dt * vc.z; x.w += dt * vc.w;
        *(float4*)(xio + i) = x;
        if (x16) *(uint2*)(x16 + i) = pack4<P>(x.x, x.y, x.z, x.w);
        if (x16lo) *(uint2*)(x16lo + i) = pack4_lo<P>(x.x, x.y, x.z, x.w);
    }
}

hipError_t launch_cfg_combine(int dtype, const float* v, int B, int64_t per_item, int use_cfg, float s,
                              float* kout, float* xio, void* x16, void* x16lo, float dt, hipStream_t stream) {
    const int64_t half = (int64_t)B * per_item;
    const int grid = (int)((half / 4 + 255) / 256);
    if (dtype == DT_BF16)
        hipLaunchKernelGGL((cfg_combine_kernel<OpBF16>), dim3(grid), dim3(256), 0, stream, v, half, use_cfg, s, kout, xio, (__bf16*)x16, (__bf16*)x16lo, dt);
    else
        hipLaunchKernelGGL((cfg_combine_kernel<OpF16>), dim3(grid), dim3(256), 0, stream, v, half, use_cfg, s, kout, xio, (_Float16*)x16, (_Float16*)x16lo, dt);
    return hipGetLastError();
}

constexpr int kMaxComb = 7;
struct LinCombArgs { const float* x; const float* k[kMaxComb]; float coef[kMaxComb]; int nk; int64_t n; float* y32; void* y16; void* y16lo; };

template <class P>
__global__ __launch_bounds__(256) void lincomb_kernel(const LinCombArgs a) {
    const int64_t i = ((int64_t)blockIdx.x * blockDim.x + threadIdx.x) * 4;
    if (i >= a.n) return;
    float4 y = *(const float4*)(a.x + i);
#pragma unroll
    for (int j = 0; j < kMaxComb; ++j) {
        if (j < a.nk) {
            const float4 kv = *(const float4*)(a.k[j] + i);
            const float c = a.coef[j];
            y.x += c * kv.x; y.y += c * kv.y; y.z += c * kv.z; y.w += c * kv.w;
        }
    }
    if (a.y32) *(float4*)(a.y32 + i) = y;
    if (a.y16) *(uint2*)((typename P::elem*)a.y16 + i) = pack4<P>(y.x, y.y, y.z, y.w);
    if (a.y16lo) *(uint2*)((typename P::elem*)a.y16lo + i) = pack4_lo<P>(y.x, y.y, y.z, y.w);
}

hipError_t launch_lincomb(int dtype, const float* x, const float* const* k, const float* coef, int nk,
                          int64_t n, float* y32, void* y16, void* y16lo, hipStream_t s) {
    LinCombArgs a;
    a.x = x; a.nk = nk; a.n = n; a.y32 = y32; a.y16 = y16; a.y16lo = y16lo;
    for (int j = 0; j < kMaxComb; ++j) { a.k[j] = j < nk ? k[j] : nullptr; a.coef[j] = j < nk ? coef[j] : 0.f; }
    const int grid = (int)((n / 4 + 255) / 256);
    if (dtype == DT_BF16) hipLaunchKernelGGL((lincomb_kernel<OpBF16>), dim3(grid), dim3(256), 0, s, a);
    else                  hipLaunchKernelGGL((lincomb_kernel<OpF16>), dim3(grid), dim3(256), 0, s, a);
    return hipGetLastError();
}

template <class P>
__global__ void pack_weight_kernel(const float* src, int cout, int cin_total, int K, int ci_off, int ci_cnt,
                                   typename P::elem* dst, int row_off, int cin_p, int col_off, int slice_w, int lo) {
    const size_t idx = (size_t)blockIdx.x * blockDim.x + threadIdx.x;
    const size_t total = (size_t)cout * K * slice_w;
    if (idx >= total) return;
    const int ci = (int)(idx % slice_w);
    const int j = (int)((idx / slice_w) % K);
    const int co = (int)(idx / ((size_t)slice_w * K));
    float v = 0.f;
    if (ci < ci_cnt) v = src[((size_t)co * cin_total + ci_off + ci) * K + j];
    if (lo) v -= (float)to16<P>(v);
    dst[((size_t)(row_off + co) * K + j) * cin_p + col_off + ci] = to16<P>(v);
}

hipError_t launch_pack_weight(int dtype, const float* src, int cout, int cin_total, int K, int ci_off,
                              int ci_cnt, void* dst, int row_off, int cin_p, int col_off, int slice_w, int lo,
                              hipStream_t s) {
    const size_t total = (size_t)cout * K * slice_w;
    const int grid = (int)((total + 255) / 256);
    if (dtype == DT_BF16)
        hipLaunchKernelGGL((pack_weight_kernel<OpBF16>), dim3(grid), dim3(256), 0, s, src, cout, cin_total, K, ci_off, ci_cnt, (__bf16*)dst, row_off, cin_p, col_off, slice_w, lo);
    else
        hipLaunchKernelGGL((pack_weight_kernel<OpF16>), dim3(grid), dim3(256), 0, s, src, cout, cin_total, K, ci_off, ci_cnt, (_Float16*)dst, row_off, cin_p, col_off, slice_w, lo);
    return hipGetLastError();
}

__global__ __launch_bounds__(256) void cfm_loss_prep_kernel(const float* x1, const float* z, const float* t_rand, float one_minus_sigma,
                                                            int B, int64_t per_item, float* t_out, float* y, float* u) {
    const int b = blockIdx.y;
    const float t = 1.0f - cosf(t_rand[b] * 0.5f * 3.14159265358979323846f);
    if (blockIdx.x == 0 && threadIdx.x == 0) t_out[b] = t;
    const float cz = 1.0f - one_minus_sigma * t;
    const int64_t base = (int64_t)b * per_item;
    const bool al16 = ((((uintptr_t)(x1 + base)) | ((uintptr_t)(z + base)) | ((uintptr_t)(y + base)) | ((uintptr_t)(u + base))) & 15) == 0;
    for (int64_t i = ((int64_t)blockIdx.x * blockDim.x + threadIdx.x) * 4; i < per_item; i += (int64_t)gridDim.x * blockDim.x * 4) {
        if (i + 4 <= per_item && al16) {
            const float4 a = *(const float4*)(x1 + base + i), n = *(const float4*)(z + base + i);
            *(float4*)(y + base + i) = make_float4(cz * n.x + t * a.x, cz * n.y + t * a.y, cz * n.z + t * a.z, cz * n.w + t * a.w);
            *(float4*)(u + base + i) = make_float4(a.x - one_minus_sigma * n.x, a.y - one_minus_sigma * n.y, a.z - one_minus_sigma * n.z, a.w - one_minus_sigma * n.w);
        } else {
            for (int64_t j = i; j < per_item && j < i + 4; ++j) {
                y[base + j] = cz * z[base + j] + t * x1[base + j];
                u[base + j] = x1[base + j] - one_minus_sigma * z[base + j];
            }
        }
    }
}
hipError_t launch_cfm_loss_prep(const float* x1, const float* z, const float* t_rand, float sigma_min, int B, int M, int T,
                                float* t_out, float* y, float* u, hipStream_t s) {
    const int64_t per_item = (int64_t)M * T;
    int gx = (int)((per_item / 4 + 255) / 256); if (gx > 256) gx = 256; if (gx < 1) gx = 1;
    hipLaunchKernelGGL(cfm_loss_prep_kernel, dim3(gx, B), dim3(256), 0, s, x1, z, t_rand, 1.0f - sigma_min, B, per_item, t_out, y, u);
    return hipGetLastError();
}

__global__ __launch_bounds__(256) void cfm_loss_partial_kernel(const float* pred, const float* u, const float* mask, int64_t n, int64_t nm, float* scratch) {
    __shared__ float red[2][4];
    float acc = 0.f, am = 0.f;
    for (int64_t i = (int64_t)blockIdx.x * blockDim.x + threadIdx.x; i < n; i += (int64_t)gridDim.x * blockDim.x) {
        const float d = pred[i] - u[i];
        acc += d * d;
    }
    for (int64_t i = (int64_t)blockIdx.x * blockDim.x + threadIdx.x; i < nm; i += (int64_t)gridDim.x * blockDim.x) am += mask[i];
    acc = wave_sum(acc); am = wave_sum(am);
    if ((threadIdx.x & 63) == 0) { red[0][threadIdx.x >> 6] = acc; red[1][threadIdx.x >> 6] = am; }
    __syncthreads();
    if (threadIdx.x == 0) {
        scratch[blockIdx.x] = (red[0][0] + red[0][1]) + (red[0][2] + red[0][3]);
        scratch[kCfmLossBlocks + blockIdx.x] = (red[1][0] + red[1][1]) + (red[1][2] + red[1][3]);
    }
}
__global__ __launch_bounds__(256) void cfm_loss_final_kernel(float* scratch, int nblocks, int M, float* loss) {
    __shared__ float red[2][4];
    float a = 0.f, m = 0.f;
    for (int i = threadIdx.x; i < nblocks; i += 256) { a += scratch[i]; m += scratch[kCfmLossBlocks + i]; }
    a = wave_sum(a); m = wave_sum(m);
    if ((threadIdx.x & 63) == 0) { red[0][threadIdx.x >> 6] = a; red[1][threadIdx.x >> 6] = m; }
    __syncthreads();
    if (threadIdx.x == 0) {
        const float ss = (red[0][0] + red[0][1]) + (red[0][2] + red[0][3]);
        const float den = ((red[1][0] + red[1][1]) + (red[1][2] + red[1][3])) * (float)M;
        scratch[2 * kCfmLossBlocks] = ss; scratch[2 * kCfmLossBlocks + 1] = den;
        *loss = ss / den;
    }
}
hipError_t launch_cfm_loss(const float* pred, const float* u, const float* mask, int B, int M, int T, float* scratch, float* loss, hipStream_t s) {
    const int64_t n = (int64_t)B * M * T, nm = (int64_t)B * T;
    int grid = (int)((n / 8 + 255) / 256); if (grid > kCfmLossBlocks) grid = kCfmLossBlocks; if (grid < 1) grid = 1;
    hipLaunchKernelGGL(cfm_loss_partial_kernel, dim3(grid), dim3(256), 0, s, pred, u, mask, n, nm, scratch);
    hipLaunchKernelGGL(cfm_loss_final_kernel, dim3(1), dim3(256), 0, s, scratch, grid, M, loss);
    return hipGetLastError();
}
__global__ __launch_bounds__(256) void cfm_loss_bwd_kernel(const float* pred, const float* u, const float* scratch, const float* grad_loss, int64_t n, float* gpred) {
    const float f = 2.0f * grad_loss[0] / scratch[2 * kCfmLossBlocks + 1];
    for (int64_t i = (int64_t)blockIdx.x * blockDim.x + threadIdx.x; i < n; i += (int64_t)gridDim.x * blockDim.x) gpred[i] = f * (pred[i] - u[i]);
}
hipError_t launch_cfm_loss_bwd(const float* pred, const float* u, const float* scratch, const float* grad_loss, int B, int M, int T, float* gpred, hipStream_t s) {
    const int64_t n = (int64_t)B * M * T;
    int grid = (int)((n / 4 + 255) / 256); if (grid > 2048) grid = 2048; if (grid < 1) grid = 1;
    hipLaunchKernelGGL(cfm_loss_bwd_kernel, dim3(grid), dim3(256), 0, s, pred, u, scratch, grad_loss, n, gpred);
    return hipGetLastError();
}

template <class P>
__global__ void pack_ffn_stream_kernel(const float* src, int stage, int F, typename P::elem* dst) {
    const size_t idx = (size_t)blockIdx.x * blockDim.x + threadIdx.x;
// ... 54 lines not shown
```

Baseline: 1.342 million.

## Fuse CFG combine and Euler update into final conv GEMM epilogue; batch adaLN linears

Adds a paired-tile GEMM epilogue in which each tile computes the conditional and unconditional final projections for the same frames side by side. The epilogue then mixes them with the CFG scale, applies the Euler step to the state, and writes the fp32, hi and lo 16-bit copies directly. This removes the separate cfg_combine launch, the v32 round trip and the per-chunk v32 memset. It also batches the per-layer adaLN and FiLM linears into one launch each, with blockIdx.y selecting the layer, instead of L sequential launches. The trade is a more constrained GEMM configuration: each tile covers half as many frames, which means more tiles, and the fused path applies only when its preconditions hold.

```diff
diff --git a/stabletts_amd/csrc/common.h b/stabletts_amd/csrc/common.h
--- a/stabletts_amd/csrc/common.h
+++ b/stabletts_amd/csrc/common.h
@@ -42,6 +42,21 @@
     v[0] = (typename P::elem)a; v[1] = (typename P::elem)b;
     v[2] = (typename P::elem)c; v[3] = (typename P::elem)d;
     return __builtin_bit_cast(uint2, v);
+}
+
+template <class P>
+__device__ __forceinline__ uint2 pack4_lo(float a, float b, float c, float d) {
+    return pack4<P>(a - (float)to16<P>(a), b - (float)to16<P>(b), c - (float)to16<P>(c), d - (float)to16<P>(d));
+}
+
+__device__ __forceinline__ float4 cfg_mix4(const float4& vc, const float4& vu, float s) {
+    return make_float4(vu.x + s * (vc.x - vu.x), vu.y + s * (vc.y - vu.y), vu.z + s * (vc.z - vu.z), vu.w + s * (vc.w - vu.w));
+}
+template <class P>
+__device__ __forceinline__ void euler_pack4(float4& x, const float4& v, float dt, uint2& hi, uint2& lo) {
+    x.x += dt * v.x; x.y += dt * v.y; x.z += dt * v.z; x.w += dt * v.w;
+    hi = pack4<P>(x.x, x.y, x.z, x.w);
+    lo = pack4_lo<P>(x.x, x.y, x.z, x.w);
 }
 
 template <class P>
diff --git a/stabletts_amd/csrc/conv_gemm2_impl.h b/stabletts_amd/csrc/conv_gemm2_impl.h
--- a/stabletts_amd/csrc/conv_gemm2_impl.h
+++ b/stabletts_amd/csrc/conv_gemm2_impl.h
@@ -203,6 +203,72 @@
     }, stage, g, n, t0, fvalid, cbase, wave, lane);
 }
 
+template <class P, int BC, int BF, int WC, int WF>
+__device__ __forceinline__ void g2_epilogue_cfg_euler(f32x16_t (&acc)[BC / WC / 32][BF / WF / 32], float* stage, const ConvGemmArgs& g,
+                                                      int n, int t0, int cbase, int wave, int lane) {
+    constexpr int NW = WC * WF, TC = BC / WC, TF = BF / WF, FC = TC / 32, FF = TF / 32, PITCH = BC + 4, HF = BF / 2;
+    static_assert(BC == 128 && NW == 4 && WF == 2, "one 32-lane half per 128-channel row, one wave column per CFG branch");
+    constexpr int RPW = HF / (2 * NW), RB = 4;
+    const int l31 = lane & 31, hi = lane >> 5, wc = wave % WC, wf = wave / WC;
+    const int T = g.T;
+#pragma unroll
+    for (int a = 0; a < FC; ++a)
+#pragma unroll
+        for (int b = 0; b < FF; ++b)
+#pragma unroll
+            for (int q4 = 0; q4 < 4; ++q4) {
+                const int fl = wf * TF + b * 32 + l31;
+                const int ch = wc * TC + a * 32 + 8 * q4 + 4 * hi;
+                *(float4*)(stage + fl * PITCH + ch) = make_float4(acc[a][b][4 * q4 + 0], acc[a][b][4 * q4 + 1],
+                                                                  acc[a][b][4 * q4 + 2], acc[a][b][4 * q4 + 3]);
+            }
+    const int chl = l31 * 4;
+    const float4 bias = g.bias ? *(const float4*)(g.bias + cbase + chl) : make_float4(0.f, 0.f, 0.f, 0.f);
+    const float* mrow = g.mask ? g.mask + (size_t)(n % g.mask_mod) * T : nullptr;
+    const bool msk = g.flags & GF_MASK;
+    const int tlim = g.t_lim ? min(T, g.t_lim[n % g.t_lim_mod]) : T;
+    const float s = g.cfg_scale, dt = g.euler_dt;
+    float mk[RPW]; float4 x[RPW]; int fr[RPW]; size_t off[RPW]; bool ok[RPW];
+#pragma unroll
+    for (int u = 0; u < RPW; ++u) {
+        const int f = (wave + u * NW) * 2 + hi;
+        const int t = t0 + f;
+        fr[u] = f;
+        ok[u] = t < tlim;
+        const int tl = ok[u] ? t : tlim - 1;
+        off[u] = ((size_t)n * T + tl) * g.cout + cbase + chl;
+        mk[u] = (msk && mrow) ? mrow[tl] : 1.0f;
+        x[u] = *(const float4*)(g.out32 + off[u]);
+    }
+    __syncthreads();
+#pragma unroll
+    for (int b0 = 0; b0 < RPW; b0 += RB) {
+        float4 vc[RB], vu[RB]; uint2 h16[RB], l16[RB];
+#pragma unroll
+        for (int u = 0; u < RB; ++u) {
+            vc[u] = *(const float4*)(stage + fr[b0 + u] * PITCH + chl);
+            vu[u] = *(const float4*)(stage + (fr[b0 + u] + HF) * PITCH + chl);
+        }
+#pragma unroll
+        for (int u = 0; u < RB; ++u) {
+            const float mm = mk[b0 + u], z = 0.f;
+            vc[u].x = (vc[u].x + bias.x + z) * mm; vc[u].y = (vc[u].y + bias.y + z) * mm;
+            vc[u].z = (vc[u].z + bias.z + z) * mm; vc[u].w = (vc[u].w + bias.w + z) * mm;
+            vu[u].x = (vu[u].x + bias.x + z) * mm; vu[u].y = (vu[u].y + bias.y + z) * mm;
+            vu[u].z = (vu[u].z + bias.z + z) * mm; vu[u].w = (vu[u].w + bias.w + z) * mm;
+        }
+#pragma unroll
+        for (int u = 0; u < RB; ++u) euler_pack4<P>(x[b0 + u], cfg_mix4(vc[u], vu[u], s), dt, h16[u], l16[u]);
+#pragma unroll
+        for (int u = 0; u < RB; ++u)
+            if (ok[b0 + u]) {
+                store_row16(g.out32 + off[b0 + u], x[b0 + u]);
+                store_row8((unsigned char*)g.out16 + off[b0 + u] * 2, h16[u]);
+                store_row8((unsigned char*)g.out16_lo + off[b0 + u] * 2, l16[u]);
+            }
+    }
+}
+
 template <int EPI, int FC, int FF>
 __device__ __forceinline__ void g2_init_acc(f32x16_t (&acc)[FC][FF], const ConvGemmArgs& g, int chw, int hi) {
 #pragma unroll
@@ -488,7 +554,10 @@
     const int wave = __builtin_amdgcn_readfirstlane(tid >> 6);
     const int l31 = lane & 31, hi = lane >> 5;
     const int wc = wave % WC, wf = wave / WC;
-    const int cbase = tc * BC, t0 = tf * BF;
+    constexpr bool PAIR = (EPI == EPI_CFG_EULER);
+    constexpr int BFT = PAIR ? BF / 2 : BF;
+    static_assert(!PAIR || (TAPS == 1 && WF == 2 && WBUF == 2), "paired tile: k = 1, one wave column per branch");
+    const int cbase = tc * BC, t0 = tf * BFT;
     if (g.t_lim && t0 >= g.t_lim[n % g.t_lim_mod]) return;
     const int cin = g.c0 + g.c1 + g.c2;
     const int nch_all = (EPI == EPI_QKV && (g.flags & GF_K2_V_ONLY) && cbase < 2 * BC ? g.c0 : cin) >> 6;
@@ -511,12 +580,17 @@
 #pragma unroll
     for (int k = 0; k <= APW; ++k) {
         const int row = (k < APW) ? (wave * APW + k) * 8 + prow : BF + prow;
-        const int t = t0 + row - (TAPS / 2);
+        const int t = PAIR ? t0 + (row & (BFT - 1)) : t0 + row - (TAPS / 2);
         const unsigned segb = (unsigned)(((lane & 7) ^ ((row >> 1) & 7)) << 4);
         const bool mine = (k < APW) || (TAPS == 3 && wave == 0 && lane < 16);
         validA[k] = mine && (t >= 0 && t < T);
         voffA0[k] = (unsigned)(t * g.c0 * 2) + segb;
         voffA1[k] = (unsigned)(t * g.c1 * 2) + segb;
+        if constexpr (PAIR) {
+            const unsigned item_rows = row >= BFT ? (unsigned)g.pair_items * (unsigned)T : 0u;
+            voffA0[k] += item_rows * (unsigned)(g.c0 * 2);
+            voffA1[k] += item_rows * (unsigned)(g.c1 * 2);
+        }
         if (mine && !(t >= 0 && t < T)) {
             const int pc = (k < APW) ? wave * APW + k : BF / 8;
             *(uint4*)(As + pc * 1024 + lane * 16) = make_uint4(0, 0, 0, 0);
@@ -637,6 +711,7 @@
     if constexpr (EPI == EPI_ACT16 || EPI == EPI_GELU16)
         g2_epilogue_act16<P, BC, BF, WC, WF, EPI == EPI_GELU16>(acc, smem, g, n, t0, BF, cbase, wave, lane);
     else if constexpr (EPI == EPI_QKV) g2_epilogue_qkv<P, BC, BF, WC, WF>(acc, smem, g, n, t0, cbase, wave, lane);
+    else if constexpr (EPI == EPI_CFG_EULER) g2_epilogue_cfg_euler<P, BC, BF, WC, WF>(acc, (float*)smem, g, n, t0, cbase, wave, lane);
     else g2_epilogue<P, EPI, BC, BF, WC, WF>(acc, (float*)smem, g, kz * g.n_items + n, t0, BF, cbase, wave, lane);
 #if ST_STAGE_TIMING
     if (g.dbg && lane == 0 && (wave == 0 || wave == NW - 1) && lin < 64) {
@@ -861,6 +936,12 @@
     ConvGemmArgs b = a;
     b.tiles_f = (a.T + BF - 1) / BF;
     b.tiles_c = a.cout / BC;
+    if (EPI == EPI_CFG_EULER) {
+        if (a.n_items != a.pair_items || a.pair_items < 1 || !a.out32 || !a.out16 || !a.out16_lo || a.ksplit > 1 || a.w_item_stride ||
+            a.a0_mod < 2 * a.pair_items || (a.c1 && a.a1_mod < 2 * a.pair_items))
+            return hipErrorInvalidValue;
+        b.tiles_f = (a.T + BF / 2 - 1) / (BF / 2);
+    }
     if (a.ksplit > 1) {
         if (EPI != EPI_F32 || a.bias || a.add32 || a.out16 || a.ln_h16 || (a.flags & GF_MASK) || !a.out32 ||
             a.ksplit > (a.c0 + a.c1 + a.c2) / 64 || a.w_item_stride)
diff --git a/stabletts_amd/csrc/conv_gemm2_inst.h b/stabletts_amd/csrc/conv_gemm2_inst.h
--- a/stabletts_amd/csrc/conv_gemm2_inst.h
+++ b/stabletts_amd/csrc/conv_gemm2_inst.h
@@ -40,6 +40,8 @@
         if (taps == 3 && epi == EPI_SILU) return launch_phased3<P, EPI_SILU>(a, s);
     } else if (cfg == 7) {
         if (taps == 1 && epi == EPI_QKV) return launch_g2<P, 1, EPI_QKV, 256, 128, 4, 2, 1>(a, s);
+    } else if (cfg == 8) {
+        if (taps == 1 && epi == EPI_CFG_EULER) return launch_g2<P, 1, EPI_CFG_EULER, 128, 128, 2, 2>(a, s);
     } else if (cfg == 2) {
         if (taps == 3 && epi == EPI_ACT16) return launch_g3<P, EPI_ACT16>(a, s);
         if (taps == 3 && epi == EPI_F32) return launch_g3<P, EPI_F32>(a, s);
diff --git a/stabletts_amd/csrc/engine.cpp b/stabletts_amd/csrc/engine.cpp
--- a/stabletts_amd/csrc/engine.cpp
+++ b/stabletts_amd/csrc/engine.cpp
@@ -213,7 +213,7 @@
     want((void**)&p->tau, (size_t)n_t * C * 4);
     want((void**)&p->film, (size_t)L * n_t * 2 * C * 4);
     want((void**)&p->cvec, N * (size_t)e->G * 4);
-    want((void**)&p->ada_tmp, N * (size_t)C * 4);
+    want((void**)&p->ada_tmp, (e->G != C ? (size_t)L : 1) * N * (size_t)C * 4);
     want((void**)&p->ada, (size_t)L * N * 6 * C * 4);
     want((void**)&p->n_full, (size_t)B * 4);
     want((void**)&p->kv_end, (size_t)B * 4);
@@ -329,10 +329,27 @@
 }
 
 int run_adaln(st_engine* e, const Plan& p, hipStream_t s) {
-    const int C = e->C;
+    const int C = e->C, L = e->L;
+    const size_t NC = (size_t)p.N * C;
     ProfScope ps(e, s, PC_PREP, 0);
-    if (e->G == C) HIPCHK(e, launch_silu_rows(p.cvec, (int64_t)p.N * C, p.ada_tmp, s));
-    for (int i = 0; i < e->L; ++i) {
+    if (e->G == C) HIPCHK(e, launch_silu_rows(p.cvec, (int64_t)NC, p.ada_tmp, s));
+    if (e->batched_linears) {
+        LinearBatch j0, j2; memset(&j0, 0, sizeof(j0)); memset(&j2, 0, sizeof(j2));
+        for (int i = 0; i < L; ++i) {
+            const std::string pre = e->blk(i) + "adaLN_modulation.";
+            if (e->G != C) { j0.W[i] = P(e, pre + "0.weight"); j0.bias[i] = P(e, pre + "0.bias"); }
+            j2.W[i] = P(e, pre + "2.weight"); j2.bias[i] = P(e, pre + "2.bias");
+        }
+        j0.n = j2.n = L;
+        if (e->G != C) {
+            HIPCHK(e, launch_linear_batch(p.cvec, 0, p.N, e->G, j0, C, p.ada_tmp, (long long)NC, 0, 0, s));
+            HIPCHK(e, launch_linear_batch(p.ada_tmp, (long long)NC, p.N, C, j2, 6 * C, p.ada, (long long)NC * 6, 1, 0, s));
+        } else {
+            HIPCHK(e, launch_linear_batch(p.ada_tmp, 0, p.N, C, j2, 6 * C, p.ada, (long long)NC * 6, 0, 0, s));
+        }
+        return ST_OK;
+    }
+    for (int i = 0; i < L; ++i) {
         const std::string pre = e->blk(i) + "adaLN_modulation.";
         if (e->G != C) {
             HIPCHK(e, launch_linear(p.cvec, p.N, e->G, P(e, pre + "0.weight"), P(e, pre + "0.bias"), C, p.ada_tmp, 0, 0, s));
@@ -347,12 +364,22 @@
 }
 
 int run_time_tables(st_engine* e, const Plan& p, hipStream_t s) {
-    const int C = e->C, F = e->F;
+    const int C = e->C, F = e->F, L = e->L;
     ProfScope ps(e, s, PC_PREP, 0);
     HIPCHK(e, launch_time_embed(p.tvals, p.n_t, C, p.emb, s));
     HIPCHK(e, launch_linear(p.emb, p.n_t, C, P(e, "time_mlp.layer.0.weight"), P(e, "time_mlp.layer.0.bias"), F, p.th, 0, 1, s));
     HIPCHK(e, launch_linear(p.th, p.n_t, F, P(e, "time_mlp.layer.2.weight"), P(e, "time_mlp.layer.2.bias"), C, p.tau, 0, 0, s));
-    for (int i = 0; i < e->L; ++i) {
+    if (e->batched_linears) {
+        LinearBatch j; memset(&j, 0, sizeof(j));
+        for (int i = 0; i < L; ++i) {
+            const std::string pre = "blocks." + std::to_string(i) + ".time_fusion.film.";
+            j.W[i] = P(e, pre + "weight"); j.bias[i] = P(e, pre + "bias");
+        }
+        j.n = L;
+        HIPCHK(e, launch_linear_batch(p.tau, 0, p.n_t, C, j, 2 * C, p.film, (long long)p.n_t * 2 * C, 0, 0, s));
+        return ST_OK;
+    }
+    for (int i = 0; i < L; ++i) {
         const std::string pre = "blocks." + std::to_string(i) + ".time_fusion.film.";
         HIPCHK(e, launch_linear(p.tau, p.n_t, C, P(e, pre + "weight"), P(e, pre + "bias"), 2 * C,
                                 p.film + (size_t)i * p.n_t * 2 * C, 0, 0, s));
@@ -360,7 +387,7 @@
     return ST_OK;
 }
 
-int run_estimator(st_engine* e, const Plan& p, const float* mask, int ev, hipStream_t s) {
+int run_estimator(st_engine* e, const Plan& p, const float* mask, int ev, hipStream_t s, const StepFuse* sf) {
     const int C = e->C, F = e->F, L = e->L, N = p.N, T = p.T;
     const int64_t rowsC = (int64_t)N * T * C;
     const bool cap = e->capture;
@@ -484,10 +511,22 @@
         ConvGemmArgs a = base_args(e, p, e->fin, N);
         a.a0 = p.cur16; a.c0 = C; a.a1 = p.cur16lo; a.c1 = C; a.c2 = C; a.mask = mask; a.flags = GF_MASK; a.out32 = p.v32;
         ProfScope ps(e, s, PC_FINAL, conv_flops(p, e->fin, N));
+        if (sf) {
+            if (!step_fusable(e, p)) return e->fail(ST_ERR_STATE, "run_estimator: this pass cannot carry the Euler update");
+            a.n_items = p.B; a.pair_items = p.B; a.cfg_scale = sf->cfg_strength; a.euler_dt = sf->dt;
+            a.out32 = p.xstate; a.out16 = p.x16; a.out16_lo = p.x16lo;
+            HIPCHK(e, e->dt == DT_BF16 ? launch_conv_gemm2_bf16(G2_PAIR, 1, EPI_CFG_EULER, a, s) : launch_conv_gemm2_f16(G2_PAIR, 1, EPI_CFG_EULER, a, s));
+            return ST_OK;
+        }
         HIPCHK(e, gemm(e, 1, EPI_F32, a, s));
     }
     if (cap) capture(e, "v", p.v32, (int64_t)N * T * e->Mp, false, s);
     return ST_OK;
+}
+
+bool step_fusable(const st_engine* e, const Plan& p) {
+    return e->fused_step && e->kind == KIND_DECODER && !e->capture && p.cfg && p.N == 2 * p.B && e->Mp == kGemmChannelsPerTile &&
+           e->fin.cout == e->Mp && (int64_t)(p.B + 1) * p.T * e->C * 2 < ((int64_t)1 << 32);
 }
 
 int check_handle(st_engine* e, Kind kind) {
@@ -1121,6 +1160,13 @@
         if (value != e->attn_split) { e->drop_graphs(); e->attn_split = value; }
         return ST_OK;
     }
+    if (n == "fused_step" || n == "batched_linears") {
+        if (value != 0 && value != 1) return e->fail(ST_ERR_INVALID, n + ": 0 (separate launches) or 1");
+        if (e->kind != KIND_DECODER) return e->fail(ST_ERR_UNSUPPORTED, n + ": CFM decoder handles only");
+        int& opt = n == "fused_step" ? e->fused_step : e->batched_linears;
+        if (value != opt) { e->drop_graphs(); opt = value; }
+        return ST_OK;
+    }
     if (n == "fused_ffn") return e->fail(ST_ERR_INVALID, "fused_ffn is read-only (ST_FUSED_FFN at st_create)");
     return e->fail(ST_ERR_INVALID, std::string("unknown option: ") + name);
 }
@@ -1129,6 +1175,8 @@
     if (!e || !name || !value) return ST_ERR_INVALID;
     const std::string n(name);
     if (n == "attention_precision") { *value = e->attn_split; return ST_OK; }
+    if (n == "fused_step") { *value = e->fused_step; return ST_OK; }
+    if (n == "batched_linears") { *value = e->batched_linears; return ST_OK; }
     if (n == "fused_ffn") { *value = e->fused_ffn; return ST_OK; }
     return ST_ERR_INVALID;
 }
diff --git a/stabletts_amd/csrc/engine_internal.h b/stabletts_amd/csrc/engine_internal.h
--- a/stabletts_amd/csrc/engine_internal.h
+++ b/stabletts_amd/csrc/engine_internal.h
@@ -150,6 +150,8 @@
     int small_tiles = 256;
     int splitk_target = 256;
     int attn_split = 0;
+    int fused_step = 1;
+    int batched_linears = 1;
     unsigned* lse_cells = nullptr;
     int attn_small_blocks = 32;
     float* kpart = nullptr;
@@ -255,7 +257,9 @@
 int run_prenet(st_engine* e, const Plan& p, hipStream_t s);
 int run_adaln(st_engine* e, const Plan& p, hipStream_t s);
 int run_time_tables(st_engine* e, const Plan& p, hipStream_t s);
-int run_estimator(st_engine* e, const Plan& p, const float* mask, int ev, hipStream_t s);
+struct StepFuse { float cfg_strength, dt; };
+bool step_fusable(const st_engine* e, const Plan& p);
+int run_estimator(st_engine* e, const Plan& p, const float* mask, int ev, hipStream_t s, const StepFuse* sf = nullptr);
 
 int train_prepare(st_engine* e, hipStream_t s);
 void train_invalidate(st_engine* e);
diff --git a/stabletts_amd/csrc/engine_solve.cpp b/stabletts_amd/csrc/engine_solve.cpp
--- a/stabletts_amd/csrc/engine_solve.cpp
+++ b/stabletts_amd/csrc/engine_solve.cpp
@@ -298,7 +298,8 @@
         ProfScope ps(e, s, PC_PREP, 0);
         HIPCHK(e, launch_set_values(p.tvals, tv.data(), (int)tv.size(), s));
         HIPCHK(e, launch_mask_prep(mask + (int64_t)pt.b0 * T, pt.nb, T, p.Tp, p.n_full, p.kv_end, p.kbias, p.t_lim, s));
-        HIPCHK(e, hipMemsetAsync(p.v32, 0, (size_t)p.N * T * e->Mp * 4, s));
+        if (!(sv.solver == ST_SOLVER_EULER && sv.use_cfg && step_fusable(e, p)))
+            HIPCHK(e, hipMemsetAsync(p.v32, 0, (size_t)p.N * T * e->Mp * 4, s));
         HIPCHK(e, launch_cvec_prep(mask + (int64_t)pt.b0 * T, nullptr, pt.nb, T, p.maskbuf, s));
         pt.mask = p.maskbuf;
         HIPCHK(e, launch_to_time_major(e->dt, mu + pt.b0 * sv.bct, pt.nb, e->M, T, e->Mp, nullptr, p.mu16, nullptr, s));
@@ -319,7 +320,10 @@
     const int64_t per_item = sv.per_item, nstate = (int64_t)Bp * per_item;
     const float cfg_strength = sv.cfg_strength, dt = sv.dts[i];
     int rc;
-    if (sv.solver == ST_SOLVER_EULER) {
+    if (sv.solver == ST_SOLVER_EULER && use_cfg && step_fusable(e, p)) {
+        const StepFuse sf{cfg_strength, dt};
+        if ((rc = run_estimator(e, p, pt.mask, i, s, &sf))) return rc;
+    } else if (sv.solver == ST_SOLVER_EULER) {
         if ((rc = run_estimator(e, p, pt.mask, i, s))) return rc;
         ProfScope ps(e, s, PC_ODE, 0);
         HIPCHK(e, launch_cfg_combine(e->dt, p.v32, Bp, per_item, use_cfg, cfg_strength, nullptr, p.xstate, p.x16, p.x16lo, dt, s));
diff --git a/stabletts_amd/csrc/launch.h b/stabletts_amd/csrc/launch.h
--- a/stabletts_amd/csrc/launch.h
+++ b/stabletts_amd/csrc/launch.h
@@ -8,7 +8,8 @@
 
 enum { EPI_ACT16 = 0, EPI_F32 = 1, EPI_RESGATE = 2, EPI_QKV = 3,
        EPI_GELU16 = 4,
-       EPI_SILU = 5 };
+       EPI_SILU = 5,
+       EPI_CFG_EULER = 6 };
 enum { GF_SILU = 1, GF_MASK = 2,
        GF_K2_V_ONLY = 4 };
 
@@ -48,6 +49,7 @@
     unsigned long long drop_seed; unsigned drop_thresh16; float drop_scale;
     int ksplit;
     const float* bias1; int cmid;
+    int pair_items; float cfg_scale, euler_dt;
     unsigned long long* dbg;
 };
 
@@ -55,7 +57,8 @@
        G2_BIG = 3,
        G2_T64 = 4, G2_RC64 = 5,
        G2_PHASED = 6,
-       G2_RC1 = 7 };
+       G2_RC1 = 7,
+       G2_PAIR = 8 };
 hipError_t launch_conv_gemm2_bf16(int cfg, int taps, int epi, const ConvGemmArgs& a, hipStream_t s);
 hipError_t launch_conv_gemm2_f16(int cfg, int taps, int epi, const ConvGemmArgs& a, hipStream_t s);
 hipError_t launch_splitk_finish_bf16(int epi, const ConvGemmArgs& a, const float* part, int S, hipStream_t s);
@@ -110,6 +113,10 @@
 hipError_t launch_linear_multi(const LinearJobs& J, int n, int k, int o, int silu_in, int silu_out, hipStream_t s);
 hipError_t launch_linear(const float* in, int n, int k, const float* W, const float* bias, int o,
                          float* out, int silu_in, int silu_out, hipStream_t s);
+constexpr int kLinearBatchMax = 16;
+struct LinearBatch { const float* W[kLinearBatchMax]; const float* bias[kLinearBatchMax]; int n; };
+hipError_t launch_linear_batch(const float* in, long long in_stride, int n, int k, const LinearBatch& J, int o,
+                               float* out, long long out_stride, int silu_in, int silu_out, hipStream_t s);
 constexpr int kFrameHalo = 4;
 hipError_t launch_mask_prep(const float* mask, int B, int T, int Tp, int* n_full, int* kv_end, float* kbias, int* t_lim, hipStream_t s);
 
diff --git a/stabletts_amd/csrc/misc_kernels.hip b/stabletts_amd/csrc/misc_kernels.hip
--- a/stabletts_amd/csrc/misc_kernels.hip
+++ b/stabletts_amd/csrc/misc_kernels.hip
@@ -84,6 +84,57 @@
     }
 }
 
+template <int R>
+__device__ __forceinline__ void linear_wave_items(const float* in, int n, int k, const float* W, const float* bias,
+                                            int o, float* out, int silu_in, int silu_out) {
+    const int lane = threadIdx.x & 63;
+    const long long wid = (long long)blockIdx.x * 4 + (threadIdx.x >> 6);
+    const int groups = (n + R - 1) / R;
+    if (wid >= (long long)groups * o) return;
+    const int n0 = (int)(wid / o) * R, oi = (int)(wid % o);
+    const float* w = W + (size_t)oi * k;
+    float acc[R];
+#pragma unroll
+    for (int r = 0; r < R; ++r) acc[r] = 0.f;
+    for (int i = lane * 4; i < k; i += 256) {
+        const float4 wv = *(const float4*)(w + i);
+#pragma unroll
+        for (int r = 0; r < R; ++r) {
+            if (n0 + r < n) {
+                float4 xv = *(const float4*)(in + (size_t)(n0 + r) * k + i);
+                if (silu_in) { xv.x = silu_f(xv.x); xv.y = silu_f(xv.y); xv.z = silu_f(xv.z); xv.w = silu_f(xv.w); }
+                acc[r] += xv.x * wv.x + xv.y * wv.y + xv.z * wv.z + xv.w * wv.w;
+            }
+        }
+    }
+    const float bv = bias ? bias[oi] : 0.f;
+#pragma unroll
+    for (int r = 0; r < R; ++r) {
+        if (n0 + r < n) {
+            const float a = wave_sum(acc[r]);
+            if (lane == 0) {
+                float v = a + bv;
+                if (silu_out) v = silu_f(v);
+                out[(size_t)(n0 + r) * o + oi] = v;
+            }
+        }
+    }
+}
+constexpr int kLinearBatchItems = 8;
+__global__ __launch_bounds__(256) void linear_batch_kernel(const float* in, long long in_stride, int n, int k, LinearBatch J,
+                                                           int o, float* out, long long out_stride, int silu_in, int silu_out) {
+    const int set = blockIdx.y;
+    linear_wave_items<kLinearBatchItems>(in + set * in_stride, n, k, J.W[set], J.bias[set], o, out + set * out_stride, silu_in, silu_out);
+}
+hipError_t launch_linear_batch(const float* in, long long in_stride, int n, int k, const LinearBatch& J, int o,
+                               float* out, long long out_stride, int silu_in, int silu_out, hipStream_t s) {
+    if (J.n < 1 || J.n > kLinearBatchMax || (k & 3) || n < 1 || o < 1) return hipErrorInvalidValue;
+    const long long waves = (long long)((n + kLinearBatchItems - 1) / kLinearBatchItems) * o;
+    hipLaunchKernelGGL(linear_batch_kernel, dim3((unsigned)((waves + 3) / 4), (unsigned)J.n), dim3(256), 0, s, in, in_stride, n, k, J, o, out,
+                       out_stride, silu_in, silu_out);
+    return hipGetLastError();
+}
+
 __global__ __launch_bounds__(256) void silu_rows_kernel(const float* in, int64_t n, float* out) {
     const int64_t i = (int64_t)blockIdx.x * 256 + threadIdx.x;
     if (i < n) out[i] = silu_f(in[i]);
@@ -346,29 +397,21 @@
 }
 
 template <class P>
-__device__ __forceinline__ uint2 pack4_lo(float a, float b, float c, float d) {
-    return pack4<P>(a - (float)to16<P>(a), b - (float)to16<P>(b), c - (float)to16<P>(c), d - (float)to16<P>(d));
-}
-
-template <class P>
 __global__ __launch_bounds__(256) void cfg_combine_kernel(const float* v, int64_t half, int use_cfg, float s,
                                                           float* kout, float* xio, typename P::elem* x16,
                                                           typename P::elem* x16lo, float dt) {
     const int64_t i = ((int64_t)blockIdx.x * blockDim.x + threadIdx.x) * 4;
     if (i >= half) return;
     float4 vc = *(const float4*)(v + i);
-    if (use_cfg) {
-        const float4 vu = *(const float4*)(v + half + i);
-        vc.x = vu.x + s * (vc.x - vu.x); vc.y = vu.y + s * (vc.y - vu.y);
-        vc.z = vu.z + s * (vc.z - vu.z); vc.w = vu.w + s * (vc.w - vu.w);
-    }
+    if (use_cfg) vc = cfg_mix4(vc, *(const float4*)(v + half + i), s);
     if (kout) *(float4*)(kout + i) = vc;
     if (xio) {
         float4 x = *(const float4*)(xio + i);
-        x.x += dt * vc.x; x.y += dt * vc.y; x.z += dt * vc.z; x.w += dt * vc.w;
+        uint2 hi, lo;
+        euler_pack4<P>(x, vc, dt, hi, lo);
         *(float4*)(xio + i) = x;
-        if (x16) *(uint2*)(x16 + i) = pack4<P>(x.x, x.y, x.z, x.w);
-        if (x16lo) *(uint2*)(x16lo + i) = pack4_lo<P>(x.x, x.y, x.z, x.w);
+        if (x16) *(uint2*)(x16 + i) = hi;
+        if (x16lo) *(uint2*)(x16lo + i) = lo;
     }
 }
 
```

New measurement: 1.352 million (median of 6 runs). No clear change (+0.8%).
